# StephenTaf/Modern-Search-Engines-Project

Measured on AMD Instinct MI355X. Metric: queries/sec, two-stage retrieval top-100 (BM25 top-1000 + dense full scan + rerank/fuse), higher is better.
Workload: dtype f32 (exact f32 cosines of every returned document; candidates filtered by one pass of f16 products with a measured margin; batches <= 64 queries: f16x2-split products, |err| <= 8e-6) (dense cosine) / f64 (BM25, fuse)

## Files before the change

include/msretr.h:

```cpp
#ifndef MSRETR_H
#define MSRETR_H

#include <stdint.h>

#ifdef __cplusplus
extern "C" {
#endif

#define MSR_ABI_VERSION 15
#define MSR_DIM 768
#define MSR_MAX_K 1024
#define MSR_MAX_QUERY_TERMS 64
#define MSR_RERANK_MAX_CHUNKS 10
#define MSR_TERMSET_SPAN_DOCS 8192
#define MSR_PHRASE_MAX_TERMS 16
#define MSR_PROX_MAX_SPAN 64
#define MSR_SNIPPET_MAX_WEIGHT (1 << 20)
#define MSR_FUZZY_MAX_LEN 32
#define MSR_FUZZY_MAX_WORDS 1024
#define MSR_FUZZY_MAX_LIMIT 16
#define MSR_FUZZY_SPAN_TERMS 1024
#define MSR_FUZZY_WORD_GROUP 16
#define MSR_MERGE_MAX_ENTRIES 8192

typedef enum msr_status {
    MSR_OK = 0,
    MSR_ERR_INVALID = -1,
    MSR_ERR_NOT_BOUND = -2,
    MSR_ERR_HIP = -3,
    MSR_ERR_NOMEM = -4
} msr_status;

typedef struct msr_engine msr_engine;

typedef struct msr_config {
    int32_t struct_size;
    int32_t device;
    int32_t dim;
    int32_t max_queries;
    int32_t max_k;
    int32_t rerank_max_docs;
    int32_t scan_layout;
    int32_t scan_variant;
    int32_t flags;
} msr_config;

#define MSR_CFG_NO_ROW_COPY 1

typedef struct msr_rerank_params {
    double smoothing;
    double max_boost;
    double max_decay;
    int32_t max_chunks;
    int32_t reserved;
} msr_rerank_params;

int msr_abi_version(void);
int msr_create(const msr_config* cfg, msr_engine** out);
int msr_destroy(msr_engine* e);
const char* msr_last_error(const msr_engine* e);

int msr_bind_postings(msr_engine* e, const int64_t* term_off, int64_t n_terms, const int32_t* post_doc,
                      const int32_t* post_tf, int64_t n_postings, const int32_t* doc_len, int64_t n_docs,
                      const float* idf, float avgdl, double k1, double b, void* stream);

int msr_bind_chunks(msr_engine* e, const float* emb, int64_t n_chunks, const int32_t* doc_off,
                    int64_t n_docs, const float* inv_norm, void* stream);
int msr_row_copy_state(const msr_engine* e);
int msr_row_image_state(const msr_engine* e);
int64_t msr_owned_bytes(const msr_engine* e);

int msr_unbind(msr_engine* e);

int msr_bind_doc_meta(msr_engine* e, const int32_t* url_group, int64_t n_docs, void* stream);

int msr_scan_arith(const msr_engine* e);

int msr_scan_width(const msr_engine* e);
int msr_dense_path(const msr_engine* e);
int msr_batch_width(const msr_engine* e);
int msr_batch_gemm_ok(const msr_engine* e);

int msr_interleave_rows(msr_engine* e, const float* src, int64_t n_rows, float* dst, void* stream);

int msr_bm25_topk(msr_engine* e, const int32_t* q_term_off, const int32_t* q_terms, const int32_t* q_qtf,
                  int32_t n_queries, int32_t k, double min_score, int32_t* out_doc, double* out_score,
                  int32_t* out_n, void* stream);

int msr_bm25_topk_within(msr_engine* e, const int32_t* q_term_off, const int32_t* q_terms, const int32_t* q_qtf,
                         int32_t n_queries, int32_t k, double min_score,
                         const uint32_t* set_bits, int32_t n_sets, int64_t set_stride, const int32_t* q_set,
                         int32_t* out_doc, double* out_score, int32_t* out_n, void* stream);

int msr_term_sets(msr_engine* e, int32_t n_rows, const int32_t* must_off, const int32_t* must_terms,
                  const int32_t* not_off, const int32_t* not_terms,
                  const uint32_t* base_bits, int32_t n_base, int64_t base_stride, const int32_t* row_base,
                  uint32_t* out_bits, int64_t out_stride, void* stream);

int msr_bind_tokens(msr_engine* e, const int64_t* tok_off, const int32_t* tok_ids, int64_t n_docs, int64_t n_tokens,
                    void* stream);

int msr_phrase_sets(msr_engine* e, int32_t n_rows, const int32_t* phrase_off, const int32_t* phrase_terms,
                    const uint32_t* cand_bits, int32_t n_cand, int64_t cand_stride, const int32_t* row_cand,
                    uint32_t* out_bits, int64_t out_stride, void* stream);

int msr_proximity_sets(msr_engine* e, int32_t n_rows, const int32_t* phrase_off, const int32_t* phrase_terms,
                       const int32_t* row_span, const int32_t* row_ordered,
                       const uint32_t* cand_bits, int32_t n_cand, int64_t cand_stride, const int32_t* row_cand,
                       uint32_t* out_bits, int64_t out_stride, void* stream);

int msr_best_windows(msr_engine* e, int32_t n_pairs, const int32_t* pair_doc, const int32_t* pair_row,
                     int32_t n_rows, const int32_t* row_off, const int32_t* row_terms, const int32_t* row_weights,
                     const int32_t* row_span, int32_t* out_start, int32_t* out_cover, int32_t* out_hits, uint64_t* out_mask,
                     uint32_t* out_terms, void* stream);

int msr_bind_vocab(msr_engine* e, const int64_t* char_off, const uint16_t* chars, const uint32_t* weight, int64_t n_terms,
                   int64_t n_chars, void* stream);
int64_t msr_fuzzy_scratch_bytes(int64_t n_terms, int32_t n_words, int32_t limit);
int msr_fuzzy_terms(msr_engine* e, int32_t n_words, const int32_t* word_off, const uint16_t* word_chars, const int32_t* word_max,
                    int32_t limit, int32_t* out_term, int32_t* out_dist, int32_t* out_n, int32_t* out_total, void* scratch,
                    int64_t scratch_bytes, void* stream);

int msr_combine_sets(msr_engine* e, int32_t n_rows, const int32_t* and_off, const int32_t* and_rows,
                     const int32_t* not_off, const int32_t* not_rows,
                     const uint32_t* in_bits, int32_t n_in, int64_t in_stride,
                     uint32_t* out_bits, int64_t out_stride, void* stream);

int msr_debug_bm25_split(msr_engine* e, int32_t n_queries, int32_t* tiles_per_item, int32_t* n_segments);

enum { MSR_SELECT_F32 = 0, MSR_SELECT_F64 = 1, MSR_SELECT_F32_WITHIN = 2, MSR_SELECT_F64_LIST = 3 };
typedef struct msr_select_state {
    uint64_t pref_hi, mask_hi;
    uint32_t pref_lo, mask_lo;
    int32_t k_rem, n_above, done, n_sel;
} msr_select_state;
int msr_debug_select(msr_engine* e, int32_t mode, const void* scores, int64_t n, int64_t stride, int32_t n_queries, int32_t k,
                     const int32_t* idx, const int32_t* counts, int32_t n_seg, int64_t seg_stride, const uint64_t* win_base,
                     const uint32_t* set_bits, int32_t n_sets, int64_t set_stride, const int32_t* q_set, const int32_t* gate,
                     int32_t gate_per64, int32_t* out_doc, void* out_score, int32_t* out_n, msr_select_state* out_state,
                     void* stream);

int msr_bm25_score_docs(msr_engine* e, const int32_t* q_term_off, const int32_t* q_terms, const int32_t* q_qtf,
                        int32_t n_queries, const int32_t* doc, const int32_t* doc_n, int32_t max_docs,
                        double* out_score, int32_t* out_touched, void* stream);
int msr_union_candidates(msr_engine* e, int32_t n_queries,
                         const int32_t* lex_doc, const double* lex_score, const int32_t* lex_n, int32_t k_lex,
                         const int32_t* dense_doc, const double* dense_bm25, const int32_t* dense_n, int32_t k_dense,
                         int32_t* out_doc, double* out_score, int32_t* out_src, int32_t* out_n, int32_t max_cand,
                         void* stream);

int msr_dense_topk(msr_engine* e, const float* q, int32_t n_queries, int32_t k, int32_t max_chunks_per_doc,
                   int32_t* out_doc, float* out_score, int32_t* out_chunk, int32_t* out_n, void* stream);

int msr_dense_topk_within(msr_engine* e, const float* q, int32_t n_queries, int32_t k, int32_t max_chunks_per_doc,
                          const uint32_t* set_bits, int32_t n_sets, int64_t set_stride, const int32_t* q_set,
                          int32_t* out_doc, float* out_score, int32_t* out_chunk, int32_t* out_n, void* stream);

int msr_gather_rows(msr_engine* e, const int32_t* rows, int32_t n, float* out, void* stream);
int msr_dense_topk_grouped(msr_engine* e, const float* q, int32_t n_rows, const int32_t* group_off, int32_t n_groups,
                           const int32_t* excl_off, const int32_t* excl_doc, int32_t k, float min_score,
                           const uint32_t* set_bits, int32_t n_sets, int64_t set_stride, const int32_t* g_set,
                           int32_t* out_doc, float* out_score, int32_t* out_chunk, int32_t* out_src_row, int32_t* out_n,
                           void* stream);

int msr_dense_split_max(const msr_engine* e, int32_t k);
int msr_dense_topk_begin(msr_engine* e, const float* q, int32_t n_queries, int32_t k, int32_t k_part, float* out_part,
                         void* stream);
int msr_dense_topk_end(msr_engine* e, int32_t n_queries, int32_t k, const float* bound, int32_t* out_doc, float* out_score,
                       int32_t* out_chunk, int32_t* out_n, void* stream);

int msr_enable_bf16(msr_engine* e, void* stream);
int msr_dense_topk_bf16(msr_engine* e, const float* q, int32_t n_queries, int32_t k, int32_t max_chunks_per_doc,
                        int32_t* out_doc, float* out_score, int32_t* out_chunk, int32_t* out_n, void* stream);

int msr_rerank(msr_engine* e, const float* q, int32_t n_queries, const int32_t* cand_doc,
               const double* cand_bm25, const int32_t* cand_n, int32_t max_cand,
               const msr_rerank_params* params, int32_t* out_doc, double* out_score, double* out_orig,
               int32_t* out_chunk, int32_t* out_n, int32_t* out_rows, void* stream);

int msr_bind_doc_domains(msr_engine* e, const int32_t* domain, int64_t n_docs, void* stream);
int msr_diversify(msr_engine* e, int32_t n_queries, const int32_t* fused_doc, const double* fused_score,
                  const double* fused_orig, const int32_t* fused_chunk, const int32_t* fused_n, int32_t max_cand,
                  int32_t top_k, double relevance_threshold, int32_t diversify, int32_t* out_doc, double* out_score,
                  double* out_orig, int32_t* out_chunk, int32_t* out_n, void* stream);

int64_t msr_format_lines(const char* qnum_blob, const int64_t* qnum_off, int32_t n_queries, const int32_t* doc,
                         const double* score, const int32_t* n, int32_t stride, const char* url_blob, const int64_t* url_off,
                         int64_t n_docs, int64_t max_url_len, char* out, int64_t capacity);

int msr_rerank_gather(msr_engine* e, const float* q, int32_t n_queries, const int32_t* cand_doc,
                      const int32_t* cand_n, int32_t max_cand, int32_t doc_base, int32_t row_base,
                      int32_t max_chunks, float* out_cos, int32_t* out_meta, void* stream);
int msr_rerank_gather_blocks(msr_engine* e, const float* q, int32_t n_queries, const int32_t* cand_doc,
                             const int32_t* cand_n, int32_t max_cand, int32_t doc_base, int32_t row_base,
                             int32_t max_chunks, int32_t* out_blocks, int32_t queries_per_block, int64_t block_words,
                             void* stream);
int msr_rerank_fuse(msr_engine* e, int32_t n_queries, const int32_t* cand_doc, const double* cand_bm25,
                    const int32_t* cand_n, int32_t max_cand, const float* cos, const int32_t* meta,
                    const msr_rerank_params* params, int32_t* out_doc, double* out_score, double* out_orig,
                    int32_t* out_chunk, int32_t* out_n, int32_t* out_rows, void* stream);

int msr_rerank_combine(msr_engine* e, const float* cos_parts, const int32_t* meta_parts, int32_t n_parts,
                       int64_t part_stride_bytes, int32_t n_queries, int32_t max_cand, float* out_cos,
                       int32_t* out_meta, void* stream);

int msr_rerank_plan(msr_engine* e, int32_t n_queries, const int32_t* cand_doc, const int32_t* cand_n, int32_t max_cand,
                    const int32_t* shard_bounds, int32_t n_shards, int32_t my_shard, int32_t queries_per_shard,
                    int32_t* counts, int32_t* send_base, int32_t* send_blk, int32_t* recv_off, int32_t* pair, void* stream);
int msr_rerank_gather_records(msr_engine* e, const float* q, int32_t n_queries, const int32_t* cand_doc,
                              const int32_t* cand_n, int32_t max_cand, int32_t doc_base, int32_t row_base,
                              int32_t max_chunks, const int32_t* send_base, const int32_t* send_blk, int32_t* out_records,
                              int64_t capacity_records, void* stream);
int msr_rerank_scatter(msr_engine* e, const int32_t* records, int64_t capacity_records, const int32_t* counts,
                       const int32_t* recv_off, int32_t n_shards, int32_t n_queries, int32_t queries_per_shard,
                       int32_t first_query, int32_t n_my_queries, int32_t max_cand, float* out_cos, int32_t* out_meta,
                       void* stream);

int msr_merge_topk(msr_engine* e, const int32_t* in_doc, const void* in_score, const int32_t* in_n,
                   int32_t n_parts, int32_t n_queries, int32_t k, int32_t score_bits, int32_t* out_doc,
                   void* out_score, int32_t* out_n, void* stream);
int msr_merge_topk_payload(msr_engine* e, const int32_t* in_doc, const void* in_score, const int32_t* in_n,
                           const int32_t* in_payload, int32_t n_parts, int64_t part_stride_bytes, int32_t n_queries,
                           int32_t k, int32_t score_bits, int32_t* out_doc, void* out_score, int32_t* out_n,
                           int32_t* out_payload, void* stream);

int msr_build_postings(const int64_t* tok_off, const int32_t* tok_ids, int64_t n_docs, int32_t n_terms, int64_t* term_off,
                       int32_t* post_doc, int32_t* post_tf, int64_t capacity, int64_t* n_postings, void* stream);

int msr_merge_postings(const int64_t* a_term_off, int64_t a_terms, const int32_t* a_doc, const int32_t* a_tf,
                       const int32_t* a_map, int64_t a_docs, const int64_t* b_term_off, int64_t b_terms, const int32_t* b_doc,
                       const int32_t* b_tf, const int32_t* b_map, int64_t b_docs, int64_t n_terms, int64_t n_docs,
                       int64_t* term_off, int32_t* post_doc, int32_t* post_tf, int64_t capacity, void* stream);
// ... 18 lines not shown
```

modern-search-engines-project_amd/_abi.py:

```python
import ctypes as C
import os

HERE = os.path.dirname(os.path.abspath(__file__))
LIB_PATH = os.path.join(HERE, "csrc", "libmsretr.so")

MSR_ABI_VERSION = 15
MSR_CFG_NO_ROW_COPY = 1
MSR_DIM = 768
MSR_MAX_K = 1024
MSR_RERANK_MAX_CHUNKS = 10
MSR_MERGE_MAX_ENTRIES = 8192
MSR_TERMSET_SPAN_DOCS = 8192
MSR_PHRASE_MAX_TERMS = 16
MSR_PROX_MAX_SPAN = 64
MSR_SNIPPET_MAX_WEIGHT = 1 << 20
MSR_FUZZY_MAX_LEN = 32
MSR_FUZZY_MAX_WORDS = 1024
MSR_FUZZY_MAX_LIMIT = 16
MSR_FUZZY_SPAN_TERMS = 1024
MSR_FUZZY_WORD_GROUP = 16
MSR_SELECT_F32, MSR_SELECT_F64, MSR_SELECT_F32_WITHIN, MSR_SELECT_F64_LIST = 0, 1, 2, 3


class MsrError(RuntimeError):
    def __init__(self, code, msg):
        super().__init__(f"libmsretr error {code}: {msg}")
        self.code = code


class MsrConfig(C.Structure):
    _fields_ = [("struct_size", C.c_int32), ("device", C.c_int32), ("dim", C.c_int32),
                ("max_queries", C.c_int32), ("max_k", C.c_int32), ("rerank_max_docs", C.c_int32),
                ("scan_layout", C.c_int32), ("scan_variant", C.c_int32), ("flags", C.c_int32)]


class MsrSelectState(C.Structure):
    _fields_ = [("pref_hi", C.c_uint64), ("mask_hi", C.c_uint64), ("pref_lo", C.c_uint32), ("mask_lo", C.c_uint32),
                ("k_rem", C.c_int32), ("n_above", C.c_int32), ("done", C.c_int32), ("n_sel", C.c_int32)]


class MsrRerankParams(C.Structure):
    _fields_ = [("smoothing", C.c_double), ("max_boost", C.c_double), ("max_decay", C.c_double),
                ("max_chunks", C.c_int32), ("reserved", C.c_int32)]


_P = C.c_void_p
_SIGNATURES = {
    "msr_abi_version": (C.c_int, []),
    "msr_create": (C.c_int, [C.POINTER(MsrConfig), C.POINTER(_P)]),
    "msr_destroy": (C.c_int, [_P]),
    "msr_last_error": (C.c_char_p, [_P]),
    "msr_bind_postings": (C.c_int, [_P, _P, C.c_int64, _P, _P, C.c_int64, _P, C.c_int64, _P, C.c_float,
                                    C.c_double, C.c_double, _P]),
    "msr_bind_chunks": (C.c_int, [_P, _P, C.c_int64, _P, C.c_int64, _P, _P]),
    "msr_bind_doc_meta": (C.c_int, [_P, _P, C.c_int64, _P]),
    "msr_unbind": (C.c_int, [_P]),
    "msr_scan_arith": (C.c_int, [_P]),
    "msr_scan_width": (C.c_int, [_P]),
    "msr_dense_path": (C.c_int, [_P]),
    "msr_row_copy_state": (C.c_int, [_P]),
    "msr_row_image_state": (C.c_int, [_P]),
    "msr_owned_bytes": (C.c_int64, [_P]),
    "msr_enc_layernorm": (C.c_int, [_P, _P, _P, _P, _P, C.c_int64, C.c_int32, C.c_float, _P]),
    "msr_enc_attention": (C.c_int, [_P, _P, C.c_int32, C.c_int32, _P, C.c_int32, C.c_int32, _P, _P]),
    "msr_enc_attention_long": (C.c_int, [_P, _P, C.c_int32, C.c_int32, _P, C.c_int32, C.c_int32, _P, _P]),
    "msr_enc_geglu": (C.c_int, [_P, _P, C.c_int64, C.c_int32, _P]),
    "msr_enc_linear": (C.c_int, [_P, _P, _P, _P, C.c_int32, C.c_int32, C.c_int32, _P]),
    "msr_enc_mean_pool": (C.c_int, [_P, _P, C.c_int32, C.c_int32, C.c_int32, _P, _P]),
    "msr_batch_width": (C.c_int, [_P]),
    "msr_batch_gemm_ok": (C.c_int, [_P]),
    "msr_interleave_rows": (C.c_int, [_P, _P, C.c_int64, _P, _P]),
    "msr_bm25_topk": (C.c_int, [_P, _P, _P, _P, C.c_int32, C.c_int32, C.c_double, _P, _P, _P, _P]),
    "msr_dense_topk": (C.c_int, [_P, _P, C.c_int32, C.c_int32, C.c_int32, _P, _P, _P, _P, _P]),
    "msr_bm25_topk_within": (C.c_int, [_P, _P, _P, _P, C.c_int32, C.c_int32, C.c_double, _P, C.c_int32, C.c_int64, _P, _P, _P,
                                       _P, _P]),
    "msr_dense_topk_within": (C.c_int, [_P, _P, C.c_int32, C.c_int32, C.c_int32, _P, C.c_int32, C.c_int64, _P, _P, _P, _P, _P,
                                        _P]),
    "msr_term_sets": (C.c_int, [_P, C.c_int32, _P, _P, _P, _P, _P, C.c_int32, C.c_int64, _P, _P, C.c_int64, _P]),
    "msr_bind_tokens": (C.c_int, [_P, _P, _P, C.c_int64, C.c_int64, _P]),
    "msr_phrase_sets": (C.c_int, [_P, C.c_int32, _P, _P, _P, C.c_int32, C.c_int64, _P, _P, C.c_int64, _P]),
    "msr_proximity_sets": (C.c_int, [_P, C.c_int32, _P, _P, _P, _P, _P, C.c_int32, C.c_int64, _P, _P, C.c_int64, _P]),
    "msr_best_windows": (C.c_int, [_P, C.c_int32, _P, _P, C.c_int32, _P, _P, _P, _P, _P, _P, _P, _P, _P, _P]),
    "msr_bind_vocab": (C.c_int, [_P, _P, _P, _P, C.c_int64, C.c_int64, _P]),
    "msr_fuzzy_scratch_bytes": (C.c_int64, [C.c_int64, C.c_int32, C.c_int32]),
    "msr_fuzzy_terms": (C.c_int, [_P, C.c_int32, _P, _P, _P, C.c_int32, _P, _P, _P, _P, _P, C.c_int64, _P]),
    "msr_combine_sets": (C.c_int, [_P, C.c_int32, _P, _P, _P, _P, _P, C.c_int32, C.c_int64, _P, C.c_int64, _P]),
    "msr_debug_bm25_split": (C.c_int, [_P, C.c_int32, C.POINTER(C.c_int32), C.POINTER(C.c_int32)]),
    "msr_debug_select": (C.c_int, [_P, C.c_int32, _P, C.c_int64, C.c_int64, C.c_int32, C.c_int32, _P, _P, C.c_int32, C.c_int64, _P,
                                   _P, C.c_int32, C.c_int64, _P, _P, C.c_int32, _P, _P, _P, _P, _P]),
    "msr_bm25_score_docs": (C.c_int, [_P, _P, _P, _P, C.c_int32, _P, _P, C.c_int32, _P, _P, _P]),
    "msr_union_candidates": (C.c_int, [_P, C.c_int32, _P, _P, _P, C.c_int32, _P, _P, _P, C.c_int32, _P, _P, _P, _P, C.c_int32, _P]),
    "msr_gather_rows": (C.c_int, [_P, _P, C.c_int32, _P, _P]),
    "msr_dense_topk_grouped": (C.c_int, [_P, _P, C.c_int32, _P, C.c_int32, _P, _P, C.c_int32, C.c_float, _P, C.c_int32, C.c_int64,
                                         _P, _P, _P, _P, _P, _P, _P]),
    "msr_dense_split_max": (C.c_int, [_P, C.c_int32]),
    "msr_dense_topk_begin": (C.c_int, [_P, _P, C.c_int32, C.c_int32, C.c_int32, _P, _P]),
    "msr_dense_topk_end": (C.c_int, [_P, C.c_int32, C.c_int32, _P, _P, _P, _P, _P, _P]),
    "msr_enable_bf16": (C.c_int, [_P, _P]),
    "msr_dense_topk_bf16": (C.c_int, [_P, _P, C.c_int32, C.c_int32, C.c_int32, _P, _P, _P, _P, _P]),
    "msr_rerank": (C.c_int, [_P, _P, C.c_int32, _P, _P, _P, C.c_int32, C.POINTER(MsrRerankParams), _P, _P, _P,
                             _P, _P, _P, _P]),
    "msr_bind_doc_domains": (C.c_int, [_P, _P, C.c_int64, _P]),
    "msr_diversify": (C.c_int, [_P, C.c_int32, _P, _P, _P, _P, _P, C.c_int32, C.c_int32, C.c_double, C.c_int32, _P, _P, _P, _P,
                                _P, _P]),
    "msr_format_lines": (C.c_int64, [_P, _P, C.c_int32, _P, _P, _P, C.c_int32, _P, _P, C.c_int64, C.c_int64, _P, C.c_int64]),
    "msr_rerank_gather": (C.c_int, [_P, _P, C.c_int32, _P, _P, C.c_int32, C.c_int32, C.c_int32, C.c_int32, _P, _P, _P]),
    "msr_rerank_gather_blocks": (C.c_int, [_P, _P, C.c_int32, _P, _P, C.c_int32, C.c_int32, C.c_int32, C.c_int32, _P, C.c_int32,
                                           C.c_int64, _P]),
    "msr_rerank_fuse": (C.c_int, [_P, C.c_int32, _P, _P, _P, C.c_int32, _P, _P, C.POINTER(MsrRerankParams), _P, _P,
                                  _P, _P, _P, _P, _P]),
    "msr_rerank_combine": (C.c_int, [_P, _P, _P, C.c_int32, C.c_int64, C.c_int32, C.c_int32, _P, _P, _P]),
    "msr_rerank_plan": (C.c_int, [_P, C.c_int32, _P, _P, C.c_int32, _P, C.c_int32, C.c_int32, C.c_int32, _P, _P, _P, _P, _P, _P]),
    "msr_rerank_gather_records": (C.c_int, [_P, _P, C.c_int32, _P, _P, C.c_int32, C.c_int32, C.c_int32, C.c_int32, _P, _P, _P, C.c_int64,
                                            _P]),
    "msr_rerank_scatter": (C.c_int, [_P, _P, C.c_int64, _P, _P, C.c_int32, C.c_int32, C.c_int32, C.c_int32, C.c_int32, C.c_int32, _P, _P, _P]),
    "msr_merge_topk": (C.c_int, [_P, _P, _P, _P, C.c_int32, C.c_int32, C.c_int32, C.c_int32, _P, _P, _P, _P]),
    "msr_merge_topk_payload": (C.c_int, [_P, _P, _P, _P, _P, C.c_int32, C.c_int64, C.c_int32, C.c_int32, C.c_int32, _P, _P, _P,
                                         _P, _P]),
    "msr_build_postings": (C.c_int, [_P, _P, C.c_int64, C.c_int32, _P, _P, _P, C.c_int64, C.POINTER(C.c_int64), _P]),
    "msr_merge_postings": (C.c_int, [_P, C.c_int64, _P, _P, _P, C.c_int64, _P, C.c_int64, _P, _P, _P, C.c_int64, C.c_int64,
                                     C.c_int64, _P, _P, _P, C.c_int64, _P]),
    "msr_compact_postings": (C.c_int, [_P, C.c_int64, _P, _P, _P, C.c_int64, _P, _P, _P, C.c_int64, C.POINTER(C.c_int64), _P]),
    "msr_debug_exclusive_scan": (C.c_int, [_P, C.c_int64, _P, _P, _P]),
    "msr_debug_chunk_layout": (C.c_int, [_P, C.c_int64, C.POINTER(C.c_int32)]),
    "msr_set_timing": (C.c_int, [_P, C.c_int32]),
    "msr_tune": (C.c_int, [_P, C.c_int32, C.c_int32]),
    "msr_kernel_time_ms": (C.c_int, [_P, C.c_int32, C.POINTER(C.c_float), C.POINTER(C.c_int32)]),
}
EXPORTS = tuple(_SIGNATURES)

_lib = None


def load():
    global _lib
    if _lib is not None:
        return _lib
    if not os.path.exists(LIB_PATH):
        raise MsrError(-100, f"{LIB_PATH} not found: build it with `python -c 'import __graft_entry__ as g; "
                             f"g.build()'` (the product path has no CPU fallback)")
    import torch
    lib = C.CDLL(LIB_PATH)
    for name, (res, args) in _SIGNATURES.items():
        fn = getattr(lib, name)
        fn.restype, fn.argtypes = res, args
    if lib.msr_abi_version() != MSR_ABI_VERSION:
        raise MsrError(-101, f"ABI version {lib.msr_abi_version()} != {MSR_ABI_VERSION}")
    _lib = lib
    return lib


def check(handle, rc):
    if rc != 0:
        msg = load().msr_last_error(handle)
        raise MsrError(rc, msg.decode("utf-8", "replace") if msg else "?")
```

modern-search-engines-project_amd/csrc/msr_engine.hip:

```cpp
#include <hip/hip_runtime.h>
#include <stdarg.h>
#include <stdio.h>
#include <stdlib.h>
#include <string.h>

#include <algorithm>
#include <new>
#include <vector>

#include "../../include/msretr.h"
#include "msr_devmem.h"
#include "msr_internal.h"

struct HipMem {
    static hipError_t alloc(void** p, size_t bytes) { return hipMalloc(p, bytes); }
    static void free(void* p) { (void)hipFree(p); }
};
using Group = DevGroup<HipMem>;

struct msr_engine {
    msr_config cfg;
    char err[512];
    Group mem_engine;
    Group mem_corpus;
    Group mem_postings;
    Group mem_chunks;
    Group mem_bf16;
    Bm25Index bm25{};
    bool have_postings = false;
    const int64_t* tok_off = nullptr;
    const int32_t* tok_ids = nullptr;
    int64_t n_tokens = 0;
    bool have_tokens = false;
    const int64_t* voc_char_off = nullptr;
    const uint16_t* voc_chars = nullptr;
    const uint32_t* voc_weight = nullptr;
    int64_t voc_n_chars = 0;
    bool have_vocab = false;
    DenseIndex dense{};
    bool have_chunks = false;
    const int32_t* url_group = nullptr;
    int64_t url_group_n = 0;
    const int32_t* doc_domain = nullptr;
    int64_t doc_domain_n = 0;
    int32_t* chunk_doc = nullptr;
    void* emb_presplit = nullptr;
    void* row_meta = nullptr;
    float* inv_norm_own = nullptr;
    int32_t* span_doc = nullptr;
    int32_t* wspan_doc = nullptr;
    int32_t* wspan12_doc = nullptr;
    float* qn = nullptr;
    float* rr_qn = nullptr;
    void* qimg = nullptr;
    SelScratch sel{};
    float* rerank_cos = nullptr;
    int32_t* rerank_meta = nullptr;
    void* score_rows = nullptr;
    size_t score_rows_bytes = 0;
    int32_t* bm_cand_doc = nullptr;
    size_t bm_cand_bytes = 0;
    int32_t* bm_heavy_id = nullptr;
    void* bm_post = nullptr;
    int32_t* bm_dense_id = nullptr;
    double* bm_dense = nullptr;
    uint32_t* bm_tile_off = nullptr;
    int32_t* bm_cand_n = nullptr;
    uint64_t* bm_win = nullptr;
    uint64_t* voc_sig = nullptr;
    int32_t* bt_top_doc = nullptr; float* bt_top_score = nullptr; int32_t* bt_top_n = nullptr;
    int32_t* bt_cand_doc = nullptr; float* bt_cand_score = nullptr; int32_t* bt_cand_chunk = nullptr;
    int32_t* bt_cand_n = nullptr;
    int32_t* tile_row = nullptr;
    int n_tiles = 0;
    bool tiles_ok = false;
    GemmF32Index gf{};
    bool gf_ok = false;
    float* gf_inv_pad = nullptr; float* gf_qn = nullptr; void* gf_fb_qimg = nullptr;
    int32_t* gf_gate = nullptr;
    void* gf_emb_tiled = nullptr;
    void* gf_emb_f16 = nullptr;
    int32_t* tile_trow = nullptr;
    void* emb_bf16 = nullptr;
    GemmIndex gemm{};
    bool gemm_ok = false;
    float* gm_qn = nullptr;
    uint32_t* bf_err = nullptr;
    float* bf_margin = nullptr;
    float* bf_ones = nullptr;
    void* bf_row_meta = nullptr;
    DenseIndex dense_bf16{};
    int n_cus = 256;
    int split_pending = 0;
    int row_copy_state = 0;
    int row_image_state = 0;
    int last_dense_width = 0;
    int32_t* sim_flag = nullptr;
    void* sim_lists = nullptr; size_t sim_lists_bytes = 0;
    void* sim_over = nullptr; size_t sim_over_bytes = 0;
    bool timing = false;
    static constexpr int EV_RING = 256;
    static constexpr int EV_KINDS = 4;
    hipEvent_t ev_start[EV_KINDS][EV_RING] = {};
    hipEvent_t ev_stop[EV_KINDS][EV_RING] = {};
    int ev_count[EV_KINDS] = {0, 0, 0, 0};
};

static constexpr size_t GF_GATE_BYTES = 16 * sizeof(int32_t);

static thread_local char g_create_err[512] = "";

static int fail(msr_engine* e, int code, const char* fmt, ...) {
    char* dst = e ? e->err : g_create_err;
    va_list ap;
    va_start(ap, fmt);
    vsnprintf(dst, 512, fmt, ap);
    va_end(ap);
    return code;
}

#define HIP_TRY(e, call)                                                                          \
    do {                                                                                          \
        hipError_t _err = (call);                                                                 \
        if (_err != hipSuccess) return fail(e, MSR_ERR_HIP, "%s: %s", #call, hipGetErrorString(_err)); \
    } while (0)

#define ALLOC(e, group, slot, bytes)                                                              \
    do {                                                                                          \
        const size_t _n = (bytes);                                                                \
        hipError_t _err = (group).alloc(&(slot), _n);                                             \
        if (_err != hipSuccess) return fail(e, MSR_ERR_NOMEM, "%s (%zu bytes): %s", #slot, _n, hipGetErrorString(_err)); \
    } while (0)

static void drop_vocab(msr_engine* e) {
    e->have_vocab = false;
    e->voc_char_off = nullptr; e->voc_chars = nullptr; e->voc_weight = nullptr; e->voc_n_chars = 0;
    e->mem_postings.free_one(&e->voc_sig);
}
static void drop_postings(msr_engine* e) {
    e->have_postings = e->have_tokens = false;
    e->tok_off = nullptr; e->tok_ids = nullptr; e->n_tokens = 0;
    drop_vocab(e);
    e->bm25 = Bm25Index{};
    e->mem_postings.release();
}
static void drop_bf16(msr_engine* e) {
    e->dense.emb_bf16 = nullptr;
    e->dense_bf16 = DenseIndex{};
    e->gemm = GemmIndex{};
    e->gemm_ok = false;
    e->mem_bf16.release();
}
static void drop_chunks(msr_engine* e) {
    e->have_chunks = false;
    e->split_pending = 0;
    e->dense = DenseIndex{};
    e->gf = GemmF32Index{};
    e->gf_ok = e->tiles_ok = false;
    e->n_tiles = 0;
    e->row_copy_state = e->row_image_state = 0;
    drop_bf16(e);
    e->mem_chunks.release();
}

template <class T>
static int grow(msr_engine* e, Group& group, T** slot, size_t* have, size_t need, const char* what) {
    if (need <= *have && *slot) return MSR_OK;
    group.free_one(slot);
    *have = 0;
    hipError_t herr = group.alloc(slot, need);
    if (herr != hipSuccess) return fail(e, MSR_ERR_NOMEM, "%s (%zu bytes): %s", what, need, hipGetErrorString(herr));
    *have = need;
    return MSR_OK;
}

extern "C" int msr_abi_version(void) { return MSR_ABI_VERSION; }

extern "C" const char* msr_last_error(const msr_engine* e) { return e ? e->err : g_create_err; }

int msr_fail_global(int code, const char* fmt, ...) {
    va_list ap;
    va_start(ap, fmt);
    vsnprintf(g_create_err, sizeof(g_create_err), fmt, ap);
    va_end(ap);
    return code;
}

static int create_scratch(msr_engine* e) {
    const msr_config& cfg = e->cfg;
    HIP_TRY(e, hipSetDevice(cfg.device));
    hipDeviceProp_t prop;
    HIP_TRY(e, hipGetDeviceProperties(&prop, cfg.device));
    e->n_cus = prop.multiProcessorCount > 0 ? prop.multiProcessorCount : 256;
    const size_t nq = (size_t)std::max(cfg.max_queries, 128);
    ALLOC(e, e->mem_engine, e->qn, 128 * MSR_DIM * sizeof(float));
    ALLOC(e, e->mem_engine, e->qimg, 256 * 1024);
    if (cfg.rerank_max_docs > 0) ALLOC(e, e->mem_engine, e->rr_qn, nq * MSR_DIM * sizeof(float));
    ALLOC(e, e->mem_engine, e->sel.hist, nq * MSR_SEL_BINS * sizeof(uint32_t));
    ALLOC(e, e->mem_engine, e->sel.state, nq * sizeof(SelState));
    ALLOC(e, e->mem_engine, e->sel.cand_hi, nq * MSR_SEL_CAP * sizeof(uint64_t));
    ALLOC(e, e->mem_engine, e->sel.cand_lo, nq * MSR_SEL_CAP * sizeof(uint32_t));
    ALLOC(e, e->mem_engine, e->sel.cand_n, nq * sizeof(int32_t));
    HIP_TRY(e, hipMemset(e->sel.hist, 0, nq * MSR_SEL_BINS * sizeof(uint32_t)));
    HIP_TRY(e, hipMemset(e->sel.cand_n, 0, nq * sizeof(int32_t)));
    if (cfg.rerank_max_docs > 0) {
        ALLOC(e, e->mem_engine, e->rerank_cos, nq * (size_t)cfg.rerank_max_docs * MSR_RERANK_MAX_CHUNKS * sizeof(float));
        ALLOC(e, e->mem_engine, e->rerank_meta, nq * (size_t)cfg.rerank_max_docs * 3 * sizeof(int32_t));
    }
    for (int w = 0; w < msr_engine::EV_KINDS; ++w)
        for (int j = 0; j < msr_engine::EV_RING; ++j) {
            HIP_TRY(e, hipEventCreate(&e->ev_start[w][j]));
            HIP_TRY(e, hipEventCreate(&e->ev_stop[w][j]));
        }
    return MSR_OK;
}

extern "C" int msr_create(const msr_config* cfg, msr_engine** out) {
    if (!cfg || !out) return fail(nullptr, MSR_ERR_INVALID, "msr_create: null argument");
    *out = nullptr;
    if (cfg->struct_size != (int32_t)sizeof(msr_config))
        return fail(nullptr, MSR_ERR_INVALID, "msr_create: struct_size %d != %zu", cfg->struct_size, sizeof(msr_config));
    if (cfg->dim != MSR_DIM) return fail(nullptr, MSR_ERR_INVALID, "msr_create: dim must be %d", MSR_DIM);
    if (cfg->max_queries < 1 || cfg->max_queries > 4096)
        return fail(nullptr, MSR_ERR_INVALID, "msr_create: max_queries out of range [1, 4096]");
    if (cfg->max_k < 1 || cfg->max_k > MSR_MAX_K)
        return fail(nullptr, MSR_ERR_INVALID, "msr_create: max_k out of range [1, %d]", MSR_MAX_K);
    if (cfg->rerank_max_docs < 0 || cfg->rerank_max_docs > 1024)
        return fail(nullptr, MSR_ERR_INVALID, "msr_create: rerank_max_docs out of range [0, 1024]");
    if (cfg->scan_layout != 0 && cfg->scan_layout != 1)
        return fail(nullptr, MSR_ERR_INVALID, "msr_create: scan_layout must be 0 or 1");
    if (cfg->scan_variant != 0 && cfg->scan_variant != 2 && cfg->scan_variant != 7 && cfg->scan_variant != 14 &&
        cfg->scan_variant != 15)
        return fail(nullptr, MSR_ERR_INVALID, "msr_create: scan_variant must be 0, 2, 7, 14 or 15");
    if (cfg->flags & ~(int32_t)MSR_CFG_NO_ROW_COPY)
        return fail(nullptr, MSR_ERR_INVALID, "msr_create: unknown flag bits 0x%x", cfg->flags);
    int ndev = 0;
    hipError_t herr = hipGetDeviceCount(&ndev);
    if (herr != hipSuccess || ndev <= 0)
        return fail(nullptr, MSR_ERR_HIP, "msr_create: no HIP device available (%s)",
                    herr == hipSuccess ? "device count is 0" : hipGetErrorString(herr));
    if (cfg->device < 0 || cfg->device >= ndev)
        return fail(nullptr, MSR_ERR_INVALID, "msr_create: device %d out of range (have %d)", cfg->device, ndev);
    msr_engine* e = new (std::nothrow) msr_engine();
    if (!e) return fail(nullptr, MSR_ERR_NOMEM, "msr_create: out of host memory");
    e->cfg = *cfg;
    e->err[0] = 0;
    const int rc = create_scratch(e);
    if (rc) {
        fail(nullptr, rc, "msr_create: %s", e->err);
        msr_destroy(e);
        return rc;
    }
    *out = e;
    return MSR_OK;
}

extern "C" int msr_destroy(msr_engine* e) {
    if (!e) return MSR_OK;
    drop_postings(e);
    drop_chunks(e);
    for (int w = 0; w < msr_engine::EV_KINDS; ++w)
        for (int j = 0; j < msr_engine::EV_RING; ++j) {
            if (e->ev_start[w][j]) (void)hipEventDestroy(e->ev_start[w][j]);
            if (e->ev_stop[w][j]) (void)hipEventDestroy(e->ev_stop[w][j]);
        }
    delete e;
    return MSR_OK;
}

static int ensure_score_rows(msr_engine* e, int64_t n_docs) {
    const size_t pad = (size_t)(n_docs + 31) / 32 * 32;
    const size_t need = std::max((size_t)e->cfg.max_queries * pad * sizeof(double), (size_t)128 * pad * sizeof(float));
    return grow(e, e->mem_corpus, &e->score_rows, &e->score_rows_bytes, need, "score rows");
}

static int build_postings(msr_engine* e, Bm25Index cand, hipStream_t st) {
    const int64_t n_terms = cand.n_terms, n_postings = cand.n_postings, n_docs = cand.n_docs;
    int rc = ensure_score_rows(e, n_docs);
    if (rc) return rc;
    rc = grow(e, e->mem_corpus, &e->bm_cand_doc, &e->bm_cand_bytes, (size_t)e->cfg.max_queries * (size_t)n_docs * sizeof(int32_t),
              "BM25 candidate lists");
    if (rc) return rc;
    ALLOC(e, e->mem_postings, e->bm_win, (size_t)e->cfg.max_queries * sizeof(uint64_t));
    ALLOC(e, e->mem_postings, e->bm_cand_n, (size_t)e->cfg.max_queries * msr_bm25_max_segments(n_docs) * sizeof(int32_t));
    int32_t h_flag = 0;
    HIP_TRY(e, msr_bm25_validate(cand, e->sel.cand_n, st));
    HIP_TRY(e, hipMemcpyAsync(&h_flag, e->sel.cand_n, sizeof(int32_t), hipMemcpyDeviceToHost, st));
    HIP_TRY(e, hipMemsetAsync(e->sel.cand_n, 0, sizeof(int32_t), st));
    HIP_TRY(e, hipStreamSynchronize(st));
    if (h_flag >= 1 && h_flag <= 5) {
        static const char* why[] = {"", "term_off is not a monotone offset array ending at n_postings",
                                    "a posting's document index is outside [0, n_docs)",
                                    "documents are not strictly ascending inside a posting list",
                                    "negative doc_len", "non-positive term frequency"};
        return fail(e, MSR_ERR_INVALID, "msr_bind_postings: malformed index: %s", why[h_flag]);
    }
    if (!(cand.avgdl > 0.0) || !(cand.k1 >= 0.0) || !(cand.b >= 0.0 && cand.b <= 1.0))
        return fail(e, MSR_ERR_INVALID, "msr_bind_postings: avgdl must be > 0, k1 >= 0, 0 <= b <= 1");
    std::vector<int32_t> dense_terms;
    if (n_terms > 0) {
        std::vector<int64_t> h_toff((size_t)n_terms + 1);
        std::vector<float> h_idf((size_t)n_terms);
        HIP_TRY(e, hipMemcpyAsync(h_toff.data(), cand.term_off, h_toff.size() * sizeof(int64_t), hipMemcpyDeviceToHost, st));
        HIP_TRY(e, hipMemcpyAsync(h_idf.data(), cand.idf, h_idf.size() * sizeof(float), hipMemcpyDeviceToHost, st));
        HIP_TRY(e, hipStreamSynchronize(st));
        std::vector<int32_t> heavy_id((size_t)n_terms, -1), heavy_terms;
        for (int64_t t = 0; t < n_terms; ++t)
            if (h_toff[t + 1] - h_toff[t] >= MSR_BM25_HEAVY_DF && h_toff[t + 1] - h_toff[t] < (1ll << 32)) {
                heavy_id[t] = (int32_t)heavy_terms.size();
                heavy_terms.push_back((int32_t)t);
                if (h_idf[t] < 0.0f) dense_terms.push_back((int32_t)t);
            }
        if (!heavy_terms.empty()) {
            DevTemp<HipMem, int32_t> d_terms;
            const size_t rows = heavy_terms.size() * (size_t)(cand.n_tiles + 1);
            ALLOC(e, e->mem_postings, e->bm_heavy_id, heavy_id.size() * sizeof(int32_t));
            ALLOC(e, e->mem_postings, e->bm_tile_off, rows * sizeof(uint32_t));
            ALLOC(e, d_terms.group, d_terms.p, heavy_terms.size() * sizeof(int32_t));
            HIP_TRY(e, hipMemcpyAsync(e->bm_heavy_id, heavy_id.data(), heavy_id.size() * sizeof(int32_t), hipMemcpyHostToDevice, st));
            HIP_TRY(e, hipMemcpyAsync(d_terms.p, heavy_terms.data(), heavy_terms.size() * sizeof(int32_t), hipMemcpyHostToDevice, st));
            HIP_TRY(e, msr_bm25_build_skip(cand, d_terms.p, (int)heavy_terms.size(), e->bm_tile_off, st));
            HIP_TRY(e, hipStreamSynchronize(st));
            cand.heavy_id = e->bm_heavy_id;
            cand.tile_off = e->bm_tile_off;
        }
        std::stable_sort(dense_terms.begin(), dense_terms.end(), [&](int32_t a, int32_t b2) {
            return h_toff[a + 1] - h_toff[a] > h_toff[b2 + 1] - h_toff[b2];
        });
        const size_t row_bytes = ((size_t)cand.n_tiles * MSR_BM25_TILE + 8) * sizeof(double);
        const size_t cap = std::min<size_t>(MSR_BM25_MAX_DENSE, (size_t)(4ull << 30) / row_bytes);
        if (dense_terms.size() > cap) dense_terms.resize(cap);
    }
    {
        const int64_t n_pad = (int64_t)cand.n_tiles * MSR_BM25_TILE;
        DevTemp<HipMem, double> dnorm;
        ALLOC(e, e->mem_postings, e->bm_post, (size_t)(n_postings + 1) * sizeof(Bm25Post));
        ALLOC(e, dnorm.group, dnorm.p, (size_t)n_pad * sizeof(double));
        HIP_TRY(e, msr_bm25_dnorm(cand.doc_len, n_docs, n_pad, cand.k1, cand.b, cand.avgdl, dnorm.p, st));
        HIP_TRY(e, msr_bm25_post_comp(cand.post_doc, cand.post_tf, dnorm.p, cand.k1, n_postings, (Bm25Post*)e->bm_post, st));
        HIP_TRY(e, hipStreamSynchronize(st));
    }
    cand.post = (const Bm25Post*)e->bm_post;
    if (!dense_terms.empty()) {
        const int64_t stride = (int64_t)cand.n_tiles * MSR_BM25_TILE + 8;
        std::vector<int32_t> dense_id((size_t)n_terms, -1);
        for (size_t h = 0; h < dense_terms.size(); ++h) dense_id[dense_terms[h]] = (int32_t)h;
        DevTemp<HipMem, int32_t> d_terms;
        ALLOC(e, e->mem_postings, e->bm_dense_id, dense_id.size() * sizeof(int32_t));
        ALLOC(e, e->mem_postings, e->bm_dense, dense_terms.size() * (size_t)stride * sizeof(double));
        ALLOC(e, d_terms.group, d_terms.p, dense_terms.size() * sizeof(int32_t));
        HIP_TRY(e, hipMemcpyAsync(e->bm_dense_id, dense_id.data(), dense_id.size() * sizeof(int32_t), hipMemcpyHostToDevice, st));
        HIP_TRY(e, hipMemcpyAsync(d_terms.p, dense_terms.data(), dense_terms.size() * sizeof(int32_t), hipMemcpyHostToDevice, st));
        HIP_TRY(e, hipMemsetAsync(e->bm_dense, 0, dense_terms.size() * (size_t)stride * sizeof(double), st));
        HIP_TRY(e, msr_bm25_build_dense(cand, d_terms.p, (int)dense_terms.size(), e->bm_dense, stride, st));
        HIP_TRY(e, hipStreamSynchronize(st));
        cand.dense_id = e->bm_dense_id;
        cand.dense_comp = e->bm_dense;
        cand.dense_stride = stride;
    }
    e->bm25 = cand;
    return MSR_OK;
}

extern "C" int msr_bind_postings(msr_engine* e, const int64_t* term_off, int64_t n_terms, const int32_t* post_doc,
                                 const int32_t* post_tf, int64_t n_postings, const int32_t* doc_len, int64_t n_docs,
                                 const float* idf, float avgdl, double k1, double b, void* stream) {
    if (!e) return MSR_ERR_INVALID;
    if (!term_off || !doc_len || !idf || n_terms < 0 || n_postings < 0 || n_docs <= 0 || n_docs >= (1ll << 31) ||
        (n_postings > 0 && (!post_doc || !post_tf)))
        return fail(e, MSR_ERR_INVALID, "msr_bind_postings: bad argument");
    if (e->have_chunks && e->dense.n_docs != n_docs)
        return fail(e, MSR_ERR_INVALID, "msr_bind_postings: n_docs %lld differs from bound chunks (%lld)",
                    (long long)n_docs, (long long)e->dense.n_docs);
    HIP_TRY(e, hipSetDevice(e->cfg.device));
    drop_postings(e);
    const Bm25Index cand{term_off, post_doc, post_tf, doc_len, idf, n_terms, n_postings, n_docs, (double)avgdl, k1, b,
                         nullptr, nullptr, (int32_t)((n_docs + MSR_BM25_TILE - 1) / MSR_BM25_TILE), nullptr, nullptr, nullptr, 0};
    const int rc = build_postings(e, cand, (hipStream_t)stream);
    if (rc) drop_postings(e);
    e->have_postings = rc == MSR_OK;
    return rc;
}

struct ChunkLayout {
    std::vector<int32_t> spans, wspans, wspans12;
    int wide_ok = 1, wide_ok64 = 1;
    bool tiles_ok = true;
    std::vector<int32_t> tiles;
    std::vector<int32_t> trow;
    int64_t n_trows = 0;
};

static int chunk_layout(msr_engine* e, int n_cus, const std::vector<int32_t>& h_off, int64_t n_chunks, int64_t n_docs,
                        ChunkLayout& L) {
    if (h_off[0] != 0 || (int64_t)h_off[n_docs] != n_chunks)
        return fail(e, MSR_ERR_INVALID, "msr_bind_chunks: doc_off[0]=%d, doc_off[n_docs]=%d, n_chunks=%lld",
                    h_off[0], h_off[n_docs], (long long)n_chunks);
    for (int64_t d = 0; d < n_docs; ++d)
        if (h_off[d + 1] < h_off[d]) return fail(e, MSR_ERR_INVALID, "msr_bind_chunks: doc_off not monotone at %lld", (long long)d);
    auto make_spans = [&](int target, int64_t min_rows) {
        if ((int64_t)target * min_rows > n_chunks) target = (int)std::max<int64_t>(1, n_chunks / min_rows);
        std::vector<int32_t> sp;
        sp.push_back(0);
        for (int s = 1; s < target; ++s) {
            const int64_t want = n_chunks * s / target;
            int64_t d = std::lower_bound(h_off.begin(), h_off.end(), (int32_t)want) - h_off.begin();
            if (d > n_docs) d = n_docs;
            if (d > sp.back()) sp.push_back((int32_t)d);
        }
        if (sp.back() != (int32_t)n_docs) sp.push_back((int32_t)n_docs);
        return sp;
    };
    L.spans = make_spans(n_cus, 256);
    L.wspans = make_spans(n_cus * 8, 64);
    L.wspans12 = make_spans(n_cus * 12, 64);
    {
        const int64_t n_groups = (n_chunks + 15) / 16;
        int64_t dl = 0, dr = 0;
        for (int64_t u = 0; u < n_groups && (L.wide_ok || L.wide_ok64); ++u) {
            const int64_t first = 16 * u, last = std::min<int64_t>(16 * (u + 2), n_chunks) - 1;
            while (h_off[dl + 1] <= first) ++dl;
            if (dr < dl) dr = dl;
            while (h_off[dr + 1] <= last) ++dr;
            if (dr - dl + 32 > MSR_WIDE_RING) L.wide_ok = 0;
            if (dr - dl + 32 > 64) L.wide_ok64 = 0;
            int64_t dm = dl;
            const int64_t glast = std::min<int64_t>(16 * (u + 1), n_chunks) - 1;
            while (h_off[dm + 1] <= glast) ++dm;
            if (dm - dl > 32) L.wide_ok = L.wide_ok64 = 0;
        }
    }
    if (L.wide_ok || L.wide_ok64) {
        int64_t lag = 0;
        for (size_t s = 0; s + 1 < L.spans.size(); ++s) {
            const int64_t d0 = L.spans[s], d1 = L.spans[s + 1];
            const int64_t c0 = h_off[d0], c1 = h_off[d1];
            if (c1 <= c0) continue;
            auto block_end = [&](int64_t b) -> int64_t { return h_off[std::min(b + 32, d1)]; };
            int64_t next_b = d0 & ~(int64_t)31;
            while (next_b < d1 && block_end(next_b) <= c0) next_b += 32;
            int64_t d = d0;
            for (int64_t g = c0 >> 4; g < (c1 + 15) >> 4; ++g) {
                const int64_t last = std::min(16 * g + 16, c1) - 1;
                while (h_off[d + 1] <= last) ++d;
                lag = std::max(lag, d - next_b);
                for (int i = 0; i < 2 && next_b < d1 && block_end(next_b) <= 16 * g; ++i) next_b += 32;
            }
        }
        if (lag >= MSR_WIDE_RING) L.wide_ok = 0;
        if (lag >= 64) L.wide_ok64 = 0;
    }
    int32_t start = 0;
    L.tiles.push_back(0);
    for (int64_t d = 0; d < n_docs && L.tiles_ok; ++d) {
        const int32_t end = h_off[d + 1];
        if (end - h_off[d] > 256) L.tiles_ok = false;
        if (end - start > 256) { L.tiles.push_back(h_off[d]); start = h_off[d]; }
    }
    if (!L.tiles_ok) return MSR_OK;
    if (L.tiles.back() != (int32_t)n_chunks) L.tiles.push_back((int32_t)n_chunks);
    const size_t n_tiles = L.tiles.size() - 1;
    L.trow.resize(n_tiles);
    for (size_t t = 0; t < n_tiles; ++t) {
        L.trow[t] = (int32_t)L.n_trows;
        L.n_trows += (L.tiles[t + 1] - L.tiles[t] + 15) / 16 * 16;
    }
    if (L.n_trows + MSR_STREAM256_TILE_ROWS >= ((int64_t)1 << 31)) { L.trow.clear(); L.n_trows = 0; }
    return MSR_OK;
}

static int bind_chunk_tables(msr_engine* e, const float* emb, int64_t n_chunks, const int32_t* doc_off, int64_t n_docs,
                             const float* inv_norm, const ChunkLayout& L, hipStream_t st) {
    ALLOC(e, e->mem_chunks, e->chunk_doc, (size_t)n_chunks * sizeof(int32_t));
    ALLOC(e, e->mem_chunks, e->span_doc, L.spans.size() * sizeof(int32_t));
    ALLOC(e, e->mem_chunks, e->wspan_doc, L.wspans.size() * sizeof(int32_t));
    HIP_TRY(e, hipMemcpyAsync(e->span_doc, L.spans.data(), L.spans.size() * sizeof(int32_t), hipMemcpyHostToDevice, st));
    HIP_TRY(e, hipMemcpyAsync(e->wspan_doc, L.wspans.data(), L.wspans.size() * sizeof(int32_t), hipMemcpyHostToDevice, st));
    ALLOC(e, e->mem_chunks, e->wspan12_doc, L.wspans12.size() * sizeof(int32_t));
    HIP_TRY(e, hipMemcpyAsync(e->wspan12_doc, L.wspans12.data(), L.wspans12.size() * sizeof(int32_t), hipMemcpyHostToDevice, st));
    HIP_TRY(e, msr_fill_chunk_doc(doc_off, n_docs, e->chunk_doc, st));
    if (!inv_norm) {
        ALLOC(e, e->mem_chunks, e->inv_norm_own, (size_t)n_chunks * sizeof(float));
        HIP_TRY(e, msr_row_inv_norm(emb, n_chunks, e->inv_norm_own, st));
        inv_norm = e->inv_norm_own;
    }
    if (L.wide_ok) {
        ALLOC(e, e->mem_chunks, e->row_meta, (size_t)(n_chunks + 16) * 8);
        HIP_TRY(e, msr_pack_row_meta(e->chunk_doc, inv_norm, n_chunks, e->row_meta, st));
    }
    int variant = e->cfg.scan_variant;
    if (variant == 0) {
        uint32_t h_rng[2] = {0, 0};
        HIP_TRY(e, msr_inv_norm_range(inv_norm, n_chunks, (uint32_t*)e->sel.cand_n, st));
        HIP_TRY(e, hipMemcpyAsync(h_rng, e->sel.cand_n, sizeof(h_rng), hipMemcpyDeviceToHost, st));
        HIP_TRY(e, hipMemsetAsync(e->sel.cand_n, 0, 2 * sizeof(int32_t), st));
        HIP_TRY(e, hipStreamSynchronize(st));
        float lo, hi;
        memcpy(&lo, &h_rng[0], 4); memcpy(&hi, &h_rng[1], 4);
        variant = (lo >= 0.5f && hi <= 2.0f) ? 7 : 2;
        if (variant == 7 && e->cfg.scan_layout == 0 && L.wide_ok) variant = 14;
    }
    if (variant == 15) {
        if (e->cfg.scan_layout != 0 || !L.wide_ok) {
            variant = 7;
        } else {
            ALLOC(e, e->mem_chunks, e->emb_presplit, (size_t)n_chunks * MSR_DIM * sizeof(float));
            HIP_TRY(e, msr_presplit_rows(emb, n_chunks, e->emb_presplit, st));
        }
    }
    e->dense = DenseIndex{emb, doc_off, e->chunk_doc, inv_norm, e->span_doc, n_chunks, n_docs, (n_docs + 31) / 32 * 32,
                          (int)L.spans.size() - 1, e->cfg.scan_layout, e->wspan_doc, (int)L.wspans.size() - 1, e->wspan12_doc,
                          (int)L.wspans12.size() - 1, e->qimg, nullptr, e->emb_presplit, e->row_meta, L.wide_ok,
                          L.wide_ok && L.wide_ok64, nullptr, variant};
    if (L.tiles_ok) {
        ALLOC(e, e->mem_chunks, e->tile_row, L.tiles.size() * 4);
        HIP_TRY(e, hipMemcpyAsync(e->tile_row, L.tiles.data(), L.tiles.size() * 4, hipMemcpyHostToDevice, st));
        e->n_tiles = (int)L.tiles.size() - 1;
        e->tiles_ok = true;
    }
    if (!L.trow.empty()) {
        ALLOC(e, e->mem_chunks, e->tile_trow, L.trow.size() * 4);
        HIP_TRY(e, hipMemcpyAsync(e->tile_trow, L.trow.data(), L.trow.size() * 4, hipMemcpyHostToDevice, st));
    }
    HIP_TRY(e, hipStreamSynchronize(st));
    return MSR_OK;
}

static int bind_stream_pass(msr_engine* e, const ChunkLayout& L, hipStream_t st) {
    if (!(e->tiles_ok && e->dense.variant == 14 && e->n_tiles >= 64)) return MSR_OK;
    const float* emb = e->dense.emb;
    const float* inv_norm = e->dense.inv_norm;
    const int64_t n_chunks = e->dense.n_chunks;
    const int n_tiles = e->n_tiles, nw = e->n_cus * 8, stride = (n_tiles + 31) / 32 * 32;
    const int groups = std::min(8, std::max(e->cfg.max_queries, 128) / 128);
    const int GF_WV_CAP = 4096 * std::max(1, groups / 2);
    const size_t QM = (size_t)groups * 128;
    const int max_nt = std::max(1, std::min(4, groups / 2));
    GemmF32Index& g = e->gf;
    g.n_tiles = n_tiles; g.n_cus = e->n_cus; g.max_groups = groups; g.tmax_stride = stride; g.wv_cap = GF_WV_CAP; g.max_nt = max_nt;
    ALLOC(e, e->mem_chunks, e->gf_inv_pad, (size_t)(n_chunks + 512) * 4);
    ALLOC(e, e->mem_chunks, g.qimg, (size_t)groups * 24 * 8192);
    ALLOC(e, e->mem_chunks, e->gf_qn, (QM + 64) * MSR_DIM * 4);
    ALLOC(e, e->mem_chunks, e->gf_fb_qimg, (QM + 63) / 64 * msr_ksplit_slice_image_bytes());
    ALLOC(e, e->mem_chunks, g.tmax_t, (size_t)n_tiles * 8 * (groups >= 2 ? 256 * max_nt : 128) * 4);
    ALLOC(e, e->mem_chunks, g.tmax, QM * stride * 4);
    ALLOC(e, e->mem_chunks, g.thr, QM * 4);
    ALLOC(e, e->mem_chunks, g.thr2, QM * 4);
    ALLOC(e, e->mem_chunks, g.flag, QM * 4);
    ALLOC(e, e->mem_chunks, g.wvbuf, (size_t)nw * GF_WV_CAP * 16);
    ALLOC(e, e->mem_chunks, g.wv_count, (size_t)nw * 4);
    ALLOC(e, e->mem_chunks, g.pairs, QM * 4096 * 8);
    ALLOC(e, e->mem_chunks, g.pair_n, QM * 4);
    ALLOC(e, e->mem_chunks, e->gf_gate, GF_GATE_BYTES);
    ALLOC(e, e->mem_chunks, g.err_max, 4);
    ALLOC(e, e->mem_chunks, g.margin, QM * 4);
    ALLOC(e, e->mem_chunks, g.cand_doc, QM * MSR_SEL_CAP * 4);
    ALLOC(e, e->mem_chunks, g.cand_score, QM * MSR_SEL_CAP * 4);
    ALLOC(e, e->mem_chunks, g.cand_chunk, QM * MSR_SEL_CAP * 4);
    ALLOC(e, e->mem_chunks, g.cand_n, QM * 4);
    g.tile_row = e->tile_row;
    g.inv_pad = e->gf_inv_pad;
    HIP_TRY(e, msr_pad_inv_norm(inv_norm, n_chunks, n_chunks + 512, e->gf_inv_pad, st));
    HIP_TRY(e, hipMemsetAsync(g.pair_n, 0, QM * 4, st));
    HIP_TRY(e, hipMemsetAsync(e->gf_gate, 0, GF_GATE_BYTES, st));
    HIP_TRY(e, hipMemsetAsync(g.cand_n, 0, QM * 4, st));
    HIP_TRY(e, msr_f16_row_error(emb, inv_norm, n_chunks, g.err_max, st));
    if (groups >= 2 && e->tile_trow) {
        const size_t copy_rows = (size_t)L.n_trows + MSR_STREAM256_TILE_ROWS;
        if ((int64_t)L.trow.back() + MSR_STREAM256_TILE_ROWS > (int64_t)copy_rows)
            return fail(e, MSR_ERR_INVALID, "msr_bind_chunks: internal: tile table exceeds the fragment-order copy");
        if (e->cfg.flags & MSR_CFG_NO_ROW_COPY) {
            e->row_copy_state = 2;
        } else if (e->mem_chunks.alloc(&e->gf_emb_tiled, copy_rows * MSR_DIM * 4) != hipSuccess) {
            (void)hipGetLastError();
            e->row_copy_state = 3;
        } else {
            HIP_TRY(e, hipMemsetAsync((char*)e->gf_emb_tiled + (size_t)L.n_trows * MSR_DIM * 4, 0,
                                      (size_t)MSR_STREAM256_TILE_ROWS * MSR_DIM * 4, st));
            HIP_TRY(e, msr_tile_rows(emb, e->tile_row, e->tile_trow, n_tiles, e->gf_emb_tiled, st));
            e->row_copy_state = 1;
        }
    }
    if (max_nt >= 2 && (e->cfg.flags & MSR_CFG_NO_ROW_COPY)) {
        e->row_image_state = 2;
    } else if (max_nt >= 2) {
        const size_t img_rows = (size_t)n_chunks + 512;
        if (e->mem_chunks.alloc(&e->gf_emb_f16, img_rows * MSR_DIM * 2) != hipSuccess) {
            (void)hipGetLastError();
            e->row_image_state = 3;
        } else {
            HIP_TRY(e, msr_f16_rows(emb, n_chunks, (int64_t)img_rows, e->gf_emb_f16, st));
            e->row_image_state = 1;
        }
    }
    g.emb_tiled = e->gf_emb_tiled;
    g.tile_trow = e->gf_emb_tiled ? e->tile_trow : nullptr;
    g.emb_f16 = e->gf_emb_f16;
    e->gf_ok = true;
    return MSR_OK;
}

extern "C" int msr_bind_chunks(msr_engine* e, const float* emb, int64_t n_chunks, const int32_t* doc_off,
                               int64_t n_docs, const float* inv_norm, void* stream) {
    if (!e) return MSR_ERR_INVALID;
    if (!emb || !doc_off || n_chunks <= 0 || n_chunks >= (1ll << 31) || n_docs <= 0 || n_docs >= (1ll << 31))
        return fail(e, MSR_ERR_INVALID, "msr_bind_chunks: bad argument");
    if (e->have_postings && e->bm25.n_docs != n_docs)
        return fail(e, MSR_ERR_INVALID, "msr_bind_chunks: n_docs %lld differs from bound postings (%lld)",
                    (long long)n_docs, (long long)e->bm25.n_docs);
    if (e->cfg.scan_layout == 1 && !inv_norm)
        return fail(e, MSR_ERR_INVALID, "msr_bind_chunks: inv_norm is required with the interleaved layout");
    hipStream_t st = (hipStream_t)stream;
    HIP_TRY(e, hipSetDevice(e->cfg.device));
    std::vector<int32_t> h_off((size_t)n_docs + 1);
    HIP_TRY(e, hipMemcpyAsync(h_off.data(), doc_off, (size_t)(n_docs + 1) * sizeof(int32_t), hipMemcpyDeviceToHost, st));
    HIP_TRY(e, hipStreamSynchronize(st));
    ChunkLayout L;
    int rc = chunk_layout(e, e->n_cus, h_off, n_chunks, n_docs, L);
    if (rc) return rc;
    drop_chunks(e);
    rc = ensure_score_rows(e, n_docs);
    if (!rc) rc = bind_chunk_tables(e, emb, n_chunks, doc_off, n_docs, inv_norm, L, st);
    if (!rc) rc = bind_stream_pass(e, L, st);
    if (rc) drop_chunks(e);
    e->have_chunks = rc == MSR_OK;
    return rc;
}

extern "C" int msr_debug_chunk_layout(const int32_t* doc_off, int64_t n_docs, int32_t out[4]) {
    if (!doc_off || !out || n_docs < 0 || n_docs >= ((int64_t)1 << 31))
        return fail(nullptr, MSR_ERR_INVALID, "msr_debug_chunk_layout: bad argument");
    const int n_cus = out[3] > 0 ? out[3] : 256;
    const std::vector<int32_t> h_off(doc_off, doc_off + n_docs + 1);
    ChunkLayout L;
    const int rc = chunk_layout(nullptr, n_cus, h_off, h_off[n_docs], n_docs, L);
    if (rc) return rc;
    out[0] = L.wide_ok; out[1] = L.wide_ok && L.wide_ok64; out[2] = L.tiles_ok; out[3] = (int32_t)L.spans.size() - 1;
    return MSR_OK;
}

extern "C" int msr_unbind(msr_engine* e) {
    if (!e) return MSR_ERR_INVALID;
    HIP_TRY(e, hipSetDevice(e->cfg.device));
    drop_postings(e);
    drop_chunks(e);
    e->url_group = nullptr; e->url_group_n = 0;
    e->doc_domain = nullptr; e->doc_domain_n = 0;
    e->last_dense_width = 0;
    e->mem_corpus.release();
    e->score_rows_bytes = e->bm_cand_bytes = 0;
    return MSR_OK;
}

extern "C" int msr_bind_doc_meta(msr_engine* e, const int32_t* url_group, int64_t n_docs, void* stream) {
    (void)stream;
    if (!e) return MSR_ERR_INVALID;
    if (url_group && e->have_chunks && n_docs != e->dense.n_docs)
        return fail(e, MSR_ERR_INVALID, "msr_bind_doc_meta: n_docs mismatch");
    e->url_group = url_group;
    e->url_group_n = n_docs;
    return MSR_OK;
}

extern "C" int msr_bind_doc_domains(msr_engine* e, const int32_t* domain, int64_t n_docs, void* stream) {
    (void)stream;
    if (!e) return MSR_ERR_INVALID;
    if (n_docs < 0 || (domain && n_docs == 0)) return fail(e, MSR_ERR_INVALID, "msr_bind_doc_domains: bad argument");
    e->doc_domain = domain;
    e->doc_domain_n = domain ? n_docs : 0;
    return MSR_OK;
}

extern "C" int msr_diversify(msr_engine* e, int32_t n_queries, const int32_t* fused_doc, const double* fused_score,
                             const double* fused_orig, const int32_t* fused_chunk, const int32_t* fused_n, int32_t max_cand,
                             int32_t top_k, double relevance_threshold, int32_t diversify, int32_t* out_doc, double* out_score,
                             double* out_orig, int32_t* out_chunk, int32_t* out_n, void* stream) {
    if (!e) return MSR_ERR_INVALID;
    if (!fused_doc || !fused_score || !fused_orig || !fused_chunk || !fused_n || !out_doc || !out_score || !out_orig || !out_chunk ||
        !out_n)
        return fail(e, MSR_ERR_INVALID, "msr_diversify: null argument");
    if (n_queries < 0 || max_cand < 1 || max_cand > 1024 || top_k < 1)
        return fail(e, MSR_ERR_INVALID, "msr_diversify: bad argument (max_cand=%d, top_k=%d)", max_cand, top_k);
    if (n_queries == 0) return MSR_OK;
    HIP_TRY(e, hipSetDevice(e->cfg.device));
    HIP_TRY(e, msr_diversify_run(n_queries, fused_doc, fused_score, fused_orig, fused_chunk, fused_n, max_cand, e->doc_domain,
                                 e->doc_domain_n, top_k, relevance_threshold, diversify, out_doc, out_score, out_orig, out_chunk,
                                 out_n, (hipStream_t)stream));
    return MSR_OK;
}

extern "C" int msr_interleave_rows(msr_engine* e, const float* src, int64_t n_rows, float* dst, void* stream) {
    if (!e) return MSR_ERR_INVALID;
    if (!src || !dst || n_rows <= 0 || src == dst) return fail(e, MSR_ERR_INVALID, "msr_interleave_rows: bad argument");
    HIP_TRY(e, hipSetDevice(e->cfg.device));
    HIP_TRY(e, msr_interleave(src, n_rows, dst, (hipStream_t)stream));
    return MSR_OK;
}

extern "C" int msr_scan_arith(const msr_engine* e) {
    if (!e || !e->have_chunks) return -1;
    const int v = e->dense.variant;
    return (v == 7 || v == 14 || v == 15) ? 1 : 0;
}

extern "C" int msr_scan_width(const msr_engine* e) {
    if (!e || !e->have_chunks) return -1;
    const int v = e->dense.variant;
    const bool wide = (v == 2 || v == 14 || v == 15) && e->dense.layout == 0 && e->dense.wide_ok;
    if (e->gf_ok && wide && v == 14) return e->gf.max_groups >= 2 ? 256 : 128;
    return wide ? 64 : 32;
}

extern "C" int msr_dense_path(const msr_engine* e) { return e ? e->last_dense_width : -1; }

extern "C" int64_t msr_owned_bytes(const msr_engine* e) {
    if (!e) return -1;
    return (int64_t)(e->mem_engine.bytes() + e->mem_corpus.bytes() + e->mem_postings.bytes() + e->mem_chunks.bytes() +
                     e->mem_bf16.bytes());
}

extern "C" int msr_row_copy_state(const msr_engine* e) { return e ? e->row_copy_state : -1; }
extern "C" int msr_row_image_state(const msr_engine* e) { return e ? e->row_image_state : -1; }

extern "C" int msr_batch_width(const msr_engine* e) {
    if (!e || !e->have_chunks || !e->emb_bf16) return -1;
    return e->dense.wide_ok && e->dense.wide_ok64 ? 128 : 64;
}

extern "C" int msr_set_timing(msr_engine* e, int32_t enabled) {
    if (!e) return MSR_ERR_INVALID;
    e->timing = enabled != 0;
    for (int w = 0; w < msr_engine::EV_KINDS; ++w) e->ev_count[w] = 0;
    return MSR_OK;
}

extern "C" int msr_kernel_time_ms(msr_engine* e, int32_t which, float* out_ms, int32_t* out_launches) {
    if (!e || which < 0 || which >= msr_engine::EV_KINDS || !out_ms) return e ? fail(e, MSR_ERR_INVALID, "msr_kernel_time_ms: bad argument") : MSR_ERR_INVALID;
    const int n = std::min(e->ev_count[which], (int)msr_engine::EV_RING);
    if (n <= 0) return fail(e, MSR_ERR_INVALID, "msr_kernel_time_ms: no timed launch recorded");
    float total = 0.f;
    for (int j = 0; j < n; ++j) {
        float ms = 0.f;
        HIP_TRY(e, hipEventSynchronize(e->ev_stop[which][j]));
        HIP_TRY(e, hipEventElapsedTime(&ms, e->ev_start[which][j], e->ev_stop[which][j]));
        total += ms;
    }
    *out_ms = total;
    if (out_launches) *out_launches = n;
    return MSR_OK;
}

static int within_args_ok(msr_engine* e, const char* fn, int64_t n_docs, const uint32_t* set_bits, int32_t n_sets,
                          int64_t set_stride, const int32_t* q_set) {
    if (n_sets < 0) return fail(e, MSR_ERR_INVALID, "%s: bad argument (n_sets=%d)", fn, n_sets);
    if (n_sets == 0) return MSR_OK;
    if (!set_bits || !q_set) return fail(e, MSR_ERR_INVALID, "%s: bad argument (set_bits or q_set is NULL with n_sets=%d)", fn, n_sets);
    if (set_stride < (n_docs + 31) / 32)
        return fail(e, MSR_ERR_INVALID, "%s: bad argument (set_stride=%lld < ceil(n_docs / 32) = %lld)", fn, (long long)set_stride,
                    (long long)((n_docs + 31) / 32));
    return MSR_OK;
}

static int bm25_topk_impl(msr_engine* e, const char* fn, const int32_t* q_term_off, const int32_t* q_terms, const int32_t* q_qtf,
                          int32_t n_queries, int32_t k, double min_score, int32_t* out_doc, double* out_score, int32_t* out_n,
                          void* stream, const uint32_t* set_bits, int32_t n_sets, int64_t set_stride, const int32_t* q_set) {
    if (!e) return MSR_ERR_INVALID;
    if (!e->have_postings) return fail(e, MSR_ERR_NOT_BOUND, "%s: postings not bound", fn);
    if (n_queries < 0 || k < 1 || k > e->cfg.max_k || !q_term_off || !out_doc || !out_score || !out_n)
        return fail(e, MSR_ERR_INVALID, "%s: bad argument (k=%d, max_k=%d)", fn, k, e->cfg.max_k);
    {
        const int rc = within_args_ok(e, fn, e->bm25.n_docs, set_bits, n_sets, set_stride, q_set);
        if (rc) return rc;
    }
    if (n_queries == 0) return MSR_OK;
    const MsrSetView set_view{set_bits, set_stride, q_set, n_sets};
    const MsrSetView* set = n_sets > 0 ? &set_view : nullptr;
    hipStream_t st = (hipStream_t)stream;
    HIP_TRY(e, hipSetDevice(e->cfg.device));
    const int slice = e->cfg.max_queries;
    const int64_t N = e->bm25.n_docs;
    for (int q0 = 0; q0 < n_queries; q0 += slice) {
        const int nq = std::min(slice, n_queries - q0);
        int32_t* o_doc = out_doc + (int64_t)q0 * k;
        double* o_score = out_score + (int64_t)q0 * k;
        const bool timed = e->timing && e->ev_count[1] < msr_engine::EV_RING;
        int n_seg = 0;
        int64_t seg_stride = 0;
        if (timed) HIP_TRY(e, hipEventRecord(e->ev_start[1][e->ev_count[1]], st));
        HIP_TRY(e, msr_bm25_scores(e->bm25, q_term_off, q_terms, q_qtf, q0, nq, min_score, (double*)e->score_rows, e->bm_cand_doc,
                                   e->bm_cand_n, &n_seg, &seg_stride, st, set));
        if (timed) {
            HIP_TRY(e, hipEventRecord(e->ev_stop[1][e->ev_count[1]], st));
            e->ev_count[1]++;
        }
        const uint64_t* win = nullptr;
        if (min_score >= 0.0) {
            HIP_TRY(e, msr_bm25_window(e->bm25, q_term_off, q_terms, q_qtf, q0, nq, e->bm_win, st));
            win = e->bm_win;
        }
        HIP_TRY(e, msr_select_topk_list((const double*)e->score_rows, e->bm_cand_doc, e->bm_cand_n, n_seg, seg_stride, N, nq, k,
                                        e->sel, o_doc, o_score, out_n + q0, st, win));
    }
    return MSR_OK;
}

extern "C" int msr_bm25_topk(msr_engine* e, const int32_t* q_term_off, const int32_t* q_terms, const int32_t* q_qtf,
                             int32_t n_queries, int32_t k, double min_score, int32_t* out_doc, double* out_score,
                             int32_t* out_n, void* stream) {
    return bm25_topk_impl(e, "msr_bm25_topk", q_term_off, q_terms, q_qtf, n_queries, k, min_score, out_doc, out_score, out_n,
                          stream, nullptr, 0, 0, nullptr);
}

extern "C" int msr_bm25_topk_within(msr_engine* e, const int32_t* q_term_off, const int32_t* q_terms, const int32_t* q_qtf,
                                    int32_t n_queries, int32_t k, double min_score, const uint32_t* set_bits, int32_t n_sets,
                                    int64_t set_stride, const int32_t* q_set, int32_t* out_doc, double* out_score,
                                    int32_t* out_n, void* stream) {
    return bm25_topk_impl(e, "msr_bm25_topk_within", q_term_off, q_terms, q_qtf, n_queries, k, min_score, out_doc, out_score,
                          out_n, stream, set_bits, n_sets, set_stride, q_set);
}

static int tokens_bound(msr_engine* e, const char* fn) {
    if (e->have_postings && e->have_tokens) return MSR_OK;
    return fail(e, MSR_ERR_NOT_BOUND, "%s: tokens not bound (msr_bind_tokens: the index has no forward index)", fn);
}

static int set_rows_args_ok(msr_engine* e, const char* fn, int32_t n_rows, bool rows_ok, const char* rows_what, int64_t out_stride,
                            const char* n_in_name, int32_t n_in, bool in_ok, const char* in_what, const char* in_stride_name,
                            int64_t in_stride) {
    const int64_t W = (e->bm25.n_docs + 31) / 32;
    if (n_rows < 0 || n_in < 0) return fail(e, MSR_ERR_INVALID, "%s: bad argument (n_rows=%d, %s=%d)", fn, n_rows, n_in_name, n_in);
    if (n_rows > 0 && !rows_ok)
        return fail(e, MSR_ERR_INVALID, "%s: bad argument (%s is NULL with n_rows=%d)", fn, rows_what, n_rows);
    if (out_stride < W)
        return fail(e, MSR_ERR_INVALID, "%s: bad argument (out_stride=%lld < ceil(n_docs / 32) = %lld)", fn, (long long)out_stride,
                    (long long)W);
    if (n_in > 0 && !in_ok)
        return fail(e, MSR_ERR_INVALID, "%s: bad argument (%s is NULL with %s=%d)", fn, in_what, n_in_name, n_in);
    if (n_in > 0 && in_stride < W)
        return fail(e, MSR_ERR_INVALID, "%s: bad argument (%s=%lld < ceil(n_docs / 32) = %lld)", fn, in_stride_name,
                    (long long)in_stride, (long long)W);
    return MSR_OK;
}

extern "C" int msr_term_sets(msr_engine* e, int32_t n_rows, const int32_t* must_off, const int32_t* must_terms,
                             const int32_t* not_off, const int32_t* not_terms, const uint32_t* base_bits, int32_t n_base,
                             int64_t base_stride, const int32_t* row_base, uint32_t* out_bits, int64_t out_stride, void* stream) {
    if (!e) return MSR_ERR_INVALID;
    if (!e->have_postings) return fail(e, MSR_ERR_NOT_BOUND, "msr_term_sets: postings not bound");
    const int rc = set_rows_args_ok(e, "msr_term_sets", n_rows, out_bits && must_off && not_off, "out_bits, must_off or not_off",
                                    out_stride, "n_base", n_base, base_bits && row_base, "base_bits or row_base", "base_stride",
                                    base_stride);
    if (rc) return rc;
    if (n_rows == 0) return MSR_OK;
    HIP_TRY(e, hipSetDevice(e->cfg.device));
    HIP_TRY(e, msr_term_sets_run(e->bm25, n_rows, must_off, must_terms, not_off, not_terms, base_bits, n_base, base_stride,
                                 row_base, out_bits, out_stride, (hipStream_t)stream));
    return MSR_OK;
}

extern "C" int msr_bind_tokens(msr_engine* e, const int64_t* tok_off, const int32_t* tok_ids, int64_t n_docs, int64_t n_tokens,
                               void* stream) {
    if (!e) return MSR_ERR_INVALID;
    if (!e->have_postings) return fail(e, MSR_ERR_NOT_BOUND, "msr_bind_tokens: postings not bound");
    e->have_tokens = false; e->tok_off = nullptr; e->tok_ids = nullptr; e->n_tokens = 0;
    if (!tok_off || n_tokens < 0 || (n_tokens > 0 && !tok_ids)) return fail(e, MSR_ERR_INVALID, "msr_bind_tokens: bad argument");
    if (n_docs != e->bm25.n_docs)
// ... 155 lines not shown
}

extern "C" int msr_debug_bm25_split(msr_engine* e, int32_t n_queries, int32_t* tiles_per_item, int32_t* n_segments) {
    if (!e) return MSR_ERR_INVALID;
    if (!e->have_postings) return fail(e, MSR_ERR_NOT_BOUND, "msr_debug_bm25_split: postings not bound");
    if (n_queries < 1 || n_queries > e->cfg.max_queries || !tiles_per_item || !n_segments)
        return fail(e, MSR_ERR_INVALID, "msr_debug_bm25_split: bad argument (n_queries=%d, max_queries=%d)", n_queries,
                    e->cfg.max_queries);
    int tpw = 1, n_spans = 0;
    msr_bm25_split(e->bm25.n_tiles, n_queries, &tpw, &n_spans);
    *tiles_per_item = tpw;
    *n_segments = n_spans;
    return MSR_OK;
}

extern "C" int msr_debug_select(msr_engine* e, int32_t mode, const void* scores, int64_t n, int64_t stride, int32_t n_queries,
                                int32_t k, const int32_t* idx, const int32_t* counts, int32_t n_seg, int64_t seg_stride,
                                const uint64_t* win_base, const uint32_t* set_bits, int32_t n_sets, int64_t set_stride,
                                const int32_t* q_set, const int32_t* gate, int32_t gate_per64, int32_t* out_doc, void* out_score,
                                int32_t* out_n, msr_select_state* out_state, void* stream) {
    static_assert(sizeof(msr_select_state) == sizeof(SelState), "msr_select_state mirrors SelState");
    if (!e) return MSR_ERR_INVALID;
    if (mode < MSR_SELECT_F32 || mode > MSR_SELECT_F64_LIST)
        return fail(e, MSR_ERR_INVALID, "msr_debug_select: bad argument (mode=%d)", mode);
    if (n_queries < 1 || n_queries > e->cfg.max_queries || k < 1 || k > e->cfg.max_k)
        return fail(e, MSR_ERR_INVALID, "msr_debug_select: bad argument (n_queries=%d, max_queries=%d, k=%d, max_k=%d)", n_queries,
                    e->cfg.max_queries, k, e->cfg.max_k);
    if (!scores || !out_doc || !out_score || !out_n || n < 0 || n >= (1ll << 31) || stride < n)
        return fail(e, MSR_ERR_INVALID, "msr_debug_select: bad argument (NULL scores or output, or n=%lld, stride=%lld)",
                    (long long)n, (long long)stride);
    if (mode == MSR_SELECT_F64_LIST && (!idx || !counts || n_seg < 1 || seg_stride < 0 || (int64_t)n_seg * seg_stride > stride))
        return fail(e, MSR_ERR_INVALID, "msr_debug_select: bad argument (list: idx or counts NULL, n_seg=%d < 1, or n_seg * "
                    "seg_stride=%lld > stride=%lld)", n_seg, (long long)seg_stride, (long long)stride);
    if (mode == MSR_SELECT_F32_WITHIN &&
        (n_sets < 1 || !set_bits || !q_set || set_stride < (n + 31) / 32))
        return fail(e, MSR_ERR_INVALID, "msr_debug_select: bad argument (within: n_sets=%d < 1, set_bits or q_set NULL, or "
                    "set_stride=%lld < ceil(n / 32))", n_sets, (long long)set_stride);
    hipStream_t st = (hipStream_t)stream;
    HIP_TRY(e, hipSetDevice(e->cfg.device));
    SelScratch sel = e->sel;
    sel.gate = gate;
    sel.gate_per64 = gate && gate_per64 ? 1 : 0;
    switch (mode) {
    case MSR_SELECT_F32:
        HIP_TRY(e, msr_select_topk(32, scores, n, stride, n_queries, k, sel, out_doc, out_score, out_n, st));
        break;
    case MSR_SELECT_F64:
        HIP_TRY(e, msr_select_topk(64, scores, n, stride, n_queries, k, sel, out_doc, out_score, out_n, st));
        break;
    case MSR_SELECT_F32_WITHIN: {
        const MsrSetView set{set_bits, set_stride, q_set, n_sets};
        HIP_TRY(e, msr_select_topk_within((const float*)scores, n, stride, n_queries, k, sel, set, out_doc, (float*)out_score,
                                          out_n, st));
        break;
    }
    default:
        HIP_TRY(e, msr_select_topk_list((const double*)scores, idx, counts, n_seg, seg_stride, stride, n_queries, k, sel, out_doc,
                                        (double*)out_score, out_n, st, win_base));
    }
    if (out_state)
        HIP_TRY(e, hipMemcpyAsync(out_state, e->sel.state, (size_t)n_queries * sizeof(SelState), hipMemcpyDeviceToDevice, st));
    return MSR_OK;
}

extern "C" int msr_bm25_score_docs(msr_engine* e, const int32_t* q_term_off, const int32_t* q_terms, const int32_t* q_qtf,
                                   int32_t n_queries, const int32_t* doc, const int32_t* doc_n, int32_t max_docs,
                                   double* out_score, int32_t* out_touched, void* stream) {
    if (!e) return MSR_ERR_INVALID;
    if (!e->have_postings) return fail(e, MSR_ERR_NOT_BOUND, "msr_bm25_score_docs: postings not bound");
    if (n_queries < 0 || max_docs < 0 || !q_term_off || (n_queries > 0 && max_docs > 0 && (!doc || !out_score || !out_touched)))
        return fail(e, MSR_ERR_INVALID, "msr_bm25_score_docs: bad argument (n_queries=%d, max_docs=%d)", n_queries, max_docs);
    if (n_queries == 0 || max_docs == 0) return MSR_OK;
    HIP_TRY(e, hipSetDevice(e->cfg.device));
    HIP_TRY(e, msr_bm25_point(e->bm25, q_term_off, q_terms, q_qtf, n_queries, doc, doc_n, max_docs, out_score, out_touched,
                              (hipStream_t)stream));
    return MSR_OK;
}

extern "C" int msr_union_candidates(msr_engine* e, int32_t n_queries, const int32_t* lex_doc, const double* lex_score,
                                    const int32_t* lex_n, int32_t k_lex, const int32_t* dense_doc, const double* dense_bm25,
                                    const int32_t* dense_n, int32_t k_dense, int32_t* out_doc, double* out_score, int32_t* out_src,
                                    int32_t* out_n, int32_t max_cand, void* stream) {
    if (!e) return MSR_ERR_INVALID;
    if (n_queries < 0 || k_lex < 0 || k_lex > MSR_MAX_K || k_dense < 0 || k_dense > MSR_MAX_K || max_cand < 1 ||
        (int64_t)k_lex + k_dense > max_cand)
        return fail(e, MSR_ERR_INVALID, "msr_union_candidates: bad argument (k_lex=%d, k_dense=%d: each in [0, %d], their sum <= "
                    "max_cand=%d)", k_lex, k_dense, MSR_MAX_K, max_cand);
    if (!out_doc || !out_score || !out_src || !out_n || (k_lex > 0 && (!lex_doc || !lex_score || !lex_n)) ||
        (k_dense > 0 && (!dense_doc || !dense_bm25 || !dense_n)))
        return fail(e, MSR_ERR_INVALID, "msr_union_candidates: bad argument (NULL list)");
    if (n_queries == 0) return MSR_OK;
    HIP_TRY(e, hipSetDevice(e->cfg.device));
    HIP_TRY(e, msr_union_lists(n_queries, lex_doc, lex_score, lex_n, k_lex, dense_doc, dense_bm25, dense_n, k_dense, out_doc,
                               out_score, out_src, out_n, max_cand, (hipStream_t)stream));
    return MSR_OK;
}

static int dense_gated_fallback(msr_engine* e, int nq, int k, int32_t* out_doc, float* out_score, int32_t* out_chunk,
                                int32_t* out_n, hipStream_t st) {
    const int64_t N = e->dense.n_docs;
    DenseIndex ix = e->dense;
    ix.gate = e->gf_gate;
    HIP_TRY(e, msr_dense_scan_slices(ix, e->gf_qn, nq, (float*)e->score_rows, e->gf_fb_qimg, st));
    SelScratch sel = e->sel;
    sel.gate = e->gf_gate; sel.gate_per64 = 1;
    HIP_TRY(e, msr_select_topk(32, e->score_rows, N, e->dense.score_stride, nq, k, sel, out_doc, out_score, out_n, st));
    ix.gate = e->gf_gate; ix.gate_per64 = 1;
    if (out_chunk) HIP_TRY(e, msr_best_chunk(ix, e->gf_qn, nq, k, 0, out_doc, out_n, out_chunk, st));
    return MSR_OK;
}

static bool dense_sweep_wide(const msr_engine* e, int max_chunks_per_doc) {
    return (e->dense.variant == 2 || e->dense.variant == 14 || e->dense.variant == 15) && e->dense.layout == 0 &&
           e->dense.wide_ok && max_chunks_per_doc == 0;
}

static bool dense_stream_ok(const msr_engine* e, int k) {
    return dense_sweep_wide(e, 0) && e->gf_ok && e->dense.variant == 14 && e->gf.n_tiles >= 2 * k;
}

static int dense_stream_cap(const msr_engine* e) { return e->gf.max_groups >= 2 ? (e->gf.max_groups & ~1) * 128 : 128; }

static hipEvent_t* pass_events(msr_engine* e, int kind, hipEvent_t ev[4]) {
    if (!e->timing || e->ev_count[kind] >= msr_engine::EV_RING || e->ev_count[3] >= msr_engine::EV_RING) return nullptr;
    ev[0] = e->ev_start[3][e->ev_count[3]]; ev[1] = e->ev_stop[3][e->ev_count[3]];
    ev[2] = e->ev_start[kind][e->ev_count[kind]]; ev[3] = e->ev_stop[kind][e->ev_count[kind]];
    return ev;
}
static void pass_events_used(msr_engine* e, int kind, const hipEvent_t* ev) {
    if (ev) { e->ev_count[kind]++; e->ev_count[3]++; }
}

extern "C" int msr_dense_split_max(const msr_engine* e, int32_t k) {
    if (!e || !e->have_chunks || k < 1 || k > e->cfg.max_k || !dense_stream_ok(e, k)) return 0;
    return dense_stream_cap(e);
}

extern "C" int msr_dense_topk_begin(msr_engine* e, const float* q, int32_t n_queries, int32_t k, int32_t k_part, float* out_part,
                                    void* stream) {
    if (!e) return MSR_ERR_INVALID;
    if (!e->have_chunks) return fail(e, MSR_ERR_NOT_BOUND, "msr_dense_topk_begin: chunks not bound");
    if (e->split_pending) return fail(e, MSR_ERR_INVALID, "msr_dense_topk_begin: the previous begin has not been ended");
    const int cap = msr_dense_split_max(e, k);
    if (!q || !out_part || k_part < 1 || k_part > k || n_queries <= 64 || n_queries > cap)
        return fail(e, MSR_ERR_INVALID, "msr_dense_topk_begin: needs 64 < n_queries <= msr_dense_split_max() = %d, 1 <= k_part <= k (got %d, %d, %d)",
                    cap, n_queries, k_part, k);
    hipStream_t st = (hipStream_t)stream;
    HIP_TRY(e, hipSetDevice(e->cfg.device));
    HIP_TRY(e, msr_prep_queries(q, n_queries, e->gf_qn, (n_queries + 63) / 64 * 64, st));
    HIP_TRY(e, hipMemsetAsync(e->gf_gate, 0, GF_GATE_BYTES, st));
    hipEvent_t ev_buf[4];
    hipEvent_t* ev = pass_events(e, 0, ev_buf);
    int width = 0;
    HIP_TRY(e, msr_gemm_f32_pass(e->gf, e->dense, e->gf_qn, n_queries, k, k_part, out_part, ev, &width, st));
    e->last_dense_width = width;
    pass_events_used(e, 0, ev);
    e->split_pending = n_queries;
    return MSR_OK;
}

extern "C" int msr_dense_topk_end(msr_engine* e, int32_t n_queries, int32_t k, const float* bound, int32_t* out_doc,
                                  float* out_score, int32_t* out_chunk, int32_t* out_n, void* stream) {
    if (!e) return MSR_ERR_INVALID;
    if (!e->have_chunks) return fail(e, MSR_ERR_NOT_BOUND, "msr_dense_topk_end: chunks not bound");
    if (!e->gf_ok || e->split_pending != n_queries || n_queries <= 0)
        return fail(e, MSR_ERR_INVALID, "msr_dense_topk_end: no matching msr_dense_topk_begin (pending %d, got %d)", e->split_pending, n_queries);
    if (!out_doc || !out_score || !out_n || k < 1 || k > e->cfg.max_k) return fail(e, MSR_ERR_INVALID, "msr_dense_topk_end: bad argument");
    e->split_pending = 0;
    hipStream_t st = (hipStream_t)stream;
    HIP_TRY(e, hipSetDevice(e->cfg.device));
    HIP_TRY(e, msr_gemm_f32_finish(e->gf, e->dense, e->gf_qn, n_queries, k, bound, out_doc, out_score, out_chunk, out_n, e->gf_gate, st));
    return dense_gated_fallback(e, n_queries, k, out_doc, out_score, out_chunk, out_n, st);
}

static int dense_sweeps(msr_engine* e, const float* q, int q0, int cnt, int k, int max_chunks_per_doc, bool wide, const int32_t* gate,
                        int32_t* out_doc, float* out_score, int32_t* out_chunk, int32_t* out_n, hipStream_t st,
                        const MsrSetView* set) {
    const int64_t N = e->dense.n_docs;
    const int slice = wide ? 64 : 32;
    DenseIndex ix = e->dense;
    SelScratch sel = e->sel;
    for (int s0 = q0; s0 < q0 + cnt; s0 += slice) {
        const int nq = std::min(slice, q0 + cnt - s0);
        ix.gate = sel.gate = gate ? gate + (s0 - q0) / 64 : nullptr;
        const int nq_pad = nq > 32 ? 64 : (nq > 16 || (wide && e->dense.variant >= 14)) ? 32 : 16;
        const bool timed = !gate && e->timing && e->ev_count[0] < msr_engine::EV_RING;
        HIP_TRY(e, msr_prep_queries(q + (int64_t)s0 * MSR_DIM, nq, e->qn, nq_pad, st));
        if (timed) HIP_TRY(e, hipEventRecord(e->ev_start[0][e->ev_count[0]], st));
        HIP_TRY(e, msr_dense_scan(ix, e->qn, nq, max_chunks_per_doc, (float*)e->score_rows, st));
        if (timed) {
            HIP_TRY(e, hipEventRecord(e->ev_stop[0][e->ev_count[0]], st));
            e->ev_count[0]++;
        }
        if (set) {
            MsrSetView sv = *set;
            sv.q_set += s0;
            HIP_TRY(e, msr_select_topk_within((const float*)e->score_rows, N, e->dense.score_stride, nq, k, sel, sv,
                                              out_doc + (int64_t)s0 * k, out_score + (int64_t)s0 * k, out_n + s0, st));
        } else {
            HIP_TRY(e, msr_select_topk(32, e->score_rows, N, e->dense.score_stride, nq, k, sel, out_doc + (int64_t)s0 * k,
                                       out_score + (int64_t)s0 * k, out_n + s0, st));
        }
        if (out_chunk)
            HIP_TRY(e, msr_best_chunk(ix, e->qn, nq, k, max_chunks_per_doc, out_doc + (int64_t)s0 * k,
                                      out_n + s0, out_chunk + (int64_t)s0 * k, st));
    }
    return MSR_OK;
}

extern "C" int msr_dense_topk(msr_engine* e, const float* q, int32_t n_queries, int32_t k, int32_t max_chunks_per_doc,
                              int32_t* out_doc, float* out_score, int32_t* out_chunk, int32_t* out_n, void* stream) {
    if (!e) return MSR_ERR_INVALID;
    if (!e->have_chunks) return fail(e, MSR_ERR_NOT_BOUND, "msr_dense_topk: chunks not bound");
    if (e->split_pending)
        return fail(e, MSR_ERR_INVALID, "msr_dense_topk: an msr_dense_topk_begin is pending (its scratch is in use): call msr_dense_topk_end first");
    if (n_queries < 0 || k < 1 || k > e->cfg.max_k || max_chunks_per_doc < 0 || !q || !out_doc || !out_score || !out_n)
        return fail(e, MSR_ERR_INVALID, "msr_dense_topk: bad argument (k=%d, max_k=%d)", k, e->cfg.max_k);
    if (n_queries == 0) return MSR_OK;
    hipStream_t st = (hipStream_t)stream;
    HIP_TRY(e, hipSetDevice(e->cfg.device));
    const bool wide = dense_sweep_wide(e, max_chunks_per_doc);
    const bool gemm = wide && dense_stream_ok(e, k);
    e->last_dense_width = gemm && n_queries > 64 ? 0 : (wide ? 64 : 32);
    int q0 = 0;
    while (q0 < n_queries) {
        const int left = n_queries - q0;
        if (gemm && left > 64) {
            const int nq = std::min(dense_stream_cap(e), left);
            HIP_TRY(e, msr_prep_queries(q + (int64_t)q0 * MSR_DIM, nq, e->gf_qn, (nq + 63) / 64 * 64, st));
            HIP_TRY(e, hipMemsetAsync(e->gf_gate, 0, GF_GATE_BYTES, st));
            hipEvent_t ev_buf[4];
            hipEvent_t* ev = pass_events(e, 0, ev_buf);
            int width = 0;
            HIP_TRY(e, msr_gemm_f32_topk(e->gf, e->dense, e->gf_qn, nq, k, out_doc + (int64_t)q0 * k,
                                         out_score + (int64_t)q0 * k, out_chunk ? out_chunk + (int64_t)q0 * k : nullptr,
                                         out_n + q0, e->gf_gate, ev, &width, st));
            e->last_dense_width = std::max(e->last_dense_width, width);
            pass_events_used(e, 0, ev);
            {
                int rcf = dense_gated_fallback(e, nq, k, out_doc + (int64_t)q0 * k, out_score + (int64_t)q0 * k,
                                               out_chunk ? out_chunk + (int64_t)q0 * k : nullptr, out_n + q0, st);
                if (rcf) return rcf;
            }
            q0 += nq;
        } else {
            const int nq = std::min(wide ? 64 : 32, left);
            int rc = dense_sweeps(e, q, q0, nq, k, max_chunks_per_doc, wide, nullptr, out_doc, out_score, out_chunk, out_n, st,
                                  nullptr);
            if (rc) return rc;
            q0 += nq;
        }
    }
    return MSR_OK;
}

extern "C" int msr_dense_topk_within(msr_engine* e, const float* q, int32_t n_queries, int32_t k, int32_t max_chunks_per_doc,
                                     const uint32_t* set_bits, int32_t n_sets, int64_t set_stride, const int32_t* q_set,
                                     int32_t* out_doc, float* out_score, int32_t* out_chunk, int32_t* out_n, void* stream) {
    if (!e) return MSR_ERR_INVALID;
    if (!e->have_chunks) return fail(e, MSR_ERR_NOT_BOUND, "msr_dense_topk_within: chunks not bound");
    if (e->split_pending)
        return fail(e, MSR_ERR_INVALID, "msr_dense_topk_within: an msr_dense_topk_begin is pending (its scratch is in use): call msr_dense_topk_end first");
    if (n_queries < 0 || k < 1 || k > e->cfg.max_k || max_chunks_per_doc < 0 || !q || !out_doc || !out_score || !out_n)
        return fail(e, MSR_ERR_INVALID, "msr_dense_topk_within: bad argument (k=%d, max_k=%d)", k, e->cfg.max_k);
    {
        const int rc = within_args_ok(e, "msr_dense_topk_within", e->dense.n_docs, set_bits, n_sets, set_stride, q_set);
        if (rc) return rc;
    }
    if (n_sets == 0)
        return msr_dense_topk(e, q, n_queries, k, max_chunks_per_doc, out_doc, out_score, out_chunk, out_n, stream);
    if (n_queries == 0) return MSR_OK;
    hipStream_t st = (hipStream_t)stream;
    HIP_TRY(e, hipSetDevice(e->cfg.device));
    const bool wide = dense_sweep_wide(e, max_chunks_per_doc);
    e->last_dense_width = wide ? 64 : 32;
    const MsrSetView set{set_bits, set_stride, q_set, n_sets};
    return dense_sweeps(e, q, 0, n_queries, k, max_chunks_per_doc, wide, nullptr, out_doc, out_score, out_chunk, out_n, st, &set);
}

static int sim_out_of_range(msr_engine* e, const int32_t* v, int64_t n, int64_t hi, hipStream_t st) {
    if (!e->sim_flag) ALLOC(e, e->mem_engine, e->sim_flag, 64);
    int32_t flag = 0;
    HIP_TRY(e, hipMemsetAsync(e->sim_flag, 0, sizeof(int32_t), st));
    HIP_TRY(e, msr_check_range(v, n, hi, e->sim_flag, st));
    HIP_TRY(e, hipMemcpyAsync(&flag, e->sim_flag, sizeof(int32_t), hipMemcpyDeviceToHost, st));
    HIP_TRY(e, hipStreamSynchronize(st));
    return flag ? 1 : 0;
}

extern "C" int msr_gather_rows(msr_engine* e, const int32_t* rows, int32_t n, float* out, void* stream) {
    if (!e) return MSR_ERR_INVALID;
    if (!e->have_chunks) return fail(e, MSR_ERR_NOT_BOUND, "msr_gather_rows: chunks not bound");
    if (n < 0 || (n > 0 && (!rows || !out))) return fail(e, MSR_ERR_INVALID, "msr_gather_rows: bad argument (n=%d)", n);
    if (n == 0) return MSR_OK;
    hipStream_t st = (hipStream_t)stream;
    HIP_TRY(e, hipSetDevice(e->cfg.device));
    const int bad = sim_out_of_range(e, rows, n, e->dense.n_chunks, st);
    if (bad < 0) return bad;
    if (bad) return fail(e, MSR_ERR_INVALID, "msr_gather_rows: a row lies outside [0, n_chunks = %lld)", (long long)e->dense.n_chunks);
    HIP_TRY(e, msr_gather_rows_run(e->dense, rows, n, out, st));
    return MSR_OK;
}

extern "C" int msr_dense_topk_grouped(msr_engine* e, const float* q, int32_t n_rows, const int32_t* group_off, int32_t n_groups,
                                      const int32_t* excl_off, const int32_t* excl_doc, int32_t k, float min_score,
                                      const uint32_t* set_bits, int32_t n_sets, int64_t set_stride, const int32_t* g_set,
                                      int32_t* out_doc, float* out_score, int32_t* out_chunk, int32_t* out_src_row,
                                      int32_t* out_n, void* stream) {
    static const char* fn = "msr_dense_topk_grouped";
    if (!e) return MSR_ERR_INVALID;
    if (!e->have_chunks) return fail(e, MSR_ERR_NOT_BOUND, "%s: chunks not bound", fn);
    if (e->split_pending)
        return fail(e, MSR_ERR_INVALID, "%s: an msr_dense_topk_begin is pending (its scratch is in use): call msr_dense_topk_end first", fn);
    if (n_rows < 0 || n_groups < 0 || k < 1 || k > e->cfg.max_k || min_score != min_score || !group_off || !excl_off ||
        (n_rows > 0 && !q) || (n_groups > 0 && (!out_doc || !out_score || !out_chunk || !out_src_row || !out_n)))
        return fail(e, MSR_ERR_INVALID, "%s: bad argument (n_rows=%d, n_groups=%d, k=%d, max_k=%d)", fn, n_rows, n_groups, k,
                    e->cfg.max_k);
    {
        const int rc = within_args_ok(e, fn, e->dense.n_docs, set_bits, n_sets, set_stride, g_set);
        if (rc) return rc;
    }
    hipStream_t st = (hipStream_t)stream;
    HIP_TRY(e, hipSetDevice(e->cfg.device));
    std::vector<int32_t> h_goff((size_t)n_groups + 1), h_eoff((size_t)n_groups + 1);
    HIP_TRY(e, hipMemcpyAsync(h_goff.data(), group_off, h_goff.size() * sizeof(int32_t), hipMemcpyDeviceToHost, st));
    HIP_TRY(e, hipMemcpyAsync(h_eoff.data(), excl_off, h_eoff.size() * sizeof(int32_t), hipMemcpyDeviceToHost, st));
    HIP_TRY(e, hipStreamSynchronize(st));
    if (h_goff[0] != 0 || h_goff[n_groups] != n_rows)
        return fail(e, MSR_ERR_INVALID, "%s: group_off must run from 0 to n_rows = %d (got %d .. %d)", fn, n_rows, h_goff[0],
                    h_goff[n_groups]);
    if (h_eoff[0] != 0) return fail(e, MSR_ERR_INVALID, "%s: excl_off[0] = %d, must be 0", fn, h_eoff[0]);
    int max_excl = 0;
    for (int g = 0; g < n_groups; ++g) {
        if (h_goff[g + 1] < h_goff[g]) return fail(e, MSR_ERR_INVALID, "%s: group_off not monotone at group %d", fn, g);
        if (h_eoff[g + 1] < h_eoff[g]) return fail(e, MSR_ERR_INVALID, "%s: excl_off not monotone at group %d", fn, g);
        max_excl = std::max(max_excl, h_eoff[g + 1] - h_eoff[g]);
    }
    if ((int64_t)k + max_excl > e->cfg.max_k)
        return fail(e, MSR_ERR_INVALID, "%s: k + max |excl_g| = %lld exceeds max_k = %d", fn, (long long)k + max_excl, e->cfg.max_k);
    const int64_t n_excl = h_eoff[n_groups];
    if (n_excl > 0) {
        if (!excl_doc) return fail(e, MSR_ERR_INVALID, "%s: excl_doc is NULL with %lld exclusions", fn, (long long)n_excl);
        const int bad = sim_out_of_range(e, excl_doc, n_excl, e->dense.n_docs, st);
        if (bad < 0) return bad;
        if (bad) return fail(e, MSR_ERR_INVALID, "%s: an excluded document lies outside [0, n_docs = %lld)", fn, (long long)e->dense.n_docs);
    }
    if (n_groups == 0) return MSR_OK;
    const int kk = k + max_excl;
    const size_t L = (size_t)n_rows * kk;
    const size_t lists_bytes = (L * 3 + 2 * (size_t)n_rows + 64) * 4;
    int rc = grow(e, e->mem_engine, &e->sim_lists, &e->sim_lists_bytes, lists_bytes, "grouped lists");
    if (rc) return rc;
    rc = grow(e, e->mem_engine, &e->sim_over, &e->sim_over_bytes, 2 * L * 16 + 64, "grouped merge records");
    if (rc) return rc;
    int32_t* l_doc = (int32_t*)e->sim_lists;
    float* l_score = (float*)(l_doc + L);
    int32_t* l_chunk = (int32_t*)(l_score + L);
    int32_t* l_n = l_chunk + L;
    int32_t* row_set = l_n + n_rows;
    if (n_sets > 0) HIP_TRY(e, msr_group_row_sets(group_off, n_groups, g_set, row_set, st));
    for (int r0 = 0; r0 < n_rows; r0 += e->cfg.max_queries) {
        const int cnt = std::min(e->cfg.max_queries, n_rows - r0);
        const int64_t o = (int64_t)r0 * kk;
        rc = msr_dense_topk_within(e, q + (int64_t)r0 * MSR_DIM, cnt, kk, 0, set_bits, n_sets, set_stride,
                                   n_sets > 0 ? row_set + r0 : nullptr, l_doc + o, l_score + o, l_chunk + o, l_n + r0, stream);
        if (rc) return rc;
    }
    GroupedMergeArgs a{};
    a.l_doc = l_doc; a.l_score = l_score; a.l_chunk = l_chunk; a.l_n = l_n; a.kk = kk;
    a.group_off = group_off; a.excl_off = excl_off; a.excl_doc = excl_doc; a.k = k; a.min_score = min_score;
    a.out_doc = out_doc; a.out_score = out_score; a.out_chunk = out_chunk; a.out_src = out_src_row; a.out_n = out_n;
    a.g_hi = (uint64_t*)e->sim_over;
    a.g_lo = (uint32_t*)(a.g_hi + 2 * L);
    a.g_val = a.g_lo + 2 * L;
    HIP_TRY(e, msr_grouped_merge(a, n_groups, st));
    return MSR_OK;
}

static int rerank_args_ok(msr_engine* e, const char* fn, int32_t n_queries, int32_t max_cand, int32_t max_chunks) {
    if (n_queries < 0 || max_cand < 1 || max_cand > e->cfg.rerank_max_docs)
        return fail(e, MSR_ERR_INVALID, "%s: bad argument (max_cand=%d, rerank_max_docs=%d)", fn, max_cand,
                    e->cfg.rerank_max_docs);
    if (max_chunks < 1 || max_chunks > MSR_RERANK_MAX_CHUNKS)
        return fail(e, MSR_ERR_INVALID, "%s: max_chunks out of range [1, %d]", fn, MSR_RERANK_MAX_CHUNKS);
    return MSR_OK;
}

static constexpr int BT_SLICE = 128;
static constexpr int GM_SLICE = 1024;
static constexpr int GM_WV_CAP = 16384;

static int build_bf16(msr_engine* e, hipStream_t st) {
    const int64_t C = e->dense.n_chunks;
    const int64_t n_pad = C + 512;
    ALLOC(e, e->mem_bf16, e->emb_bf16, (size_t)n_pad * MSR_DIM * 2);
    const size_t QS = GM_SLICE;
    if (!e->bt_top_doc) ALLOC(e, e->mem_engine, e->bt_top_doc, (size_t)BT_SLICE * MSR_MAX_K * 4);
    if (!e->bt_top_score) ALLOC(e, e->mem_engine, e->bt_top_score, (size_t)BT_SLICE * MSR_MAX_K * 4);
    if (!e->bt_top_n) ALLOC(e, e->mem_engine, e->bt_top_n, (size_t)BT_SLICE * 4);
    if (!e->bt_cand_doc) ALLOC(e, e->mem_engine, e->bt_cand_doc, QS * MSR_SEL_CAP * 4);
    if (!e->bt_cand_score) ALLOC(e, e->mem_engine, e->bt_cand_score, QS * MSR_SEL_CAP * 4);
    if (!e->bt_cand_chunk) ALLOC(e, e->mem_engine, e->bt_cand_chunk, QS * MSR_SEL_CAP * 4);
    if (!e->bt_cand_n) ALLOC(e, e->mem_engine, e->bt_cand_n, QS * 4);
    ALLOC(e, e->mem_bf16, e->bf_ones, (size_t)C * 4);
    ALLOC(e, e->mem_bf16, e->bf_err, 4);
    ALLOC(e, e->mem_bf16, e->bf_margin, QS * 4);
    HIP_TRY(e, hipMemsetAsync(e->bt_cand_n, 0, QS * 4, st));
    HIP_TRY(e, msr_unit_bf16_rows(e->dense.emb, e->dense.inv_norm, C, n_pad, e->emb_bf16, e->bf_err, st));
    HIP_TRY(e, msr_fill_f32(e->bf_ones, C, 1.0f, st));
    e->dense.emb_bf16 = e->emb_bf16;
    e->dense_bf16 = e->dense;
    e->dense_bf16.inv_norm = e->bf_ones;
    if (e->dense.wide_ok) {
        ALLOC(e, e->mem_bf16, e->bf_row_meta, (size_t)(C + 16) * 8);
        HIP_TRY(e, msr_pack_row_meta(e->chunk_doc, e->bf_ones, C, e->bf_row_meta, st));
        e->dense_bf16.row_meta = e->bf_row_meta;
    }
    const int n_tiles = e->n_tiles;
    const int grid = e->n_cus / 8 * 8;
    if (e->tiles_ok && n_tiles >= 64 && grid >= 32) {
        const int stride = (n_tiles + 31) / 32 * 32;
        GemmIndex& g = e->gemm;
        g.emb_n = e->emb_bf16; g.tile_row = e->tile_row; g.n_tiles = n_tiles; g.n_cus = e->n_cus; g.max_queries = GM_SLICE;
        g.tmax_stride = stride; g.wv_cap = GM_WV_CAP;
        ALLOC(e, e->mem_bf16, g.qmat, (size_t)GM_SLICE * MSR_DIM * 2);
        ALLOC(e, e->mem_bf16, e->gm_qn, (size_t)GM_SLICE * MSR_DIM * 4);
        ALLOC(e, e->mem_bf16, g.tmax, (size_t)GM_SLICE * stride * 4);
        ALLOC(e, e->mem_bf16, g.tmax_t, (size_t)n_tiles * 2 * GM_SLICE * 4);
// ... 285 lines not shown
```

modern-search-engines-project_amd/csrc/msr_gemm.hip:

```cpp
#include <type_traits>

#include "msr_common.h"
#include "msr_internal.h"
#include "msr_frag.h"
#include "msr_gemm_dev.h"

namespace {


__global__ __launch_bounds__(256) void unit_bf16_rows_kernel(const float* __restrict__ src, const float* __restrict__ inv_norm,
                                                              int64_t n_rows, int64_t n_pad, bf16x8* __restrict__ dst,
                                                              uint32_t* __restrict__ err_max) {
    const int lane = threadIdx.x & 63;
    const int64_t wave = (int64_t)blockIdx.x * 4 + (threadIdx.x >> 6), n_waves = (int64_t)gridDim.x * 4;
    float worst = 0.f;
    for (int64_t r = wave; r < n_pad; r += n_waves) {
        float ss = 0.f;
#pragma unroll
        for (int h = 0; h < 2; ++h) {
            const int c = lane + 64 * h;
            if (c >= MSR_DIM / 8) continue;
            bf16x8 v;
            if (r < n_rows) {
                const float sc = inv_norm ? inv_norm[r] : 1.0f;
                const f32x4 x = ((const f32x4*)(src + (size_t)r * MSR_DIM))[2 * c], y = ((const f32x4*)(src + (size_t)r * MSR_DIM))[2 * c + 1];
                const float u[8] = {x.x * sc, x.y * sc, x.z * sc, x.w * sc, y.x * sc, y.y * sc, y.z * sc, y.w * sc};
#pragma unroll
                for (int j = 0; j < 8; ++j) {
                    v[j] = (__bf16)u[j];
                    const float d = (float)v[j] - u[j];
                    ss += d * d;
                }
            } else {
#pragma unroll
                for (int j = 0; j < 8; ++j) v[j] = (__bf16)0.f;
            }
            dst[(size_t)r * (MSR_DIM / 8) + c] = v;
        }
        for (int o = 32; o > 0; o >>= 1) ss += __shfl_xor(ss, o);
        worst = fmaxf(worst, ss);
    }
    if (lane == 0 && err_max) atomicMax(err_max, __float_as_uint(sqrtf(worst)));
}

__global__ __launch_bounds__(256) void batch_margin_kernel(const float* __restrict__ qn, int nq, const uint32_t* __restrict__ err_max,
                                                            float* __restrict__ margin) {
    const int q = blockIdx.x * 4 + (threadIdx.x >> 6), lane = threadIdx.x & 63;
    if (q >= nq) return;
    float ss = 0.f;
    for (int j = lane; j < MSR_DIM; j += 64) {
        const float x = qn[(size_t)q * MSR_DIM + j];
        const float d = (float)(__bf16)x - x;
        ss += d * d;
    }
    for (int o = 32; o > 0; o >>= 1) ss += __shfl_xor(ss, o);
    if (lane == 0) {
        const float dq = sqrtf(ss) * 1.0001f, dE = __uint_as_float(*err_max) * 1.0001f;
        margin[q] = 2.0f * (dE * (1.0f + dq) + dq * 1.000001f) + 1.0e-4f;
    }
}

template <int PARTS>
__global__ __launch_bounds__(256) void gemm_tmax_kernel(const float* __restrict__ in, int n_j, int parts, int nq_pad,
                                                         float* __restrict__ out, int out_stride) {
    __shared__ __attribute__((aligned(16))) float t[32][132];
    const int j0 = blockIdx.x * 32, q0 = blockIdx.y * 128;
    const int tx = threadIdx.x & 31, ty = threadIdx.x >> 5;
    const float ninf = -__builtin_inff();
    const size_t step = (size_t)nq_pad / 4;
#pragma unroll
    for (int h = 0; h < 2; ++h) {
        const f32x4* src[2];
#pragma unroll
        for (int r = 0; r < 2; ++r) {
            const int j = j0 + ty + 8 * (2 * h + r);
            const int jc = j < n_j ? j : n_j - 1;
            src[r] = (const f32x4*)(in + (size_t)jc * parts * nq_pad + q0) + tx;
        }
        f32x4 v[2] = {{ninf, ninf, ninf, ninf}, {ninf, ninf, ninf, ninf}};
        if constexpr (PARTS > 0) {
            f32x4 x[2][PARTS];
#pragma unroll
            for (int r = 0; r < 2; ++r)
#pragma unroll
                for (int p = 0; p < PARTS; ++p) x[r][p] = src[r][p * step];
#pragma unroll
            for (int r = 0; r < 2; ++r)
#pragma unroll
                for (int p = 0; p < PARTS; ++p) {
                    v[r].x = fmaxf(v[r].x, x[r][p].x); v[r].y = fmaxf(v[r].y, x[r][p].y);
                    v[r].z = fmaxf(v[r].z, x[r][p].z); v[r].w = fmaxf(v[r].w, x[r][p].w);
                }
        } else {
            for (int p = 0; p < parts; ++p) {
#pragma unroll
                for (int r = 0; r < 2; ++r) {
                    const f32x4 x = src[r][p * step];
                    v[r].x = fmaxf(v[r].x, x.x); v[r].y = fmaxf(v[r].y, x.y); v[r].z = fmaxf(v[r].z, x.z); v[r].w = fmaxf(v[r].w, x.w);
                }
            }
        }
#pragma unroll
        for (int r = 0; r < 2; ++r) *(f32x4*)&t[ty + 8 * (2 * h + r)][4 * tx] = v[r];
    }
    __syncthreads();
    const int j = j0 + tx;
    if (j < n_j) {
#pragma unroll
        for (int r = 0; r < 4; ++r) {
            const int ql = 4 * (ty + 8 * r);
            const f32x4 v = *(const f32x4*)&t[tx][ql];
            float* o = out + (size_t)(q0 + ql) * out_stride + j;
            o[0] = v.x; o[(size_t)out_stride] = v.y; o[2 * (size_t)out_stride] = v.z; o[3 * (size_t)out_stride] = v.w;
        }
    }
}

__global__ __launch_bounds__(1024) void gemm_kth_kernel(const float* __restrict__ tmax, int n, int stride, int nq, int k,
                                                         const float* __restrict__ margin, float* __restrict__ thr,
                                                         int32_t* __restrict__ flag, float short_val, float margin_scale) {
    __shared__ uint32_t hist[2048];
    __shared__ uint32_t wsum[16];
    __shared__ uint32_t s_bin, s_kk, s_hit;
    const int q = blockIdx.x, t = threadIdx.x, lane = t & 63, wave = t >> 6;
    if (q >= nq) {
        if (t == 0) { thr[q] = short_val; if (flag) flag[q] = 0; }
        return;
    }
    const float* row = tmax + (size_t)q * stride;
    uint32_t prefix = 0, mask = 0, kk = (uint32_t)k;
    bool short_row = false;
#pragma unroll 1
    for (int pass = 0; pass < 3; ++pass) {
        const int shift = pass == 0 ? 21 : pass == 1 ? 10 : 0;
        const uint32_t nb = pass == 2 ? 1024u : 2048u;
        hist[t] = 0; hist[t + 1024] = 0;
        if (t == 0) s_hit = 0;
        __syncthreads();
        for (int i = t; i < n; i += 1024) {
            const float x = row[i];
            if (!msr_valid(x)) continue;
            const uint32_t key = msr_ord32(x);
            if ((key & mask) == prefix) atomicAdd(&hist[(key >> shift) & (nb - 1)], 1u);
        }
        __syncthreads();
        const uint32_t h0 = 2 * t < (int)nb ? hist[2 * t] : 0u, h1 = 2 * t + 1 < (int)nb ? hist[2 * t + 1] : 0u;
        const uint32_t c2 = h0 + h1;
        uint32_t inc = c2;
#pragma unroll
        for (int o = 1; o < 64; o <<= 1) {
            const uint32_t v = __shfl_down(inc, o);
            if (lane + o < 64) inc += v;
        }
        if (lane == 0) wsum[wave] = inc;
        __syncthreads();
        uint32_t above = inc - c2;
        for (int w2 = wave + 1; w2 < 16; ++w2) above += wsum[w2];
        if (above < kk && kk <= above + c2) {
            if (above + h1 >= kk) { s_bin = 2 * t + 1; s_kk = kk - above; }
            else { s_bin = 2 * t; s_kk = kk - above - h1; }
            s_hit = 1;
        }
        __syncthreads();
        if (!s_hit) { short_row = true; break; }
        prefix |= s_bin << shift;
        mask |= (nb - 1) << shift;
        kk = s_kk;
        __syncthreads();
    }
    if (t == 0) {
        thr[q] = short_row ? short_val : msr_unord32(prefix) - (margin ? margin_scale * margin[q] : 0.0f);
        if (flag) flag[q] = short_row ? 1 : 0;
    }
}


__global__ __launch_bounds__(256) void gemm_bucket_kernel(const int4* __restrict__ wgbuf, int wg_cap,
                                                           const int32_t* __restrict__ wg_count,
                                                           const float* __restrict__ thr2, int2* __restrict__ pairs,
                                                           int pair_cap, int32_t* __restrict__ pair_n) {
    const int wg = blockIdx.y;
    int n = wg_count[wg];
    if (n > wg_cap) n = wg_cap;
    for (int i = blockIdx.x * 256 + threadIdx.x; i < n; i += gridDim.x * 256) {
        const int4 e = wgbuf[(size_t)wg * wg_cap + i];
        if (__int_as_float(e.z) >= thr2[e.y]) {
            const int pos = atomicAdd(&pair_n[e.y], 1);
            if (pos < pair_cap) pairs[(size_t)e.y * pair_cap + pos] = make_int2(e.x, e.z);
        }
    }
}

constexpr int GM_PAIR_CAP = 4096;
static_assert(GM_PAIR_CAP <= (1 << 13), "cand_first_len packs first and len into 13 bits each");
__global__ __launch_bounds__(1024) void gemm_cand_kernel(int2* __restrict__ pairs, int32_t* __restrict__ pair_n,
                                                          const int32_t* __restrict__ chunk_doc, int64_t n_rows,
                                                          const int32_t* __restrict__ wg_count, int n_wg, int wg_cap,
                                                          const int32_t* __restrict__ flag, int k,
                                                          const float* __restrict__ margin,
                                                          int32_t* __restrict__ cand_doc, int32_t* __restrict__ cand_first_len,
                                                          int32_t* __restrict__ cand_n) {
    __shared__ uint64_t key[GM_PAIR_CAP];
    __shared__ uint32_t pay[GM_PAIR_CAP];
    __shared__ int s_heads, s_over;
    const int q = blockIdx.x, t = threadIdx.x;
    const int raw = pair_n[q];
    int over = raw > GM_PAIR_CAP || (flag && flag[q]);
    for (int i = t; i < n_wg; i += 1024) over |= wg_count[i] > wg_cap;
    if (t == 0) s_heads = 0;
    s_over = 0;
    __syncthreads();
    if (over) s_over = 1;
    __syncthreads();
    if (s_over) {
        if (t == 0) { cand_n[q] = MSR_SEL_CAP + 1; pair_n[q] = 0; }
        return;
    }
    int P = 64;
    while (P < raw) P <<= 1;
    auto sort_desc = [&]() {
        for (int kk = 2; kk <= P; kk <<= 1)
            for (int j = kk >> 1; j > 0; j >>= 1) {
                for (int idx = t; idx < (P >> 1); idx += 1024) {
                    const int i = ((idx & ~(j - 1)) << 1) | (idx & (j - 1));
                    const int p = i | j;
                    const bool desc = (i & kk) == 0;
                    const uint64_t x = key[i], y = key[p];
                    if (desc ? x < y : x > y) {
                        key[i] = y; key[p] = x;
                        const uint32_t v = pay[i]; pay[i] = pay[p]; pay[p] = v;
                    }
                }
                __syncthreads();
            }
    };
    for (int i = t; i < P; i += 1024) {
        uint64_t kk = 0;
        uint32_t row = 0;
        if (i < raw) {
            const int2 e = pairs[(size_t)q * GM_PAIR_CAP + i];
            if (e.x >= 0 && e.x < n_rows) {
                kk = ((uint64_t)(uint32_t)(chunk_doc[e.x] + 1) << 32) | msr_ord32(__int_as_float(e.y));
                row = (uint32_t)e.x;
            }
        }
        key[i] = kk; pay[i] = row;
    }
    __syncthreads();
    sort_desc();
    uint64_t mine[GM_PAIR_CAP / 1024];
    uint32_t mine_run[GM_PAIR_CAP / 1024];
#pragma unroll
    for (int u = 0; u < GM_PAIR_CAP / 1024; ++u) {
        const int i = t + u * 1024;
        uint64_t kk = 0;
        uint32_t run = 0;
        if (i < P && key[i] != 0) {
            pairs[(size_t)q * GM_PAIR_CAP + i].x = (int32_t)pay[i];
            const uint32_t d = (uint32_t)(key[i] >> 32);
            if (i == 0 || (uint32_t)(key[i - 1] >> 32) != d) {
                kk = ((uint64_t)(uint32_t)key[i] << 32) | (uint32_t)~(uint32_t)(d - 1);
                int len = 1;
                while (i + len < P && (uint32_t)(key[i + len] >> 32) == d) ++len;
                run = (uint32_t)i | ((uint32_t)len << 13);
            }
        }
        mine[u] = kk; mine_run[u] = run;
    }
    __syncthreads();
#pragma unroll
    for (int u = 0; u < GM_PAIR_CAP / 1024; ++u) {
        const int i = t + u * 1024;
        if (i < P) {
            key[i] = mine[u]; pay[i] = mine_run[u];
            if (mine[u]) atomicAdd(&s_heads, 1);
        }
    }
    __syncthreads();
    sort_desc();
    const int heads = s_heads;
    const float tk = heads >= k ? msr_unord32((uint32_t)(key[k - 1] >> 32)) : -__builtin_inff();
    const float cut = tk - margin[q];
    __shared__ int s_keep;
    if (t == 0) s_keep = 0;
    __syncthreads();
    for (int i = t; i < heads; i += 1024)
        if (msr_unord32((uint32_t)(key[i] >> 32)) >= cut) {
            atomicAdd(&s_keep, 1);
            if (i < MSR_SEL_CAP) {
                cand_doc[(size_t)q * MSR_SEL_CAP + i] = (int32_t)~(uint32_t)key[i];
                cand_first_len[(size_t)q * MSR_SEL_CAP + i] = (int32_t)pay[i];
            }
        }
    __syncthreads();
    if (t == 0) { cand_n[q] = s_keep; pair_n[q] = 0; }
}

int g_gemm_dbg = 0;

}

hipError_t msr_unit_bf16_rows(const float* src, const float* inv_norm, int64_t n_rows, int64_t n_pad, void* dst,
                              uint32_t* err_max, hipStream_t stream) {
    if (n_pad <= 0) return hipSuccess;
    hipError_t err = err_max ? hipMemsetAsync(err_max, 0, 4, stream) : hipSuccess;
    if (err != hipSuccess) return err;
    unit_bf16_rows_kernel<<<8192, 256, 0, stream>>>(src, inv_norm, n_rows, n_pad, (bf16x8*)dst, err_max);
    return hipGetLastError();
}

hipError_t msr_batch_margin(const float* qn, int nq, const uint32_t* err_max, float* margin, hipStream_t stream) {
    if (nq <= 0) return hipSuccess;
    batch_margin_kernel<<<(nq + 3) / 4, 256, 0, stream>>>(qn, nq, err_max, margin);
    return hipGetLastError();
}

int msr_gemm_pair_cap() { return GM_PAIR_CAP; }

hipError_t msr_gemm_tmax(const float* tmax_t, int n_j, int parts, int nq_pad, float* out, int out_stride, hipStream_t stream) {
    if (n_j <= 0 || nq_pad <= 0) return hipSuccess;
    if (parts <= 0 || nq_pad % 128 != 0) return hipErrorInvalidValue;
    const dim3 grid((n_j + 31) / 32, nq_pad / 128);
    if (parts == 8) gemm_tmax_kernel<8><<<grid, 256, 0, stream>>>(tmax_t, n_j, parts, nq_pad, out, out_stride);
    else if (parts == 1) gemm_tmax_kernel<1><<<grid, 256, 0, stream>>>(tmax_t, n_j, parts, nq_pad, out, out_stride);
    else gemm_tmax_kernel<0><<<grid, 256, 0, stream>>>(tmax_t, n_j, parts, nq_pad, out, out_stride);
    return hipGetLastError();
}
hipError_t msr_gemm_kth(const float* tmax, int n, int stride, int nq, int nq_pad, int k, const float* margin, float* thr,
                        int32_t* flag, hipStream_t stream, float short_val, float margin_scale) {
    if (nq_pad <= 0) return hipSuccess;
    gemm_kth_kernel<<<nq_pad, 1024, 0, stream>>>(tmax, n, stride, nq, k, margin, thr, flag, short_val, margin_scale);
    return hipGetLastError();
}
hipError_t msr_gemm_bucket(const void* wvbuf, int wv_cap, const int32_t* wv_count, int n_waves, const float* thr2,
                           void* pairs, int32_t* pair_n, hipStream_t stream) {
    gemm_bucket_kernel<<<dim3(2, (unsigned)n_waves), 256, 0, stream>>>((const int4*)wvbuf, wv_cap, wv_count, thr2, (int2*)pairs,
                                                                      GM_PAIR_CAP, pair_n);
    return hipGetLastError();
}
void msr_gemm_set_dbg(int v) { g_gemm_dbg = v; }

hipError_t msr_gemm_candidates(const GemmIndex& g, const DenseIndex& ix, const float* qn, int nq, int k, const float* margin,
                               int32_t* cand_doc, int32_t* cand_first_len, int32_t* cand_n, hipEvent_t* ev, hipStream_t stream) {
    const int nq_pad = (nq + 255) / 256 * 256;
    const int nt = nq_pad / 256;
    if (nq <= 0 || nq_pad > g.max_queries || k < 1 || g.n_tiles < 2 * k) return hipErrorInvalidValue;
    const int grid = g.n_cus / 8 * 8;
    if (grid < 8 || grid / 8 < nt) return hipErrorInvalidValue;
    hipError_t err;
    int ss = g.n_tiles / (8 * k);
    ss = ss < 1 ? 1 : (ss > 16 ? 16 : ss);
#ifdef MSR_DIAG
    if (g_gemm_dbg & 256) ss = 1;
#endif
    const int n_s = (g.n_tiles - ss / 2 + ss - 1) / ss;
    {
        if ((err = msr_stream256_bf16_qimage(qn, nq, nt, g.qmat, stream)) != hipSuccess) return err;
        StreamArgs a{};
        a.E = (const char*)g.emb_n; a.inv_pad = nullptr; a.qimg = (const char*)g.qmat; a.tile_row = g.tile_row;
        a.n_rows = ix.n_chunks; a.tmax_t = g.tmax_t; a.nt = nt; a.q_base = 0; a.append = 0;
        a.t_first = ss / 2; a.t_stride = ss; a.t_count = n_s;
        if (ev && (err = hipEventRecord(ev[0], stream)) != hipSuccess) return err;
        if ((err = msr_stream256_bf16_launch(false, a, grid, stream)) != hipSuccess) return err;
        if (ev && (err = hipEventRecord(ev[1], stream)) != hipSuccess) return err;
        if ((err = msr_gemm_tmax(g.tmax_t, n_s, 1, nq_pad, (float*)g.tmax, g.tmax_stride, stream)) != hipSuccess) return err;
        gemm_kth_kernel<<<nq_pad, 1024, 0, stream>>>((const float*)g.tmax, n_s, g.tmax_stride, nq, k, margin, g.thr, g.flag, __builtin_inff(), 1.0f);
        a.t_first = 0; a.t_stride = 1; a.t_count = g.n_tiles;
        a.thr = g.thr; a.wvbuf = g.wgbuf; a.wv_cap = g.wv_cap; a.wv_count = g.wv_count;
        if (ev && (err = hipEventRecord(ev[2], stream)) != hipSuccess) return err;
        if ((err = msr_stream256_bf16_launch(true, a, grid, stream)) != hipSuccess) return err;
        if (ev && (err = hipEventRecord(ev[3], stream)) != hipSuccess) return err;
        if ((err = msr_gemm_tmax(g.tmax_t, g.n_tiles, 1, nq_pad, (float*)g.tmax, g.tmax_stride, stream)) != hipSuccess) return err;
        gemm_kth_kernel<<<nq_pad, 1024, 0, stream>>>((const float*)g.tmax, g.n_tiles, g.tmax_stride, nq, k, margin, g.thr2, nullptr, __builtin_inff(), 1.0f);
    }
    gemm_bucket_kernel<<<dim3(2, (unsigned)grid * 8), 256, 0, stream>>>((const int4*)g.wgbuf, g.wv_cap, g.wv_count, g.thr2,
                                                                       (int2*)g.pairs, GM_PAIR_CAP, g.pair_n);
    gemm_cand_kernel<<<nq, 1024, 0, stream>>>((int2*)g.pairs, g.pair_n, ix.chunk_doc, ix.n_chunks, g.wv_count, grid * 8, g.wv_cap,
                                              g.flag, k, margin, cand_doc, cand_first_len, cand_n);
    return hipGetLastError();
}
```

modern-search-engines-project_amd/csrc/msr_gemm_f32.hip:

```cpp
#include <type_traits>

#include "msr_common.h"
#include "msr_internal.h"
#include "msr_frag.h"
#include "msr_gemm_dev.h"

namespace {

constexpr int GF_THREADS = 512;
constexpr int GF_KT = MSR_DIM / 32;
constexpr int GF_ROWB = MSR_DIM * 4;
constexpr int GF_PAIR_CAP = 4096;

typedef StreamArgs GemmF32Args;

__device__ __forceinline__ const char* uniform_ptr(const char* p) {
    const uint64_t u = (uint64_t)p;
    const uint32_t lo = __builtin_amdgcn_readfirstlane((uint32_t)u), hi = __builtin_amdgcn_readfirstlane((uint32_t)(u >> 32));
    return (const char*)(((uint64_t)hi << 32) | lo);
}

constexpr int GS_NB = 8;
constexpr int GS_STEP = 8192;
constexpr int GS_BLK = GS_NB * GS_STEP;
constexpr int GS_LDS = 2 * GS_BLK;
constexpr int GS_D = 4;

typedef const __attribute__((address_space(1))) char* gptr;
template <int OFF>
__device__ __forceinline__ void gload16(f32x4& r, gptr p) {
    asm volatile("global_load_dwordx4 %0, %1, off offset:%2" : "=v"(r) : "v"(p), "n"(OFF) : "memory");
}
__device__ __forceinline__ void pin4(f32x4& a, f32x4& b, f32x4& c, f32x4& d) { asm volatile("" : "+v"(a), "+v"(b), "+v"(c), "+v"(d)); }
__device__ __forceinline__ void pin2(f32x4& a, f32x4& b) { asm volatile("" : "+v"(a), "+v"(b)); }

template <bool EMIT>
__global__ __launch_bounds__(GF_THREADS) void gemm_stream_kernel(GemmF32Args a) {
    extern __shared__ __attribute__((aligned(16))) char smem[];
    const int tid = threadIdx.x, lane = tid & 63;
    const int w = __builtin_amdgcn_readfirstlane(tid >> 6);
    const int li16 = lane & 15, lg = lane >> 4;
    const int G = (int)gridDim.x, gid = (int)blockIdx.x;
    int wave_cnt = EMIT && a.append ? __builtin_amdgcn_readfirstlane(a.wv_count[blockIdx.x * 8 + w]) : 0;
    int4* wvbuf = EMIT ? (int4*)a.wvbuf + ((size_t)blockIdx.x * 8 + w) * a.wv_cap : nullptr;
    if (gid >= a.t_count) {
        if (EMIT && lane == 0) a.wv_count[blockIdx.x * 8 + w] = wave_cnt;
        return;
    }
    const int n_mine = (a.t_count - gid + G - 1) / G;
#ifdef MSR_DIAG
    const int dbg = a.dbg;
#else
    constexpr int dbg = 0;
#endif
    const uint32_t foffB = (uint32_t)(li16 * 64 + ((lg ^ (((li16 >> 3) & 1) << 1)) << 4));
    auto stage_b = [&](int blk, int pb) {
        const char* base = uniform_ptr(a.qimg + (size_t)blk * GS_BLK + (size_t)w * 8192);
#pragma unroll
        for (int i = 0; i < 8; ++i)
            __builtin_amdgcn_global_load_lds((glb_void*)(base + (uint32_t)(i * 1024 + lane * 16)),
                                             (lds_void*)(smem + pb * GS_BLK + w * 8192 + i * 1024), 16, 0, 0);
    };

    float thrv[8];
#pragma unroll
    for (int ni = 0; ni < 8; ++ni) thrv[ni] = EMIT ? a.thr[ni * 16 + li16] : 0.f;

    f32x4 acc[2][8];
#pragma unroll
    for (int mi = 0; mi < 2; ++mi)
#pragma unroll
        for (int ni = 0; ni < 8; ++ni) acc[mi][ni] = (f32x4){0.f, 0.f, 0.f, 0.f};

    auto tile_of = [&](int j) { return a.t_first + j * a.t_stride; };
    auto row_ptr = [&](int row0, int mi) -> gptr {
        int64_t r = (int64_t)row0 + 32 * w + 16 * mi + li16;
        if (r > a.n_rows - 1) r = a.n_rows - 1;
        return (gptr)a.E + (size_t)r * GF_ROWB + lg * 32;
    };
    int jt = gid;
    int row0 = a.tile_row[tile_of(jt)], row_end = a.tile_row[tile_of(jt) + 1];
    int jn = jt + G < a.t_count ? jt + G : jt;
    int row0n = a.tile_row[tile_of(jn)];
    gptr rp0 = row_ptr(row0, 0), rp1 = row_ptr(row0, 1);
    gptr rn0 = row_ptr(row0n, 0), rn1 = row_ptr(row0n, 1);
    const __attribute__((address_space(1))) float* invp = (const __attribute__((address_space(1))) float*)a.inv_pad + w * 32 + 4 * lg;

    f32x4 ring[GS_D][2][2];
    auto load_rows = [&](auto slot_c, gptr p0, gptr p1, auto off_c) {
        constexpr int slot = decltype(slot_c)::value, off = decltype(off_c)::value;
        if (dbg & 4) return;
        gload16<off>(ring[slot][0][0], p0);
        gload16<off + 16>(ring[slot][0][1], p0);
        gload16<off>(ring[slot][1][0], p1);
        gload16<off + 16>(ring[slot][1][1], p1);
    };
    auto pin_rows = [&](auto slot_c) {
        constexpr int slot = decltype(slot_c)::value;
        pin4(ring[slot][0][0], ring[slot][0][1], ring[slot][1][0], ring[slot][1][1]);
    };
    stage_b(0, 0);
#pragma unroll
    for (int s = 0; s < GS_D; ++s)
#pragma unroll
        for (int mi = 0; mi < 2; ++mi) ring[s][mi][0] = ring[s][mi][1] = (f32x4){0.f, 0.f, 0.f, 0.f};
    load_rows(std::integral_constant<int, 0>{}, rp0, rp1, std::integral_constant<int, 0>{});
    load_rows(std::integral_constant<int, 1>{}, rp0, rp1, std::integral_constant<int, 128>{});
    load_rows(std::integral_constant<int, 2>{}, rp0, rp1, std::integral_constant<int, 256>{});
    load_rows(std::integral_constant<int, 3>{}, rp0, rp1, std::integral_constant<int, 384>{});
    wait_vm0();
    pin_rows(std::integral_constant<int, 0>{}); pin_rows(std::integral_constant<int, 1>{});
    pin_rows(std::integral_constant<int, 2>{}); pin_rows(std::integral_constant<int, 3>{});
    wg_barrier();
    int pb = 0;

    f32x4 inv4[2];
    inv4[0] = inv4[1] = (f32x4){1.f, 1.f, 1.f, 1.f};
    const float NEG_INF = -__builtin_inff();
    auto step = [&](auto s8_c, int b3, bool last) {
        constexpr int s8 = decltype(s8_c)::value, slot = s8 % GS_D;
        using SL = std::integral_constant<int, slot>;
        __builtin_amdgcn_sched_barrier(0);
        if (s8 < GS_D) {
            if (b3 == 0) asm volatile("s_waitcnt vmcnt(28)" ::: "memory");
            else asm volatile("s_waitcnt vmcnt(20)" ::: "memory");
        } else {
            asm volatile("s_waitcnt vmcnt(12)" ::: "memory");
        }
        pin_rows(SL{});
        f16x8 af[2];
#pragma unroll
        for (int mi = 0; mi < 2; ++mi) af[mi] = cvt_f16_rtn(ring[slot][mi][0], ring[slot][mi][1]);
        asm volatile("" :: "v"(af[0]), "v"(af[1]));
        if (s8 == GS_NB - 3 && last && !(dbg & 64)) {
#pragma unroll
            for (int mi = 0; mi < 2; ++mi) {
                const __attribute__((address_space(1))) float* p = invp + (size_t)row0 + mi * 16;
                gload16<0>(inv4[mi], (gptr)p);
            }
        }
        if (s8 < GS_NB - GS_D) {
            load_rows(SL{}, rp0 + b3 * (GS_NB * 128), rp1 + b3 * (GS_NB * 128), std::integral_constant<int, (s8 + GS_D) * 128>{});
        } else {
            gptr q0 = last ? rn0 : rp0 + (b3 + 1) * (GS_NB * 128), q1 = last ? rn1 : rp1 + (b3 + 1) * (GS_NB * 128);
            load_rows(SL{}, q0, q1, std::integral_constant<int, (s8 + GS_D - GS_NB) * 128>{});
        }
        __builtin_amdgcn_sched_barrier(0);
        const char* bq = smem + pb * GS_BLK + s8 * GS_STEP + foffB;
#pragma unroll
        for (int n4 = 0; n4 < 2; ++n4) {
            f16x8 bh[4] = {};
            if (!(dbg & 16)) {
// ... 606 lines not shown
            if (row >= 0 && row < n_rows)
                kk = ((uint64_t)((uint32_t)chunk_doc[row] + 1u) << 32) | (uint32_t)row;
        }
        key[i] = kk;
    }
    __syncthreads();
    for (int kk = 2; kk <= P; kk <<= 1)
        for (int j = kk >> 1; j > 0; j >>= 1) {
            for (int idx = t; idx < (P >> 1); idx += 1024) {
                const int i = ((idx & ~(j - 1)) << 1) | (idx & (j - 1));
                const int p = i | j;
                const bool desc = (i & kk) == 0;
                const uint64_t a = key[i], b = key[p];
                if (desc ? a < b : a > b) { key[i] = b; key[p] = a; }
            }
            __syncthreads();
        }
    for (int i = t; i < P; i += 1024) {
        const uint64_t kk = key[i];
        if (kk == 0) continue;
        pairs[(size_t)q * GF_PAIR_CAP + i].x = (int32_t)(uint32_t)kk;
        const uint32_t d = (uint32_t)(kk >> 32);
        if (i == 0 || (uint32_t)(key[i - 1] >> 32) != d) {
            int len = 1;
            while (i + len < P && (uint32_t)(key[i + len] >> 32) == d) ++len;
            const int slot = atomicAdd(&s_n, 1);
            cand_doc[(size_t)q * MSR_SEL_CAP + slot] = (int32_t)(d - 1u);
            cand_first_len[(size_t)q * MSR_SEL_CAP + slot] = i | (len << 13);
        }
    }
    __syncthreads();
    if (t == 0) { cand_n[q] = s_n; pair_n[q] = 0; }
}

int g_f32_dbg = 0;

template <bool EMIT>
hipError_t launch_stream_t(const GemmF32Args& a, int grid, hipStream_t stream) {
    static bool attr_done = false;
    if (!attr_done) {
        hipError_t err = hipFuncSetAttribute((const void*)gemm_stream_kernel<EMIT>, hipFuncAttributeMaxDynamicSharedMemorySize, GS_LDS);
        if (err != hipSuccess) return err;
        attr_done = true;
    }
    gemm_stream_kernel<EMIT><<<grid, GF_THREADS, GS_LDS, stream>>>(a);
    return hipGetLastError();
}
template <bool EMIT, bool BF16, bool TILED = false, bool NTL = false, bool F16I = false>
hipError_t launch_stream256_t(const GemmF32Args& a, int grid, hipStream_t stream) {
    static bool attr_done = false;
    if (!attr_done) {
        hipError_t err = hipFuncSetAttribute((const void*)gemm_stream256_kernel<EMIT, BF16, TILED, NTL, F16I>, hipFuncAttributeMaxDynamicSharedMemorySize, G2_LDS);
        if (err != hipSuccess) return err;
        attr_done = true;
    }
    gemm_stream256_kernel<EMIT, BF16, TILED, NTL, F16I><<<grid, G2_THREADS, G2_LDS, stream>>>(a);
    return hipGetLastError();
}

__global__ __launch_bounds__(256) void f16_rows_kernel(const float* __restrict__ src, int64_t n_rows, int64_t n_pad,
                                                        f16x8* __restrict__ dst) {
    const int64_t n8 = n_pad * (MSR_DIM / 8), stride = (int64_t)gridDim.x * 256;
    for (int64_t i = (int64_t)blockIdx.x * 256 + threadIdx.x; i < n8; i += stride) {
        const int64_t r = i / (MSR_DIM / 8);
        f16x8 h;
        if (r < n_rows) {
            const float* p = src + i * 8;
            h = cvt_f16_rtn(*(const f32x4*)p, *(const f32x4*)(p + 4));
        } else {
#pragma unroll
            for (int j = 0; j < 8; ++j) h[j] = (_Float16)0.f;
        }
        dst[i] = h;
    }
}

template <int ROWB>
__global__ __launch_bounds__(256) void tile_rows_kernel(const char* __restrict__ E, const int32_t* __restrict__ tile_row,
                                                         const int32_t* __restrict__ tile_trow, f32x4* __restrict__ Et) {
    constexpr int SLOTS = ROWB / 128;
    const int t_ = blockIdx.x;
    const int row0 = tile_row[t_], n = tile_row[t_ + 1] - row0;
    const int groups = (n + 15) >> 4;
    f32x4* dst = Et + (size_t)tile_trow[t_] * (ROWB / 16);
    const int pieces = groups * SLOTS * 128;
    for (int i = threadIdx.x; i < pieces; i += 256) {
        const int lane = i & 63, half = (i >> 6) & 1, sl = (i >> 7) % SLOTS, g = i / (128 * SLOTS);
        const int lr = 16 * g + (lane & 15);
        f32x4 v = {0.f, 0.f, 0.f, 0.f};
        if (lr < n) v = *(const f32x4*)(E + (size_t)(row0 + lr) * ROWB + 128 * sl + 32 * (lane >> 4) + 16 * half);
        dst[i] = v;
    }
}
hipError_t launch_f32(int width, bool emit, const GemmF32Args& a, int grid, hipStream_t stream, bool tiled = false,
                      bool image16 = false) {
    if (image16)
        return emit ? launch_stream256_t<true, true, false, false, true>(a, grid, stream)
                    : launch_stream256_t<false, true, false, false, true>(a, grid, stream);
    bool ntl = width == 256 && tiled && a.nt == 1;
#ifdef MSR_DIAG
    if (g_f32_dbg & 16384) ntl = false;
#endif
    if (ntl)
        return emit ? launch_stream256_t<true, false, true, true>(a, grid, stream) : launch_stream256_t<false, false, true, true>(a, grid, stream);
    if (width == 256 && tiled)
        return emit ? launch_stream256_t<true, false, true>(a, grid, stream) : launch_stream256_t<false, false, true>(a, grid, stream);
    if (width == 256) return emit ? launch_stream256_t<true, false>(a, grid, stream) : launch_stream256_t<false, false>(a, grid, stream);
    return emit ? launch_stream_t<true>(a, grid, stream) : launch_stream_t<false>(a, grid, stream);
}

}

void msr_gemm_f32_set_dbg(int v) { g_f32_dbg = v; }

hipError_t msr_stream256_bf16_launch(bool emit, const StreamArgs& a, int grid, hipStream_t stream) {
    if (a.nt < 1 || (grid & 7) || (grid >> 3) < a.nt) return hipErrorInvalidValue;
#ifdef MSR_DIAG
    if (g_f32_dbg & (32768 | 65536 | 131072 | 262144 | 524288)) { StreamArgs b = a; b.dbg |= g_f32_dbg & (32768 | 65536 | 131072 | 262144 | 524288); return emit ? launch_stream256_t<true, true>(b, grid, stream) : launch_stream256_t<false, true>(b, grid, stream); }
#endif
    return emit ? launch_stream256_t<true, true>(a, grid, stream) : launch_stream256_t<false, true>(a, grid, stream);
}
hipError_t msr_stream256_bf16_qimage(const float* qn, int nq, int n_groups, void* qimg, hipStream_t stream) {
    build_qimg2_kernel<true><<<dim3((GF_KT * 256 * 4 + 255) / 256, n_groups), 256, 0, stream>>>(qn, nq, (f16x8*)qimg);
    return hipGetLastError();
}

hipError_t msr_tile_rows(const float* emb, const int32_t* tile_row, const int32_t* tile_trow, int n_tiles, void* emb_tiled,
                         hipStream_t stream) {
    if (n_tiles <= 0) return hipSuccess;
    tile_rows_kernel<MSR_DIM * 4><<<n_tiles, 256, 0, stream>>>((const char*)emb, tile_row, tile_trow, (f32x4*)emb_tiled);
    return hipGetLastError();
}


hipError_t msr_f16_rows(const float* emb, int64_t n_rows, int64_t n_pad, void* out, hipStream_t stream) {
    if (n_pad <= 0) return hipSuccess;
    f16_rows_kernel<<<8192, 256, 0, stream>>>(emb, n_rows, n_pad, (f16x8*)out);
    return hipGetLastError();
}

hipError_t msr_pad_inv_norm(const float* inv, int64_t n, int64_t n_pad, float* out, hipStream_t stream) {
    if (n_pad <= 0) return hipSuccess;
    pad_inv_kernel<<<(unsigned)((n_pad + 255) / 256), 256, 0, stream>>>(inv, n, n_pad, out);
    return hipGetLastError();
}

hipError_t msr_f16_row_error(const float* emb, const float* inv_norm, int64_t n_rows, uint32_t* err_max, hipStream_t stream) {
    hipError_t err = hipMemsetAsync(err_max, 0, 4, stream);
    if (err != hipSuccess) return err;
    f16_row_error_kernel<<<8192, 256, 0, stream>>>(emb, inv_norm, n_rows, err_max);
    return hipGetLastError();
}

hipError_t msr_gemm_f32_pass(const GemmF32Index& g, const DenseIndex& ix, const float* qn, int nq, int k, int k_part,
                             float* out_part, hipEvent_t* ev, int* width_out, hipStream_t stream) {
    const int W = nq > 128 ? 256 : 128;
    const int waves = 8;
    const int G = (nq + W - 1) / W;
    if (nq <= 0 || G * W > 128 * g.max_groups || k < 1 || g.n_tiles < 2 * k) return hipErrorInvalidValue;
    if (width_out) *width_out = W;
    hipError_t err;
    int NT0 = 1;
    if (W == 256 && (g.n_cus & 7) == 0) NT0 = std::min(std::min(G, g.max_nt), g.n_cus >> 3);
    bool image16 = W == 256 && NT0 > 1 && g.emb_f16 != nullptr;
#ifdef MSR_DIAG
    if (g_f32_dbg & (2048 | 1048576)) image16 = false;
#endif
    if (image16) build_qimg2_kernel<true, false><<<dim3((GF_KT * 256 * 4 + 255) / 256, G), 256, 0, stream>>>(qn, nq, (f16x8*)g.qimg);
    else if (W == 256) build_qimg2_kernel<false><<<dim3((GF_KT * 256 * 4 + 255) / 256, G), 256, 0, stream>>>(qn, nq, (f16x8*)g.qimg);
    else build_qimg1_kernel<<<dim3((GF_KT * 128 * 4 + 255) / 256, G), 256, 0, stream>>>(qn, nq, (f16x8*)g.qimg);
    f16_margin_kernel<<<(nq + 3) / 4, 256, 0, stream>>>(qn, nq, g.err_max, g.margin);
    const float* margin = g.margin;
    int ss = g.n_tiles / (3 * k);
    ss = ss < 1 ? 1 : (ss > 64 ? 64 : ss);
    const int n_s = (g.n_tiles - ss / 2 + ss - 1) / ss;
    const int grid = g.n_cus;
    const size_t qimg_bytes = (size_t)GF_KT * W * 64;
    int NT = 1;
    if (W == 256 && (grid & 7) == 0) NT = std::min(std::min(G, g.max_nt), grid >> 3);
#ifdef MSR_DIAG
    if (g_f32_dbg & 2048) NT = 1;
    if (g_f32_dbg & 4096) NT = std::min(NT, 2);
#endif
    GemmF32Args a{};
    a.dbg = g_f32_dbg; a.nt = 1;
    a.E = (const char*)ix.emb; a.inv_pad = g.inv_pad; a.tile_row = g.tile_row;
    bool tiled = W == 256 && g.emb_tiled != nullptr && !image16;
#ifdef MSR_DIAG
    if (g_f32_dbg & 8192) tiled = false;
#endif
    if (tiled) { a.E = (const char*)g.emb_tiled; a.tile_trow = g.tile_trow; }
    if (image16) a.E = (const char*)g.emb_f16;
    const int tmax_parts = image16 ? 1 : waves;
    a.n_rows = ix.n_chunks; a.tmax_t = g.tmax_t;
    a.t_first = ss / 2; a.t_stride = ss; a.t_count = n_s;
    for (int gi = 0; gi < G; gi += NT) {
        a.nt = std::min(NT, G - gi);
        a.qimg = (const char*)g.qimg + gi * qimg_bytes;
        if (ev && gi == 0 && (err = hipEventRecord(ev[0], stream)) != hipSuccess) return err;
        if ((err = launch_f32(W, false, a, grid, stream, tiled, image16)) != hipSuccess) return err;
        if (ev && gi == 0 && (err = hipEventRecord(ev[1], stream)) != hipSuccess) return err;
        if ((err = msr_gemm_tmax(g.tmax_t, n_s, tmax_parts, W * a.nt, g.tmax + (size_t)gi * W * g.tmax_stride, g.tmax_stride, stream)) != hipSuccess) return err;
    }
    if ((err = msr_gemm_kth(g.tmax, n_s, g.tmax_stride, nq, W * G, k, margin, g.thr, g.flag, stream)) != hipSuccess) return err;
    a.t_first = 0; a.t_stride = 1; a.t_count = g.n_tiles;
    a.wvbuf = g.wvbuf; a.wv_cap = g.wv_cap * (8 / waves); a.wv_count = g.wv_count;
    for (int gi = 0; gi < G; gi += NT) {
        a.nt = std::min(NT, G - gi);
        a.qimg = (const char*)g.qimg + gi * qimg_bytes;
        a.thr = g.thr + gi * W; a.q_base = gi * W; a.append = gi > 0;
        if (ev && gi == 0 && (err = hipEventRecord(ev[2], stream)) != hipSuccess) return err;
        if ((err = launch_f32(W, true, a, grid, stream, tiled, image16)) != hipSuccess) return err;
        if (ev && gi == 0 && (err = hipEventRecord(ev[3], stream)) != hipSuccess) return err;
        if ((err = msr_gemm_tmax(g.tmax_t, g.n_tiles, tmax_parts, W * a.nt, g.tmax + (size_t)gi * W * g.tmax_stride, g.tmax_stride, stream)) != hipSuccess) return err;
    }
    if ((err = msr_gemm_kth(g.tmax, g.n_tiles, g.tmax_stride, nq, W * G, k, margin, g.thr2, nullptr, stream)) != hipSuccess) return err;
    if (out_part && (err = msr_gemm_kth(g.tmax, g.n_tiles, g.tmax_stride, nq, nq, k_part, margin, out_part, nullptr, stream,
                                        -__builtin_inff(), 0.5f)) != hipSuccess) return err;
    return hipSuccess;
}

namespace {
__global__ __launch_bounds__(256) void raise_thr_kernel(float* __restrict__ thr2, const float* __restrict__ bound,
                                                         const float* __restrict__ margin, int nq) {
    const int q = blockIdx.x * 256 + threadIdx.x;
    if (q >= nq) return;
    const float b = bound[q] - 0.5f * margin[q];
    if (b > thr2[q]) thr2[q] = b;
}
}

hipError_t msr_gemm_f32_finish(const GemmF32Index& g, const DenseIndex& ix, const float* qn, int nq, int k, const float* bound,
                               int32_t* out_doc, float* out_score, int32_t* out_chunk, int32_t* out_n, int32_t* gate,
                               hipStream_t stream) {
    const int waves = 8, grid = g.n_cus;
    const int wv_cap = g.wv_cap * (8 / waves);
    if (nq <= 0 || k < 1) return hipErrorInvalidValue;
    hipError_t err;
    if (bound) {
        raise_thr_kernel<<<(nq + 255) / 256, 256, 0, stream>>>(g.thr2, bound, g.margin, nq);
        if ((err = hipGetLastError()) != hipSuccess) return err;
    }
    if ((err = msr_gemm_bucket(g.wvbuf, wv_cap, g.wv_count, grid * waves, g.thr2, g.pairs, g.pair_n, stream)) != hipSuccess) return err;
    gemm_f32_cand_kernel<<<nq, 1024, 0, stream>>>((int2*)g.pairs, g.pair_n, ix.chunk_doc, ix.n_chunks, g.wv_count, grid * waves,
                                                  wv_cap, g.flag, g.cand_doc, g.cand_chunk, g.cand_n, gate);
    if ((err = hipGetLastError()) != hipSuccess) return err;
    return msr_batch_rescore_rows(ix, qn, nq, k, (const int32_t*)g.pairs, 2, GF_PAIR_CAP, g.cand_doc, g.cand_score, g.cand_chunk,
                                  g.cand_n, out_doc, out_score, out_chunk, out_n, stream);
}

hipError_t msr_gemm_f32_topk(const GemmF32Index& g, const DenseIndex& ix, const float* qn, int nq, int k,
                             int32_t* out_doc, float* out_score, int32_t* out_chunk,
                             int32_t* out_n, int32_t* gate, hipEvent_t* ev, int* width_out, hipStream_t stream) {
    hipError_t err = msr_gemm_f32_pass(g, ix, qn, nq, k, k, nullptr, ev, width_out, stream);
    if (err != hipSuccess) return err;
    return msr_gemm_f32_finish(g, ix, qn, nq, k, nullptr, out_doc, out_score, out_chunk, out_n, gate, stream);
}
```

modern-search-engines-project_amd/csrc/msr_internal.h:

```cpp
#pragma once
#include <hip/hip_runtime.h>
#include <stdint.h>

#define MSR_DIM 768
#define MSR_SEL_BINS 4096
#define MSR_SEL_CAP 4096

struct SelState {
    uint64_t pref_hi, mask_hi;
    uint32_t pref_lo, mask_lo;
    int32_t k_rem;
    int32_t n_above;
    int32_t done;
    int32_t n_sel;
};

struct SelScratch {
    uint32_t* hist;
    SelState* state;
    uint64_t* cand_hi;
    uint32_t* cand_lo;
    int32_t* cand_n;
    const int32_t* gate;
    int gate_per64;
// ... 96 lines not shown
                             int64_t base_stride, const int32_t* row_base, uint32_t* out_bits, int64_t out_stride,
                             hipStream_t stream);

hipError_t msr_tokens_validate(const int64_t* tok_off, const int32_t* tok_ids, int64_t n_docs, int64_t n_tokens, int64_t n_terms,
                               int32_t* flag, hipStream_t stream);
hipError_t msr_phrase_sets_run(const int64_t* tok_off, const int32_t* tok_ids, int64_t n_docs, int64_t n_terms, int n_rows,
                               const int32_t* phrase_off, const int32_t* phrase_terms, const uint32_t* cand_bits, int n_cand,
                               int64_t cand_stride, const int32_t* row_cand, uint32_t* out_bits, int64_t out_stride,
                               hipStream_t stream);
hipError_t msr_proximity_sets_run(const int64_t* tok_off, const int32_t* tok_ids, int64_t n_docs, int64_t n_terms, int n_rows,
                                  const int32_t* phrase_off, const int32_t* phrase_terms, const int32_t* row_span,
                                  const int32_t* row_ordered, const uint32_t* cand_bits, int n_cand, int64_t cand_stride,
                                  const int32_t* row_cand, uint32_t* out_bits, int64_t out_stride, hipStream_t stream);
hipError_t msr_best_windows_run(const int64_t* tok_off, const int32_t* tok_ids, int64_t n_docs, int64_t n_terms, int n_pairs,
                                const int32_t* pair_doc, const int32_t* pair_row, int n_rows, const int32_t* row_off,
                                const int32_t* row_terms, const int32_t* row_weights, const int32_t* row_span, int32_t* out_start,
                                int32_t* out_cover, int32_t* out_hits, uint64_t* out_mask, uint32_t* out_terms,
                                hipStream_t stream);
hipError_t msr_vocab_validate(const int64_t* char_off, const uint32_t* weight, int64_t n_terms, int64_t n_chars, int32_t* flag,
                              hipStream_t stream);
hipError_t msr_vocab_signatures(const int64_t* char_off, const uint16_t* chars, int64_t n_terms, uint64_t* sig,
                                hipStream_t stream);
int64_t msr_fuzzy_spans(int64_t n_terms);
hipError_t msr_fuzzy_terms_run(const int64_t* char_off, const uint16_t* chars, const uint32_t* weight, const uint64_t* sig,
                               int64_t n_terms, int n_words, const int32_t* word_off, const uint16_t* word_chars,
                               const int32_t* word_max, int limit, int32_t* out_term, int32_t* out_dist, int32_t* out_n,
                               int32_t* out_total, void* scratch, hipStream_t stream);
hipError_t msr_combine_sets_run(int64_t n_docs, int n_rows, const int32_t* and_off, const int32_t* and_rows,
                                const int32_t* not_off, const int32_t* not_rows, const uint32_t* in_bits, int n_in,
                                int64_t in_stride, uint32_t* out_bits, int64_t out_stride, hipStream_t stream);

hipError_t msr_bm25_validate(const Bm25Index& ix, int32_t* flag, hipStream_t stream);

constexpr int MSR_WIDE_RING = 128;
struct DenseIndex {
    const float* emb;
    const int32_t* doc_off;
    const int32_t* chunk_doc;
    const float* inv_norm;
    const int32_t* span_doc;
    int64_t n_chunks, n_docs;
    int64_t score_stride;
    int32_t n_spans;
    int32_t layout;
    const int32_t* wspan_doc;
    int32_t n_wspans;
    const int32_t* wspan12_doc;
    int32_t n_wspans12;
    void* qimg;
    const void* emb_bf16;
    const void* emb_presplit;
    const void* row_meta;
    int32_t wide_ok;
    int32_t wide_ok64;
    const int32_t* gate;
    int32_t variant;
    int32_t gate_per64;
};
hipError_t msr_dense_scan(const DenseIndex& ix, const float* qn, int nq, int max_chunks, float* docscore,
                          hipStream_t stream);
hipError_t msr_dense_scan_bf16(const DenseIndex& ix, const float* qn, int nq, int max_chunks, float* docscore,
                               hipStream_t stream);
hipError_t msr_dense_scan_wide(const DenseIndex& ix, const float* qn, int nq, float* docscore, hipStream_t stream);
size_t msr_ksplit_slice_image_bytes();
hipError_t msr_dense_scan_slices(const DenseIndex& ix, const float* qn, int nq, float* docscore, void* qimg_slices,
                                 hipStream_t stream);
hipError_t msr_dense_scan_wide_exact(const DenseIndex& ix, const float* qn, int nq, float* docscore, hipStream_t stream);
hipError_t msr_dense_scan_bf16_wide(const DenseIndex& ix, const float* qn, int nq, float* docscore,
                                    hipStream_t stream);
hipError_t msr_build_qimage(int mode, const float* qn, int n_blocks, void* qimg, hipStream_t stream);
hipError_t msr_presplit_rows(const float* src, int64_t n_rows, void* dst, hipStream_t stream);
hipError_t msr_pack_row_meta(const int32_t* chunk_doc, const float* inv_norm, int64_t n, void* row_meta, hipStream_t stream);
hipError_t msr_fill_f32(float* dst, int64_t n, float value, hipStream_t stream);
hipError_t msr_inv_norm_range(const float* inv_norm, int64_t n, uint32_t* out2, hipStream_t stream);
hipError_t msr_prep_queries(const float* q, int nq, float* qn, int nq_pad, hipStream_t stream);
hipError_t msr_fill_chunk_doc(const int32_t* doc_off, int64_t n_docs, int32_t* chunk_doc, hipStream_t stream);
hipError_t msr_row_inv_norm(const float* emb, int64_t n_rows, float* inv_norm, hipStream_t stream);
hipError_t msr_interleave(const float* src, int64_t n_rows, float* dst, hipStream_t stream);
hipError_t msr_best_chunk(const DenseIndex& ix, const float* qn, int nq, int k, int max_chunks,
                          const int32_t* out_doc, const int32_t* out_n, int32_t* out_chunk, hipStream_t stream);

hipError_t msr_check_range(const int32_t* v, int64_t n, int64_t hi, int32_t* flag, hipStream_t stream);
hipError_t msr_gather_rows_run(const DenseIndex& ix, const int32_t* rows, int n, float* out, hipStream_t stream);
hipError_t msr_group_row_sets(const int32_t* group_off, int n_groups, const int32_t* g_set, int32_t* row_set, hipStream_t stream);
struct GroupedMergeArgs {
    const int32_t* l_doc; const float* l_score; const int32_t* l_chunk; const int32_t* l_n;
    int32_t kk;
    const int32_t* group_off;
    const int32_t* excl_off;
    const int32_t* excl_doc;
    int32_t k;
    float min_score;
    int32_t* out_doc; float* out_score; int32_t* out_chunk; int32_t* out_src; int32_t* out_n;
    uint64_t* g_hi; uint32_t* g_lo; uint32_t* g_val;
};
hipError_t msr_grouped_merge(const GroupedMergeArgs& a, int n_groups, hipStream_t stream);

struct RerankParams {
    double smoothing, max_boost, max_decay;
    int32_t max_chunks;
};
#define MSR_RERANK_RECORD_WORDS 16
struct RerankRecords {
    int32_t* out;
    const int32_t* q_base;
    const int32_t* blk_off;
    int64_t capacity;
    int q_first;
};
hipError_t msr_rerank_gather(const DenseIndex& ix, const int32_t* url_group, const float* qn, int nq,
                             const int32_t* cand_doc, const int32_t* cand_n, int max_cand, int doc_base,
                             int row_base, int max_chunks, float* cos_out ,
                             int32_t* meta , int q_per_block, int64_t block_stride,
                             const RerankRecords& rec, hipStream_t stream);
hipError_t msr_rerank_plan_run(int nq, const int32_t* cand_doc, const int32_t* cand_n, int max_cand, const int32_t* bounds,
                               int n_shards, int my, int qps, int32_t* counts, int32_t* send_base, int32_t* blk_off,
                               int32_t* recv_off, int32_t* pair, hipStream_t stream);
hipError_t msr_rerank_scatter_run(const int32_t* records, int64_t capacity, const int32_t* counts, const int32_t* recv_off, int n_shards, int nq,
                                  int qps, int q_first, int n_mine, int max_cand, float* cos_out, int32_t* meta_out,
                                  hipStream_t stream);
hipError_t msr_rerank_fuse_run(int nq, const int32_t* cand_doc, const double* cand_bm25, const int32_t* cand_n,
                               int max_cand, const RerankParams& p, const float* cos_in, const int32_t* meta,
                               int32_t* out_doc, double* out_score, double* out_orig, int32_t* out_chunk,
                               int32_t* out_n, int32_t* out_rows, hipStream_t stream);

hipError_t msr_diversify_run(int nq, const int32_t* f_doc, const double* f_score, const double* f_orig, const int32_t* f_chunk,
                             const int32_t* f_n, int max_cand, const int32_t* doc_domain, int64_t n_domain_docs, int top_k,
                             double threshold, int diversify, int32_t* out_doc, double* out_score, double* out_orig,
                             int32_t* out_chunk, int32_t* out_n, hipStream_t stream);

hipError_t msr_or_parts(const void* in, int n_parts, int64_t part_stride_bytes, int64_t n_words, void* out, hipStream_t stream);

struct GemmIndex {
    const void* emb_n;
    const int32_t* tile_row;
    int32_t n_tiles;
    int32_t n_cus;
    int32_t max_queries;
    void* qmat;
    float* tmax;
    int32_t tmax_stride;
    float* tmax_t;
    float* thr; float* thr2;
    int32_t* flag;
    void* wgbuf;
    int32_t wv_cap;
    int32_t* wv_count;
    void* pairs;
    int32_t* pair_n;
};
int msr_gemm_pair_cap();
hipError_t msr_gemm_tmax(const float* tmax_t, int n_j, int parts, int nq_pad, float* out, int out_stride, hipStream_t stream);
hipError_t msr_gemm_kth(const float* tmax, int n, int stride, int nq, int nq_pad, int k, const float* margin, float* thr,
                        int32_t* flag, hipStream_t stream, float short_val = __builtin_inff(), float margin_scale = 1.0f);
hipError_t msr_gemm_bucket(const void* wvbuf, int wv_cap, const int32_t* wv_count, int n_waves, const float* thr2,
                           void* pairs, int32_t* pair_n, hipStream_t stream);
void msr_bm25_set_dbg(int v);
void msr_gemm_set_dbg(int v);
hipError_t msr_unit_bf16_rows(const float* src, const float* inv_norm, int64_t n_rows, int64_t n_pad, void* dst,
                              uint32_t* err_max, hipStream_t stream);
hipError_t msr_batch_margin(const float* qn, int nq, const uint32_t* err_max, float* margin, hipStream_t stream);
hipError_t msr_gemm_candidates(const GemmIndex& g, const DenseIndex& ix, const float* qn, int nq, int k, const float* margin,
                               int32_t* cand_doc, int32_t* cand_first_len, int32_t* cand_n, hipEvent_t* ev,
                               hipStream_t stream);

constexpr int MSR_STREAM256_TILE_ROWS = 256;

struct StreamArgs {
    const char* E;
    const float* inv_pad;
    const char* qimg;
    const int32_t* tile_row;
    const int32_t* tile_trow;
    int64_t n_rows;
    int t_first, t_stride, t_count;
    float* tmax_t;
    const float* thr;
    void* wvbuf; int wv_cap; int32_t* wv_count;
    int q_base;
    int append;
    int nt;
    int dbg;
};
hipError_t msr_stream256_bf16_launch(bool emit, const StreamArgs& a, int grid, hipStream_t stream);
hipError_t msr_stream256_bf16_qimage(const float* qn, int nq, int n_groups, void* qimg, hipStream_t stream);

struct GemmF32Index {
    const int32_t* tile_row;
    int32_t n_tiles;
    int32_t n_cus;
    int32_t max_groups;
    const float* inv_pad;
    void* qimg;
    float* tmax_t;
    float* tmax;
    int32_t tmax_stride;
    float* thr; float* thr2; int32_t* flag;
    void* wvbuf; int32_t wv_cap; int32_t* wv_count;
    void* pairs; int32_t* pair_n;
    uint32_t* err_max; float* margin;
    int32_t* cand_doc; float* cand_score; int32_t* cand_chunk; int32_t* cand_n;
    int32_t max_nt;
    const void* emb_tiled;
    const int32_t* tile_trow;
    const void* emb_f16;
};
hipError_t msr_f16_rows(const float* emb, int64_t n_rows, int64_t n_pad, void* out, hipStream_t stream);
hipError_t msr_tile_rows(const float* emb, const int32_t* tile_row, const int32_t* tile_trow, int n_tiles, void* emb_tiled,
                         hipStream_t stream);
hipError_t msr_f16_row_error(const float* emb, const float* inv_norm, int64_t n_rows, uint32_t* err_max, hipStream_t stream);
void msr_gemm_f32_set_dbg(int v);
hipError_t msr_pad_inv_norm(const float* inv, int64_t n, int64_t n_pad, float* out, hipStream_t stream);
hipError_t msr_gemm_f32_topk(const GemmF32Index& g, const DenseIndex& ix, const float* qn, int nq, int k,
                             int32_t* out_doc, float* out_score, int32_t* out_chunk,
                             int32_t* out_n, int32_t* gate, hipEvent_t* ev, int* width_out, hipStream_t stream);
hipError_t msr_gemm_f32_pass(const GemmF32Index& g, const DenseIndex& ix, const float* qn, int nq, int k, int k_part,
                             float* out_part, hipEvent_t* ev, int* width_out, hipStream_t stream);
hipError_t msr_gemm_f32_finish(const GemmF32Index& g, const DenseIndex& ix, const float* qn, int nq, int k, const float* bound,
                               int32_t* out_doc, float* out_score, int32_t* out_chunk, int32_t* out_n, int32_t* gate,
                               hipStream_t stream);

hipError_t msr_batch_rescore_rows(const DenseIndex& ix, const float* qn, int nq, int k, const int32_t* rows, int row_stride,
                                  int row_cap, int32_t* cand_doc, float* cand_score, int32_t* cand_chunk, int32_t* cand_n,
                                  int32_t* out_doc, float* out_score, int32_t* out_chunk, int32_t* out_n, hipStream_t stream);
hipError_t msr_batch_finish(const DenseIndex& ix, const float* qn, int nq, int k, int max_chunks, const float* margin,
                            const float* scores, const float* top_score, const int32_t* top_n, int32_t* cand_doc,
                            float* cand_score, int32_t* cand_chunk, int32_t* cand_n, int32_t* out_doc,
                            float* out_score, int32_t* out_chunk, int32_t* out_n, hipStream_t stream);
```

modern-search-engines-project_amd/engine.py:

```python
import ctypes as C

import numpy as np
import torch

from . import _abi
from .index import DIM, CorpusIndex

RERANK_DEFAULTS = dict(smoothing=0.15, max_boost=0.1, max_decay=0.05, max_chunks=10)


def _ptr(t):
    return C.c_void_p(t.data_ptr()) if t is not None else C.c_void_p(0)


STREAM_MIN_BYTES = 64 << 20
_NP_OF = {torch.float32: np.float32, torch.float64: np.float64, torch.int32: np.int32, torch.int64: np.int64,
          torch.int16: np.int16}


def stream_to_device(arr, device, block_bytes=128 << 20):
    dev = torch.device(device)
    out = torch.empty(arr.shape, dtype=torch.from_numpy(np.empty(0, arr.dtype)).dtype, device=dev)
    if arr.size == 0:
        return out
    flat_out = out.view(-1)
    row = int(np.prod(arr.shape[1:], dtype=np.int64)) if arr.ndim > 1 else 1
    rows_per_block = max(1, block_bytes // max(1, row * arr.itemsize))
    pinned = dev.type == "cuda"
    stage = [torch.empty(rows_per_block * row, dtype=out.dtype, pin_memory=pinned) for _ in range(2)]
    done = [None, None]
    for b, r0 in enumerate(range(0, arr.shape[0], rows_per_block)):
        r1 = min(arr.shape[0], r0 + rows_per_block)
        buf = stage[b & 1]
        if done[b & 1] is not None:
            done[b & 1].synchronize()
        n = (r1 - r0) * row
        np.copyto(buf.numpy()[:n].reshape((r1 - r0,) + tuple(arr.shape[1:])), arr[r0:r1])
        flat_out[r0 * row:r0 * row + n].copy_(buf[:n], non_blocking=pinned)
        if pinned:
            done[b & 1] = torch.cuda.Event()
            done[b & 1].record(torch.cuda.current_stream(dev))
    if pinned:
        torch.cuda.current_stream(dev).synchronize()
    return out


class DeviceEngine:
    def __init__(self, index: CorpusIndex, device=0, max_queries=32, max_k=1000, rerank_max_docs=1000,
                 scan_layout=0, scan_variant=0, row_copy=True):
        if not torch.cuda.is_available():
            raise _abi.MsrError(-102, "no GPU visible: the retrieval path runs on MI355X only (no CPU fallback)")
        self.lib = _abi.load()
        self.index = index
        self.device = torch.device("cuda", device) if isinstance(device, int) else torch.device(device)
        self.max_k = int(max_k)
        self.max_queries = int(max_queries)
        self.scan_layout = int(scan_layout)
        self.rerank_max_docs = int(rerank_max_docs)
        cfg = _abi.MsrConfig(C.sizeof(_abi.MsrConfig), self.device.index or 0, DIM, int(max_queries), int(max_k),
                             int(rerank_max_docs), int(scan_layout), int(scan_variant),
                             0 if row_copy else _abi.MSR_CFG_NO_ROW_COPY)
        self.handle = C.c_void_p()
        rc = self.lib.msr_create(C.byref(cfg), C.byref(self.handle))
        if rc != 0:
            raise _abi.MsrError(rc, (self.lib.msr_last_error(None) or b"?").decode())
        self._t = {}
        self._bf16 = False
        self._bind(index)

    def _stream(self):
        return C.c_void_p(torch.cuda.current_stream(self.device).cuda_stream)

    def _dev(self, x, dtype):
        if x is None:
            return None
        if torch.is_tensor(x):
            return x.to(device=self.device, dtype=dtype).contiguous()
        if isinstance(x, np.ndarray) and x.nbytes >= STREAM_MIN_BYTES and x.dtype == _NP_OF[dtype]:
            return stream_to_device(x, self.device)
        x = np.ascontiguousarray(x)
        if not x.flags.writeable:
            x = x.copy()
        return torch.as_tensor(x).to(device=self.device, dtype=dtype)

    def _check(self, rc):
        _abi.check(self.handle, rc)

    def close(self):
        if getattr(self, "handle", None) is not None and self.handle.value:
            torch.cuda.synchronize(self.device)
            self.lib.msr_destroy(self.handle)
            self.handle = C.c_void_p()

    def __del__(self):
        try:
            self.close()
        except Exception:
            pass

    def _bind(self, ix):
        t = self._t
        with torch.cuda.device(self.device):
            if ix.term_off is not None and ix.n_terms > 0:
                t["term_off"] = self._dev(ix.term_off, torch.int64)
                t["post_doc"] = self._dev(ix.post_doc, torch.int32)
                t["post_tf"] = self._dev(ix.post_tf, torch.int32)
                t["doc_len"] = self._dev(ix.doc_len, torch.int32)
                t["idf"] = self._dev(ix.idf, torch.float32)
                self._check(self.lib.msr_bind_postings(
                    self.handle, _ptr(t["term_off"]), ix.n_terms, _ptr(t["post_doc"]), _ptr(t["post_tf"]),
                    int(t["post_doc"].numel()), _ptr(t["doc_len"]), ix.n_docs, _ptr(t["idf"]),
                    C.c_float(ix.avgdl), C.c_double(ix.k1), C.c_double(ix.b), self._stream()))
                if ix.tok_off is not None:
                    tok_off, tok_ids = self._dev(ix.tok_off, torch.int64), self._dev(ix.tok_ids, torch.int32)
                    self._check(self.lib.msr_bind_tokens(self.handle, _ptr(tok_off), _ptr(tok_ids) if tok_ids.numel() else
                                                         C.c_void_p(0), ix.n_docs, int(tok_ids.numel()), self._stream()))
                    t["tok_off"], t["tok_ids"] = tok_off, tok_ids
                if ix.vocab:
                    char_off, chars, weight = ix.vocab_image()
                    v_off, v_w = self._dev(char_off, torch.int64), self._dev(weight.view(np.int32), torch.int32)
                    v_chars = self._dev(chars.view(np.int16), torch.int16)
                    self._check(self.lib.msr_bind_vocab(self.handle, _ptr(v_off), _ptr(v_chars) if v_chars.numel() else
                                                        C.c_void_p(0), _ptr(v_w), ix.n_terms, int(v_chars.numel()),
                                                        self._stream()))
                    t["voc_off"], t["voc_chars"], t["voc_weight"] = v_off, v_chars, v_w
            if ix.doc_off is not None and ix.emb is not None:
                t["doc_off"] = self._dev(ix.doc_off, torch.int32)
                emb = self._dev(ix.emb, torch.float32)
                n_chunks = int(emb.shape[0])
                inv = None
                if self.scan_layout == 1:
                    nrm = torch.linalg.vector_norm(emb, dim=1)
                    inv = (1.0 / torch.where(nrm == 0, torch.ones_like(nrm), nrm)).contiguous()
                    pad = (n_chunks + 15) // 16 * 16
                    tiled = torch.empty((pad, DIM), dtype=torch.float32, device=self.device)
                    self._check(self.lib.msr_interleave_rows(self.handle, _ptr(emb), n_chunks, _ptr(tiled), self._stream()))
                    torch.cuda.synchronize(self.device)
                    del emb
                    emb = tiled
                t["emb"], t["inv_norm"] = emb, inv
                self._check(self.lib.msr_bind_chunks(self.handle, _ptr(emb), n_chunks, _ptr(t["doc_off"]),
                                                     ix.n_docs, _ptr(inv), self._stream()))
                t["url_group"] = self._dev(ix.url_group(), torch.int32)
                self._check(self.lib.msr_bind_doc_meta(self.handle, _ptr(t["url_group"]), ix.n_docs, self._stream()))
            torch.cuda.synchronize(self.device)

    def rebind(self, ix: CorpusIndex):
        torch.cuda.synchronize(self.device)
        self._check(self.lib.msr_unbind(self.handle))
        self._t = {}
        self.index = ix
        try:
            self._bind(ix)
            if self._bf16:
                self.enable_bf16()
        except Exception:
            torch.cuda.synchronize(self.device)
            self.lib.msr_unbind(self.handle)
            self._t = {}
            raise

    @property
    def has_tokens(self):
        return "tok_off" in self._t

    @property
    def has_vocab(self):
        return "voc_off" in self._t

    def fuzzy_terms(self, words, max_edits=None, limit=1):
        from .fuzzy import auto_edits, encode_words, lookable
        if not self.has_vocab:
            raise _abi.MsrError(-2, "fuzzy_terms: the index has no vocabulary (CorpusIndex.vocab: term strings); a term-id-only "
                                    "index cannot suggest words")
        limit = int(limit)
        if not 1 <= limit <= _abi.MSR_FUZZY_MAX_LIMIT:
            raise ValueError(f"fuzzy_terms: limit must be 1 .. MSR_FUZZY_MAX_LIMIT = {_abi.MSR_FUZZY_MAX_LIMIT} (got {limit})")
        words = list(words)
        W = len(words)
        if max_edits is None:
            maxes = [auto_edits(len(w)) if isinstance(w, str) else 0 for w in words]
        else:
            maxes = [int(max_edits)] * W if np.ndim(max_edits) == 0 else [int(v) for v in max_edits]
            if len(maxes) != W or any(not 0 <= m <= 2 for m in maxes):
                raise ValueError("fuzzy_terms: max_edits is None, or 0 .. 2 for every word")
        out = [([], 0)] * W
        ask = [i for i in range(W) if lookable(words[i])]
        step = _abi.MSR_FUZZY_MAX_WORDS
        for a in range(0, len(ask), step):
            part = ask[a:a + step]
            n = len(part)
            off, chars = encode_words([words[i] for i in part])
            chars32 = np.zeros((len(chars) + 1) // 2 + 1, np.int32)
            chars32.view(np.uint16)[:len(chars)] = chars
            up = self._dev(np.concatenate([off, np.asarray([maxes[i] for i in part], np.int32), chars32]), torch.int32)
            d_off, d_max, d_chars = up[:n + 1], up[n + 1:2 * n + 1], up[2 * n + 1:]
            res = torch.empty((2 * n * limit + 2 * n,), dtype=torch.int32, device=self.device)
            need = int(self.lib.msr_fuzzy_scratch_bytes(self.index.n_terms, n, limit))
            scratch = torch.empty(((need + 7) // 8,), dtype=torch.int64, device=self.device)
            r_term, r_dist = res[:n * limit], res[n * limit:2 * n * limit]
            r_n, r_total = res[2 * n * limit:2 * n * limit + n], res[2 * n * limit + n:]
            self._check(self.lib.msr_fuzzy_terms(self.handle, n, _ptr(d_off), _ptr(d_chars), _ptr(d_max), limit, _ptr(r_term),
                                                 _ptr(r_dist), _ptr(r_n), _ptr(r_total), _ptr(scratch), need, self._stream()))
            host = res.cpu().numpy()
            term, dist = host[:n * limit].reshape(n, limit), host[n * limit:2 * n * limit].reshape(n, limit)
            cnt, total = host[2 * n * limit:2 * n * limit + n], host[2 * n * limit + n:]
            for j, i in enumerate(part):
                out[i] = ([(int(term[j, c]), int(dist[j, c])) for c in range(int(cnt[j]))], int(total[j]))
        return out

    def scan_arith(self):
        return {0: "f32", 1: "f16x2"}.get(self.lib.msr_scan_arith(self.handle), "none")

    def batch_width(self):
        return int(self.lib.msr_batch_width(self.handle))

    def batch_gemm_ok(self):
        return bool(self.lib.msr_batch_gemm_ok(self.handle))

    def scan_width(self):
        return int(self.lib.msr_scan_width(self.handle))

    def row_copy_state(self):
        return {0: "none", 1: "built", 2: "declined", 3: "alloc_failed"}.get(self.lib.msr_row_copy_state(self.handle), "?")

    def row_image_state(self):
        return {0: "none", 1: "built", 2: "declined", 3: "alloc_failed"}.get(self.lib.msr_row_image_state(self.handle), "?")

    def owned_bytes(self):
        return int(self.lib.msr_owned_bytes(self.handle))

    def dense_path(self):
        return int(self.lib.msr_dense_path(self.handle))

    def pack_queries(self, term_lists):
        off, terms, qtf = [0], [], []
        for tl in term_lists:
            cnt = {}
            for t in tl:
                cnt[int(t)] = cnt.get(int(t), 0) + 1
            if len(cnt) > 64:
                raise ValueError("a query may hold at most 64 unique terms (MSR_MAX_QUERY_TERMS)")
            for t, c in cnt.items():
                terms.append(t)
                qtf.append(c)
            off.append(len(terms))
        mk = lambda a: torch.tensor(a if a else [0], dtype=torch.int32, device=self.device)
        return mk(off), mk(terms), mk(qtf), len(term_lists)

    def pack_within(self, within, n_queries):
        from .docset import DeviceSets, DocSet, pack_within
        if isinstance(within, DeviceSets):
            within.check(self.index)
            if len(within) != n_queries:
                raise ValueError(f"within: {len(within)} entries for {n_queries} queries")
            return within.bits, within.q_set, within.n_sets, within.stride
        if isinstance(within, DocSet):
            within.check(self.index)
            stride = max(1, (self.index.n_docs + 31) // 32)
            bits = within.to(self.device).reshape(1, -1)
            if bits.shape[1] < stride:
                bits = torch.nn.functional.pad(bits, (0, stride - bits.shape[1]))
            return bits, torch.zeros((n_queries,), dtype=torch.int32, device=self.device), 1, stride
        words, q_set, n_sets, stride = pack_within(within, n_queries, self.index)
        bits = torch.from_numpy(words.view(np.int32)).to(self.device)
        return bits, torch.from_numpy(q_set).to(self.device), n_sets, stride

    def term_sets(self, must, must_not=None, within=None):
        from .docset import DeviceSets
        bits, q_set, n_sets, stride, _ = self._term_rows(must, must_not, within)
        return DeviceSets(self.index, bits, torch.tensor(q_set, dtype=torch.int32, device=self.device), n_sets, stride)

    def _term_rows(self, must, must_not, within, extra_rows=0, tail=None):
        from .docset import DeviceSets, DocSet, pack_within
        from .index import _np
        ix = self.index
        if ix.term_off is None or ix.n_terms <= 0:
            raise _abi.MsrError(-2, "term_sets: the index has no postings")
        if must is None and must_not is None:
            raise ValueError("term_sets: must or must_not is needed (a list of term ids per query)")
        Q = len(must if must is not None else must_not)
        must = [()] * Q if must is None else list(must)
        must_not = [()] * Q if must_not is None else list(must_not)
        if len(must) != Q or len(must_not) != Q:
            raise ValueError(f"term_sets: {len(must)} must lists and {len(must_not)} must_not lists")
        stride = max(1, (ix.n_docs + 31) // 32)
        base_bits, n_base, base_of = None, 0, [-1] * Q
        if isinstance(within, DocSet):
            base_bits, _, n_base, _ = self.pack_within(within, Q)
            base_of = [0] * Q
        elif within is not None:
            if isinstance(within, DeviceSets):
                raise TypeError("term_sets: within takes DocSets (a DeviceSets is a result, not a base)")
            words, base_q, n_base, _ = pack_within(within, Q, ix)
            base_of = base_q.tolist()
            if n_base:
                base_bits = torch.from_numpy(words.view(np.int32)).to(self.device)
        df = getattr(self, "_df", None)
        if df is None or df[0] is not ix:
            df = self._df = (ix, np.diff(_np(ix.term_off).astype(np.int64)))
        df, n_terms = df[1], int(ix.n_terms)
        EMPTY = ((-1,), ())
        rows, row_of, q_row, keep_base = [], {}, [], False
        for q in range(Q):
            m = {int(t) if 0 <= int(t) < n_terms else -1 for t in must[q]}
            x = {int(t) for t in must_not[q] if 0 <= int(t) < n_terms and df[int(t)] > 0}
            if not m and not x:
                q_row.append(None)
                keep_base = keep_base or base_of[q] >= 0
                continue
            if -1 in m or m & x or any(df[t] == 0 for t in m):
                key = EMPTY + (-1,)
            else:
                key = (tuple(sorted(m, key=lambda t: (df[t], t))), tuple(sorted(x)), base_of[q])
            r = row_of.get(key)
            if r is None:
                r = row_of[key] = len(rows)
                rows.append(key)
            q_row.append(r)
        first = n_base if keep_base else 0
        q_set = [(base_of[q] if base_of[q] >= 0 and keep_base else -1) if r is None else first + r for q, r in enumerate(q_row)]
        bits = torch.empty((first + len(rows) + int(extra_rows), stride), dtype=torch.int32, device=self.device)
        if first:
            bits[:first] = base_bits
        n_sets = first + len(rows)
        tail_host = [int(v) for v in tail(q_set, n_sets)] if tail is not None else []
        d_tail = None
        if not rows and tail_host:
            d_tail = torch.from_numpy(np.asarray(tail_host, np.int32)).to(self.device)
        if rows:
            m_off, m_terms, x_off, x_terms = [0], [], [0], []
            for m, x, _ in rows:
                m_terms.extend(m); m_off.append(len(m_terms))
                x_terms.extend(x); x_off.append(len(x_terms))
            R = len(rows)
            host = np.asarray(m_off + x_off + [b for _, _, b in rows] + m_terms + x_terms + tail_host, np.int32)
            dev = torch.from_numpy(host).to(self.device)
            p_moff, p_xoff, p_base = dev[:R + 1], dev[R + 1:2 * R + 2], dev[2 * R + 2:3 * R + 2]
            p_m = dev[3 * R + 2:3 * R + 2 + len(m_terms)]
            end = 3 * R + 2 + len(m_terms) + len(x_terms)
            p_x = dev[3 * R + 2 + len(m_terms):end]
            if tail_host:
                d_tail = dev[end:]
            self._check(self.lib.msr_term_sets(self.handle, R, _ptr(p_moff), _ptr(p_m), _ptr(p_xoff), _ptr(p_x),
                                               _ptr(base_bits) if n_base else C.c_void_p(0), n_base, stride,
                                               _ptr(p_base) if n_base else C.c_void_p(0), _ptr(bits[first:]), stride,
                                               self._stream()))
        return bits, q_set, n_sets, stride, d_tail

    def phrase_sets(self, must_phrases, must_not_phrases=None, must=None, must_not=None, within=None):
        from .docset import DeviceSets, DocSet
        from .text import Near
        ix = self.index
        if not self.has_tokens:
            raise _abi.MsrError(-2, "phrase_sets: the index has no forward index (tok_off / tok_ids): build it with "
                                    "keep_tokens=True or attach the token streams with index_build.attach_tokens, then rebind")
        if must_phrases is None and must_not_phrases is None:
            raise ValueError("phrase_sets: must_phrases or must_not_phrases is needed (a list of phrases per query)")
        Q = len(must_phrases if must_phrases is not None else must_not_phrases)
        lists = [[()] * Q if x is None else list(x) for x in (must_phrases, must_not_phrases, must, must_not)]
        if any(len(x) != Q for x in lists):
            raise ValueError(f"phrase_sets: {[len(x) for x in lists]} must_phrases / must_not_phrases / must / must_not lists")
        mp, xp, m, x = lists
        if isinstance(within, DocSet) or within is None:
            base = [within] * Q
        else:
            if isinstance(within, DeviceSets):
                raise TypeError("phrase_sets: within takes DocSets (a DeviceSets is a result, not a base)")
            base = list(within)
            if len(base) != Q:
                raise ValueError(f"within: {len(base)} entries for {Q} queries")
        n_terms = int(ix.n_terms)
        ids_of = lambda p: tuple(int(t) if 0 <= int(t) < n_terms else -1 for t in p)
        norm = lambda p: p.with_terms(ids_of(p.terms)) if isinstance(p, Near) else ids_of(p)
        terms_of = lambda p: list(p.terms) if isinstance(p, Near) else list(p)
        v_must, v_not, v_base, plan = [], [], [], []
        for q in range(Q):
            ph_m, ph_x = [norm(p) for p in mp[q]], [norm(p) for p in xp[q]]
            for p in ph_m + ph_x:
                if len(p) > _abi.MSR_PHRASE_MAX_TERMS:
                    raise ValueError(f"a phrase may hold at most {_abi.MSR_PHRASE_MAX_TERMS} terms (MSR_PHRASE_MAX_TERMS), got {len(p)}")
            own = len(v_must)
            v_must.append(list(m[q])); v_not.append(list(x[q])); v_base.append(base[q])
            plan.append((own, ph_m, len(v_must), ph_x, len(v_must) + len(ph_m)))
            for p in ph_m:
                v_must.append(terms_of(p) + list(m[q])); v_not.append(list(x[q])); v_base.append(base[q])
# ... 446 lines not shown
```

Before: 59270.

## Split the f32 emit pass into segments and tighten thresholds between them

The emit pass of the dense f32 GEMM filter now runs over tile segments, two by default with the split near sqrt(T·n_s). After each non-final segment it recomputes the k-th tile maximum over the tiles seen so far and raises the per-query threshold, so later segments emit fewer candidates into the wave buffers. This adds extra kth-kernel launches and per-segment launches in exchange for fewer candidate emits and less downstream bucketing and rerank work. A config flag restores single-segment behaviour, and a diagnostic API reports segment and entry counts.

Measured after the change: 60550 (median of 6 runs). 1.02x the previous value.

```diff
diff --git a/include/msretr.h b/include/msretr.h
--- a/include/msretr.h
+++ b/include/msretr.h
@@ -46,6 +46,7 @@
 } msr_config;
 
 #define MSR_CFG_NO_ROW_COPY 1
+#define MSR_CFG_SINGLE_EMIT 2
 
 typedef struct msr_rerank_params {
     double smoothing;
@@ -78,6 +79,7 @@
 
 int msr_scan_width(const msr_engine* e);
 int msr_dense_path(const msr_engine* e);
+int msr_dense_pass_info(msr_engine* e, int32_t* segments, int64_t* entries);
 int msr_batch_width(const msr_engine* e);
 int msr_batch_gemm_ok(const msr_engine* e);
 
diff --git a/modern-search-engines-project_amd/_abi.py b/modern-search-engines-project_amd/_abi.py
--- a/modern-search-engines-project_amd/_abi.py
+++ b/modern-search-engines-project_amd/_abi.py
@@ -6,6 +6,7 @@
 
 MSR_ABI_VERSION = 15
 MSR_CFG_NO_ROW_COPY = 1
+MSR_CFG_SINGLE_EMIT = 2
 MSR_DIM = 768
 MSR_MAX_K = 1024
 MSR_RERANK_MAX_CHUNKS = 10
@@ -58,6 +59,7 @@
     "msr_scan_arith": (C.c_int, [_P]),
     "msr_scan_width": (C.c_int, [_P]),
     "msr_dense_path": (C.c_int, [_P]),
+    "msr_dense_pass_info": (C.c_int, [_P, C.POINTER(C.c_int32), C.POINTER(C.c_int64)]),
     "msr_row_copy_state": (C.c_int, [_P]),
     "msr_row_image_state": (C.c_int, [_P]),
     "msr_owned_bytes": (C.c_int64, [_P]),
diff --git a/modern-search-engines-project_amd/csrc/msr_engine.hip b/modern-search-engines-project_amd/csrc/msr_engine.hip
--- a/modern-search-engines-project_amd/csrc/msr_engine.hip
+++ b/modern-search-engines-project_amd/csrc/msr_engine.hip
@@ -95,6 +95,7 @@
     int row_copy_state = 0;
     int row_image_state = 0;
     int last_dense_width = 0;
+    int last_dense_segments = 0;
     int32_t* sim_flag = nullptr;
     void* sim_lists = nullptr; size_t sim_lists_bytes = 0;
     void* sim_over = nullptr; size_t sim_over_bytes = 0;
@@ -232,7 +233,7 @@
     if (cfg->scan_variant != 0 && cfg->scan_variant != 2 && cfg->scan_variant != 7 && cfg->scan_variant != 14 &&
         cfg->scan_variant != 15)
         return fail(nullptr, MSR_ERR_INVALID, "msr_create: scan_variant must be 0, 2, 7, 14 or 15");
-    if (cfg->flags & ~(int32_t)MSR_CFG_NO_ROW_COPY)
+    if (cfg->flags & ~(int32_t)(MSR_CFG_NO_ROW_COPY | MSR_CFG_SINGLE_EMIT))
         return fail(nullptr, MSR_ERR_INVALID, "msr_create: unknown flag bits 0x%x", cfg->flags);
     int ndev = 0;
     hipError_t herr = hipGetDeviceCount(&ndev);
@@ -538,6 +539,7 @@
     const int max_nt = std::max(1, std::min(4, groups / 2));
     GemmF32Index& g = e->gf;
     g.n_tiles = n_tiles; g.n_cus = e->n_cus; g.max_groups = groups; g.tmax_stride = stride; g.wv_cap = GF_WV_CAP; g.max_nt = max_nt;
+    g.single_emit = (e->cfg.flags & MSR_CFG_SINGLE_EMIT) ? 1 : 0;
     ALLOC(e, e->mem_chunks, e->gf_inv_pad, (size_t)(n_chunks + 512) * 4);
     ALLOC(e, e->mem_chunks, g.qimg, (size_t)groups * 24 * 8192);
     ALLOC(e, e->mem_chunks, e->gf_qn, (QM + 64) * MSR_DIM * 4);
@@ -647,6 +649,7 @@
     e->url_group = nullptr; e->url_group_n = 0;
     e->doc_domain = nullptr; e->doc_domain_n = 0;
     e->last_dense_width = 0;
+    e->last_dense_segments = 0;
     e->mem_corpus.release();
     e->score_rows_bytes = e->bm_cand_bytes = 0;
     return MSR_OK;
@@ -712,6 +715,22 @@
 }
 
 extern "C" int msr_dense_path(const msr_engine* e) { return e ? e->last_dense_width : -1; }
+
+extern "C" int msr_dense_pass_info(msr_engine* e, int32_t* segments, int64_t* entries) {
+    if (!e) return MSR_ERR_INVALID;
+    if (!segments || !entries) return fail(e, MSR_ERR_INVALID, "msr_dense_pass_info: null argument");
+    *segments = e->last_dense_segments;
+    *entries = 0;
+    if (!e->have_chunks || !e->gf_ok || e->last_dense_segments == 0) return MSR_OK;
+    HIP_TRY(e, hipSetDevice(e->cfg.device));
+    HIP_TRY(e, hipDeviceSynchronize());
+    std::vector<int32_t> cnt((size_t)e->gf.n_cus * 8);
+    HIP_TRY(e, hipMemcpy(cnt.data(), e->gf.wv_count, cnt.size() * sizeof(int32_t), hipMemcpyDeviceToHost));
+    int64_t sum = 0;
+    for (int32_t c : cnt) sum += c;
+    *entries = sum;
+    return MSR_OK;
+}
 
 extern "C" int64_t msr_owned_bytes(const msr_engine* e) {
     if (!e) return -1;
@@ -1173,8 +1192,10 @@
     hipEvent_t ev_buf[4];
     hipEvent_t* ev = pass_events(e, 0, ev_buf);
     int width = 0;
-    HIP_TRY(e, msr_gemm_f32_pass(e->gf, e->dense, e->gf_qn, n_queries, k, k_part, out_part, ev, &width, st));
+    int segs = 0;
+    HIP_TRY(e, msr_gemm_f32_pass(e->gf, e->dense, e->gf_qn, n_queries, k, k_part, out_part, ev, &width, &segs, st));
     e->last_dense_width = width;
+    e->last_dense_segments = segs;
     pass_events_used(e, 0, ev);
     e->split_pending = n_queries;
     return MSR_OK;
@@ -1243,6 +1264,7 @@
     const bool wide = dense_sweep_wide(e, max_chunks_per_doc);
     const bool gemm = wide && dense_stream_ok(e, k);
     e->last_dense_width = gemm && n_queries > 64 ? 0 : (wide ? 64 : 32);
+    e->last_dense_segments = 0;
     int q0 = 0;
     while (q0 < n_queries) {
         const int left = n_queries - q0;
@@ -1252,11 +1274,12 @@
             HIP_TRY(e, hipMemsetAsync(e->gf_gate, 0, GF_GATE_BYTES, st));
             hipEvent_t ev_buf[4];
             hipEvent_t* ev = pass_events(e, 0, ev_buf);
-            int width = 0;
+            int width = 0, segs = 0;
             HIP_TRY(e, msr_gemm_f32_topk(e->gf, e->dense, e->gf_qn, nq, k, out_doc + (int64_t)q0 * k,
                                          out_score + (int64_t)q0 * k, out_chunk ? out_chunk + (int64_t)q0 * k : nullptr,
-                                         out_n + q0, e->gf_gate, ev, &width, st));
+                                         out_n + q0, e->gf_gate, ev, &width, &segs, st));
             e->last_dense_width = std::max(e->last_dense_width, width);
+            e->last_dense_segments = segs;
             pass_events_used(e, 0, ev);
             {
                 int rcf = dense_gated_fallback(e, nq, k, out_doc + (int64_t)q0 * k, out_score + (int64_t)q0 * k,
@@ -1295,6 +1318,7 @@
     HIP_TRY(e, hipSetDevice(e->cfg.device));
     const bool wide = dense_sweep_wide(e, max_chunks_per_doc);
     e->last_dense_width = wide ? 64 : 32;
+    e->last_dense_segments = 0;
     const MsrSetView set{set_bits, set_stride, q_set, n_sets};
     return dense_sweeps(e, q, 0, n_queries, k, max_chunks_per_doc, wide, nullptr, out_doc, out_score, out_chunk, out_n, st, &set);
 }
diff --git a/modern-search-engines-project_amd/csrc/msr_gemm.hip b/modern-search-engines-project_amd/csrc/msr_gemm.hip
--- a/modern-search-engines-project_amd/csrc/msr_gemm.hip
+++ b/modern-search-engines-project_amd/csrc/msr_gemm.hip
@@ -118,13 +118,14 @@
 
 __global__ __launch_bounds__(1024) void gemm_kth_kernel(const float* __restrict__ tmax, int n, int stride, int nq, int k,
                                                          const float* __restrict__ margin, float* __restrict__ thr,
-                                                         int32_t* __restrict__ flag, float short_val, float margin_scale) {
+                                                         int32_t* __restrict__ flag, float short_val, float margin_scale,
+                                                         int raise) {
     __shared__ uint32_t hist[2048];
     __shared__ uint32_t wsum[16];
     __shared__ uint32_t s_bin, s_kk, s_hit;
     const int q = blockIdx.x, t = threadIdx.x, lane = t & 63, wave = t >> 6;
     if (q >= nq) {
-        if (t == 0) { thr[q] = short_val; if (flag) flag[q] = 0; }
+        if (t == 0 && !raise) { thr[q] = short_val; if (flag) flag[q] = 0; }
         return;
     }
     const float* row = tmax + (size_t)q * stride;
@@ -169,8 +170,13 @@
         __syncthreads();
     }
     if (t == 0) {
-        thr[q] = short_row ? short_val : msr_unord32(prefix) - (margin ? margin_scale * margin[q] : 0.0f);
-        if (flag) flag[q] = short_row ? 1 : 0;
+        const float v = short_row ? short_val : msr_unord32(prefix) - (margin ? margin_scale * margin[q] : 0.0f);
+        if (raise) {
+            if (!short_row && v > thr[q]) thr[q] = v;
+        } else {
+            thr[q] = v;
+            if (flag) flag[q] = short_row ? 1 : 0;
+        }
     }
 }
 
@@ -327,9 +333,10 @@
     return hipGetLastError();
 }
 hipError_t msr_gemm_kth(const float* tmax, int n, int stride, int nq, int nq_pad, int k, const float* margin, float* thr,
-                        int32_t* flag, hipStream_t stream, float short_val, float margin_scale) {
+                        int32_t* flag, hipStream_t stream, float short_val, float margin_scale, bool raise) {
     if (nq_pad <= 0) return hipSuccess;
-    gemm_kth_kernel<<<nq_pad, 1024, 0, stream>>>(tmax, n, stride, nq, k, margin, thr, flag, short_val, margin_scale);
+    gemm_kth_kernel<<<nq_pad, 1024, 0, stream>>>(tmax, n, stride, nq, k, margin, thr, raise ? nullptr : flag, short_val, margin_scale,
+                                                 raise ? 1 : 0);
     return hipGetLastError();
 }
 hipError_t msr_gemm_bucket(const void* wvbuf, int wv_cap, const int32_t* wv_count, int n_waves, const float* thr2,
@@ -364,14 +371,14 @@
         if ((err = msr_stream256_bf16_launch(false, a, grid, stream)) != hipSuccess) return err;
         if (ev && (err = hipEventRecord(ev[1], stream)) != hipSuccess) return err;
         if ((err = msr_gemm_tmax(g.tmax_t, n_s, 1, nq_pad, (float*)g.tmax, g.tmax_stride, stream)) != hipSuccess) return err;
-        gemm_kth_kernel<<<nq_pad, 1024, 0, stream>>>((const float*)g.tmax, n_s, g.tmax_stride, nq, k, margin, g.thr, g.flag, __builtin_inff(), 1.0f);
+        gemm_kth_kernel<<<nq_pad, 1024, 0, stream>>>((const float*)g.tmax, n_s, g.tmax_stride, nq, k, margin, g.thr, g.flag, __builtin_inff(), 1.0f, 0);
         a.t_first = 0; a.t_stride = 1; a.t_count = g.n_tiles;
         a.thr = g.thr; a.wvbuf = g.wgbuf; a.wv_cap = g.wv_cap; a.wv_count = g.wv_count;
         if (ev && (err = hipEventRecord(ev[2], stream)) != hipSuccess) return err;
         if ((err = msr_stream256_bf16_launch(true, a, grid, stream)) != hipSuccess) return err;
         if (ev && (err = hipEventRecord(ev[3], stream)) != hipSuccess) return err;
         if ((err = msr_gemm_tmax(g.tmax_t, g.n_tiles, 1, nq_pad, (float*)g.tmax, g.tmax_stride, stream)) != hipSuccess) return err;
-        gemm_kth_kernel<<<nq_pad, 1024, 0, stream>>>((const float*)g.tmax, g.n_tiles, g.tmax_stride, nq, k, margin, g.thr2, nullptr, __builtin_inff(), 1.0f);
+        gemm_kth_kernel<<<nq_pad, 1024, 0, stream>>>((const float*)g.tmax, g.n_tiles, g.tmax_stride, nq, k, margin, g.thr2, nullptr, __builtin_inff(), 1.0f, 0);
     }
     gemm_bucket_kernel<<<dim3(2, (unsigned)grid * 8), 256, 0, stream>>>((const int4*)g.wgbuf, g.wv_cap, g.wv_count, g.thr2,
                                                                        (int2*)g.pairs, GM_PAIR_CAP, g.pair_n);
diff --git a/modern-search-engines-project_amd/csrc/msr_gemm_f32.hip b/modern-search-engines-project_amd/csrc/msr_gemm_f32.hip
--- a/modern-search-engines-project_amd/csrc/msr_gemm_f32.hip
+++ b/modern-search-engines-project_amd/csrc/msr_gemm_f32.hip
@@ -1,3 +1,4 @@
+#include <cmath>
 #include <type_traits>
 
 #include "msr_common.h"
@@ -910,8 +911,56 @@
     return hipGetLastError();
 }
 
+namespace {
+struct PassShape {
+    int ss, n_s;
+    int n_seg;
+    int bound[4];
+};
+PassShape pass_shape(int T, int k, int grid, bool single, int dbg) {
+    PassShape p{};
+    int ss = T / (3 * k);
+    ss = ss < 1 ? 1 : (ss > 64 ? 64 : ss);
+    p.ss = ss;
+    p.n_s = (T - ss / 2 + ss - 1) / ss;
+    p.n_seg = 1; p.bound[0] = 0; p.bound[1] = T;
+    if (single) return p;
+    (void)dbg;
+#ifdef MSR_DIAG
+    if ((dbg & 16777216) && grid >= 2 * k && p.n_s > grid) {
+        p.n_s = p.n_s / grid * grid;
+        p.ss = T / p.n_s;
+    }
+#endif
+    const double root = std::sqrt((double)T * (double)p.n_s);
+    int want3 = 0;
+#ifdef MSR_DIAG
+    want3 = dbg & 2097152;
+#endif
+    if (want3) {
+        const double r = std::cbrt((double)T / (double)p.n_s);
+        const int m1 = (int)std::floor(p.n_s * r / grid + 0.5), m2 = (int)std::floor(p.n_s * r * r / grid + 0.5);
+        const int64_t t1 = (int64_t)m1 * grid, t2 = (int64_t)m2 * grid;
+        if (m1 >= 1 && m2 > m1 && t1 >= 2 * k && T - t2 >= grid) {
+            p.n_seg = 3; p.bound[1] = (int)t1; p.bound[2] = (int)t2; p.bound[3] = T;
+            return p;
+        }
+    }
+    int64_t t1 = (int64_t)std::floor(root / grid + 0.5) * grid;
+#ifdef MSR_DIAG
+    if (dbg & 4194304) t1 = std::max<int64_t>(grid, t1 / 2 / grid * grid);
+    if (dbg & 8388608) t1 = 2 * t1;
+#endif
+    if (t1 >= std::max(grid, 2 * k) && T - t1 >= grid) {
+        p.n_seg = 2; p.bound[1] = (int)t1; p.bound[2] = T;
+    }
+    return p;
+}
+
+}
+
 hipError_t msr_gemm_f32_pass(const GemmF32Index& g, const DenseIndex& ix, const float* qn, int nq, int k, int k_part,
-                             float* out_part, hipEvent_t* ev, int* width_out, hipStream_t stream) {
+                             float* out_part, hipEvent_t* ev, int* width_out, int* seg_out, hipStream_t stream) {
     const int W = nq > 128 ? 256 : 128;
     const int waves = 8;
     const int G = (nq + W - 1) / W;
@@ -929,10 +978,10 @@
     else build_qimg1_kernel<<<dim3((GF_KT * 128 * 4 + 255) / 256, G), 256, 0, stream>>>(qn, nq, (f16x8*)g.qimg);
     f16_margin_kernel<<<(nq + 3) / 4, 256, 0, stream>>>(qn, nq, g.err_max, g.margin);
     const float* margin = g.margin;
-    int ss = g.n_tiles / (3 * k);
-    ss = ss < 1 ? 1 : (ss > 64 ? 64 : ss);
-    const int n_s = (g.n_tiles - ss / 2 + ss - 1) / ss;
     const int grid = g.n_cus;
+    const PassShape shape = pass_shape(g.n_tiles, k, grid, g.single_emit != 0, g_f32_dbg);
+    const int ss = shape.ss, n_s = shape.n_s;
+    if (seg_out) *seg_out = shape.n_seg;
     const size_t qimg_bytes = (size_t)GF_KT * W * 64;
     int NT = 1;
     if (W == 256 && (grid & 7) == 0) NT = std::min(std::min(G, g.max_nt), grid >> 3);
@@ -961,16 +1010,23 @@
         if ((err = msr_gemm_tmax(g.tmax_t, n_s, tmax_parts, W * a.nt, g.tmax + (size_t)gi * W * g.tmax_stride, g.tmax_stride, stream)) != hipSuccess) return err;
     }
     if ((err = msr_gemm_kth(g.tmax, n_s, g.tmax_stride, nq, W * G, k, margin, g.thr, g.flag, stream)) != hipSuccess) return err;
-    a.t_first = 0; a.t_stride = 1; a.t_count = g.n_tiles;
+    a.t_stride = 1;
     a.wvbuf = g.wvbuf; a.wv_cap = g.wv_cap * (8 / waves); a.wv_count = g.wv_count;
-    for (int gi = 0; gi < G; gi += NT) {
-        a.nt = std::min(NT, G - gi);
-        a.qimg = (const char*)g.qimg + gi * qimg_bytes;
-        a.thr = g.thr + gi * W; a.q_base = gi * W; a.append = gi > 0;
-        if (ev && gi == 0 && (err = hipEventRecord(ev[2], stream)) != hipSuccess) return err;
-        if ((err = launch_f32(W, true, a, grid, stream, tiled, image16)) != hipSuccess) return err;
-        if (ev && gi == 0 && (err = hipEventRecord(ev[3], stream)) != hipSuccess) return err;
-        if ((err = msr_gemm_tmax(g.tmax_t, g.n_tiles, tmax_parts, W * a.nt, g.tmax + (size_t)gi * W * g.tmax_stride, g.tmax_stride, stream)) != hipSuccess) return err;
+    for (int s = 0; s < shape.n_seg; ++s) {
+        const int t0 = shape.bound[s], t1 = shape.bound[s + 1];
+        a.t_first = t0; a.t_count = t1 - t0;
+        for (int gi = 0; gi < G; gi += NT) {
+            a.nt = std::min(NT, G - gi);
+            a.qimg = (const char*)g.qimg + gi * qimg_bytes;
+            a.thr = g.thr + gi * W; a.q_base = gi * W; a.append = (s > 0 || gi > 0);
+            if (ev && gi == 0 && s == 0 && (err = hipEventRecord(ev[2], stream)) != hipSuccess) return err;
+            if ((err = launch_f32(W, true, a, grid, stream, tiled, image16)) != hipSuccess) return err;
+            if (ev && gi == 0 && s == shape.n_seg - 1 && (err = hipEventRecord(ev[3], stream)) != hipSuccess) return err;
+            if ((err = msr_gemm_tmax(g.tmax_t, t1 - t0, tmax_parts, W * a.nt, g.tmax + (size_t)gi * W * g.tmax_stride + t0, g.tmax_stride, stream)) != hipSuccess) return err;
+        }
+        if (s + 1 < shape.n_seg &&
+            (err = msr_gemm_kth(g.tmax, t1, g.tmax_stride, nq, W * G, k, margin, g.thr, nullptr, stream, __builtin_inff(), 1.0f, true)) != hipSuccess)
+            return err;
     }
     if ((err = msr_gemm_kth(g.tmax, g.n_tiles, g.tmax_stride, nq, W * G, k, margin, g.thr2, nullptr, stream)) != hipSuccess) return err;
     if (out_part && (err = msr_gemm_kth(g.tmax, g.n_tiles, g.tmax_stride, nq, nq, k_part, margin, out_part, nullptr, stream,
@@ -1009,8 +1065,8 @@
 
 hipError_t msr_gemm_f32_topk(const GemmF32Index& g, const DenseIndex& ix, const float* qn, int nq, int k,
                              int32_t* out_doc, float* out_score, int32_t* out_chunk,
-                             int32_t* out_n, int32_t* gate, hipEvent_t* ev, int* width_out, hipStream_t stream) {
-    hipError_t err = msr_gemm_f32_pass(g, ix, qn, nq, k, k, nullptr, ev, width_out, stream);
+                             int32_t* out_n, int32_t* gate, hipEvent_t* ev, int* width_out, int* seg_out, hipStream_t stream) {
+    hipError_t err = msr_gemm_f32_pass(g, ix, qn, nq, k, k, nullptr, ev, width_out, seg_out, stream);
     if (err != hipSuccess) return err;
     return msr_gemm_f32_finish(g, ix, qn, nq, k, nullptr, out_doc, out_score, out_chunk, out_n, gate, stream);
 }
diff --git a/modern-search-engines-project_amd/csrc/msr_internal.h b/modern-search-engines-project_amd/csrc/msr_internal.h
--- a/modern-search-engines-project_amd/csrc/msr_internal.h
+++ b/modern-search-engines-project_amd/csrc/msr_internal.h
@@ -272,7 +272,8 @@
 int msr_gemm_pair_cap();
 hipError_t msr_gemm_tmax(const float* tmax_t, int n_j, int parts, int nq_pad, float* out, int out_stride, hipStream_t stream);
 hipError_t msr_gemm_kth(const float* tmax, int n, int stride, int nq, int nq_pad, int k, const float* margin, float* thr,
-                        int32_t* flag, hipStream_t stream, float short_val = __builtin_inff(), float margin_scale = 1.0f);
+                        int32_t* flag, hipStream_t stream, float short_val = __builtin_inff(), float margin_scale = 1.0f,
+                        bool raise = false);
 hipError_t msr_gemm_bucket(const void* wvbuf, int wv_cap, const int32_t* wv_count, int n_waves, const float* thr2,
                            void* pairs, int32_t* pair_n, hipStream_t stream);
 void msr_bm25_set_dbg(int v);
@@ -324,6 +325,7 @@
     const void* emb_tiled;
     const int32_t* tile_trow;
     const void* emb_f16;
+    int32_t single_emit;
 };
 hipError_t msr_f16_rows(const float* emb, int64_t n_rows, int64_t n_pad, void* out, hipStream_t stream);
 hipError_t msr_tile_rows(const float* emb, const int32_t* tile_row, const int32_t* tile_trow, int n_tiles, void* emb_tiled,
@@ -333,9 +335,9 @@
 hipError_t msr_pad_inv_norm(const float* inv, int64_t n, int64_t n_pad, float* out, hipStream_t stream);
 hipError_t msr_gemm_f32_topk(const GemmF32Index& g, const DenseIndex& ix, const float* qn, int nq, int k,
                              int32_t* out_doc, float* out_score, int32_t* out_chunk,
-                             int32_t* out_n, int32_t* gate, hipEvent_t* ev, int* width_out, hipStream_t stream);
+                             int32_t* out_n, int32_t* gate, hipEvent_t* ev, int* width_out, int* seg_out, hipStream_t stream);
 hipError_t msr_gemm_f32_pass(const GemmF32Index& g, const DenseIndex& ix, const float* qn, int nq, int k, int k_part,
-                             float* out_part, hipEvent_t* ev, int* width_out, hipStream_t stream);
+                             float* out_part, hipEvent_t* ev, int* width_out, int* seg_out, hipStream_t stream);
 hipError_t msr_gemm_f32_finish(const GemmF32Index& g, const DenseIndex& ix, const float* qn, int nq, int k, const float* bound,
                                int32_t* out_doc, float* out_score, int32_t* out_chunk, int32_t* out_n, int32_t* gate,
                                hipStream_t stream);
diff --git a/modern-search-engines-project_amd/engine.py b/modern-search-engines-project_amd/engine.py
--- a/modern-search-engines-project_amd/engine.py
+++ b/modern-search-engines-project_amd/engine.py
@@ -47,7 +47,7 @@
 
 class DeviceEngine:
     def __init__(self, index: CorpusIndex, device=0, max_queries=32, max_k=1000, rerank_max_docs=1000,
-                 scan_layout=0, scan_variant=0, row_copy=True):
+                 scan_layout=0, scan_variant=0, row_copy=True, single_emit=False):
         if not torch.cuda.is_available():
             raise _abi.MsrError(-102, "no GPU visible: the retrieval path runs on MI355X only (no CPU fallback)")
         self.lib = _abi.load()
@@ -59,7 +59,7 @@
         self.rerank_max_docs = int(rerank_max_docs)
         cfg = _abi.MsrConfig(C.sizeof(_abi.MsrConfig), self.device.index or 0, DIM, int(max_queries), int(max_k),
                              int(rerank_max_docs), int(scan_layout), int(scan_variant),
-                             0 if row_copy else _abi.MSR_CFG_NO_ROW_COPY)
+                             (0 if row_copy else _abi.MSR_CFG_NO_ROW_COPY) | (_abi.MSR_CFG_SINGLE_EMIT if single_emit else 0))
         self.handle = C.c_void_p()
         rc = self.lib.msr_create(C.byref(cfg), C.byref(self.handle))
         if rc != 0:
@@ -232,6 +232,11 @@
 
     def dense_path(self):
         return int(self.lib.msr_dense_path(self.handle))
+
+    def dense_pass_info(self):
+        seg, ent = C.c_int32(0), C.c_int64(0)
+        self._check(self.lib.msr_dense_pass_info(self.handle, C.byref(seg), C.byref(ent)))
+        return int(seg.value), int(ent.value)
 
     def pack_queries(self, term_lists):
         off, terms, qtf = [0], [], []
```
